# apache/yunikorn-k8shim

Measured on AMD Instinct MI355X. Metric: pod×node predicate evals/sec + decisions/sec, 50k nodes × 1M pods, higher is better.
Workload: dtype int64; 1 GPU; configs[2]: 50k nodes x 1M pods, NodeResourcesFit + TaintToleration + NodeAffinity; nodes_per_gpu=50000, total_nodes=50000, pods=1000000, templates=2000, pod_classes=2061, signature_planes=327, unique_requests=False, spread=False, gang_size=0, parallelism=single GPU

## Files before the change

### yunikorn-k8shim_amd/csrc/engine/engine.hip

```cpp
#include "../../../include/ykpred.h"

#include <hip/hip_runtime.h>
#include <dlfcn.h>
#include <rccl/rccl.h>

#include <algorithm>
#include <chrono>
#include <cstdio>
#include <cstdlib>
#include <cstring>
#include <mutex>
#include <string>
#include <map>
#include <unordered_map>
#include <vector>

#include "kernels.hip.h"
#include "preempt_headroom_finish.h"

using ykk::i64;
using ykk::u64;

namespace {

// ... 126 lines not shown
  T* as() const {
    return static_cast<T*>(p);
  }
};

struct ClassKey {
  int32_t a, b, c, d, pin;
  bool operator==(const ClassKey& o) const { return a == o.a && b == o.b && c == o.c && d == o.d && pin == o.pin; }
};
struct ClassKeyHash {
  size_t operator()(const ClassKey& k) const {
    uint64_t h = (uint64_t)(uint32_t)k.a * 0x9e3779b97f4a7c15ull;
    h ^= ((uint64_t)(uint32_t)k.b + 0x7f4a7c15ull) * 0xbf58476d1ce4e5b9ull;
    h ^= ((uint64_t)(uint32_t)k.c + 0x1ce4e5b9ull) * 0x94d049bb133111ebull;
    h ^= ((uint64_t)(uint32_t)k.pin + 0x133111ebull) * 0xd6e8feb86659fd93ull;
    h ^= ((uint64_t)(uint32_t)k.d + 0x6659fd93ull) * 0xff51afd7ed558ccdull;
    return (size_t)(h ^ (h >> 29));
  }
};

struct Family {
  int D = 0;
  int base = 0;
};

}

struct ykpred_engine {
  mutable std::recursive_mutex mu;
  ykpred_config_t cfg{};
  int R = 3, KT = 1, W = 1;
  hipStream_t own_stream = nullptr;
  std::string err;

  int N = 0;
  int row_words = 0, row_stride = 0;
  DevBuf d_alloc, d_req, d_allowed, d_count, d_nflags, d_taints, d_labels, d_domain, d_selcount, d_ports;
  int KD = 0, KS = 0, KP = 0;
  std::vector<int32_t> h_domain_sizes;
  DevBuf d_score, d_key, d_rank, d_perm, d_rankbuf, d_member_key, d_name_rank, d_member_tie;
  bool has_name_rank = false;
  bool nodes_set = false;

  int S = 0;
  std::vector<i64> h_req;
  std::vector<u64> h_tol, h_wanted;
  std::vector<uint32_t> h_sflags;
  std::vector<int32_t> h_aff_off, h_pre_off, h_spread_off;
  std::vector<ykpred_spread_t> h_spread;
  std::vector<u64> h_aff_terms, h_pre_terms;
  DevBuf d_sreq, d_stol, d_sflags, d_aff_off, d_aff_terms, d_pre_off, d_pre_terms;
  std::vector<int32_t> spec_sig_res, spec_sig_tol, spec_sig_aff;
  Family fam_res, fam_tol, fam_aff, fam_spread;
  DevBuf planes_canon, planes_ranked;
  DevBuf base_canon, base_ranked;
  u64 taint_used[ykk::kMaxKT] = {0, 0, 0, 0};
  int plane_rows_alloc = 0;
  std::vector<int32_t> spec_sig_spread;
  std::vector<std::vector<ykpred_spread_t>> spread_sig;
  std::vector<int32_t> spread_sig_aff, spread_sig_tol;
  DevBuf d_spec_spread, d_sp_coff, d_sp_c, d_sp_aff, d_sp_tol, d_sp_cnt, d_sp_present, d_sp_min;
  DevBuf d_sp_cnt_prev, d_sp_present_prev, d_sp_min_prev, d_sig_changed, d_class_dirty;
  int spread_constraints = 0;
  int64_t spread_cells = 0;
  bool spread_dirty = true;
  int res_vectors = 0;
  std::vector<i64> h_dim_val;
  std::vector<int32_t> h_dim_of;
  std::vector<int32_t> h_stage_rows;
  DevBuf d_dim_val, d_dim_order, d_dim_chunk_dim, d_dim_chunk_begin, d_dim_chunk_len, d_res_rows;
  int dim_chunks = 0;
  int walk_rows = 256;
  int wave_combine_below = 16;
  int n_big = 0, walk_chunks = 0, index_rows = 0;
  int NCB = 0;
  DevBuf d_big_dim, d_walk_big, d_walk_begin, d_walk_len, d_sfree_c, d_pmask_c, d_sfree_r, d_pmask_r, d_rbits_c;
  std::vector<int32_t> h_res_rows;
  std::vector<int32_t> h_row_pos;
  std::vector<int32_t> h_row_big;
  std::vector<int32_t> h_sorted_off;
  DevBuf d_sorted, d_sorted_off, d_ent_c;
  int sweep_min_run = 1;
  int sweep_groups = 0;
  bool sweep_ready = false;
  std::vector<int32_t> h_class_sweep;
  int sweep_rows[ykk::kMaxIdxRows] = {0, 0}, sweep_row_off[ykk::kMaxIdxRows + 1] = {0, 0, 0}, sweep_runs = 0;
  int index_rows_needed = 0;
  DevBuf d_agree;
  DevBuf d_explain;
  DevBuf d_headroom;
  DevBuf d_groups;
  DevBuf d_domain_head;
  DevBuf d_reach;
  DevBuf d_rc_req, d_rc_pods, d_rc_ports;
  int rc_tiers = 0;
  bool rc_ports = false;
  DevBuf d_victims;
  DevBuf d_vt_base, d_vt_tier_end, d_vt_cum, d_vt_ports;
  std::vector<int32_t> h_vt_base, h_vt_cap;
  int vt_tiers = 0;
  size_t vt_rows = 0;
  bool vt_ports = false;
  DevBuf d_bytes_gather;
  DevBuf d_topo_agree;
  u64 dict_digest = 0;
  int fuse_rows = 1;
  int fuse_wpl = 0;
  int fuse_count = 0, fuse_row_count = 0;
  bool fuse_ready = false;
  DevBuf d_fuse_rec;
  int fuse_combos = 0;
  int fuse_combine = 1;
  DevBuf d_fuse_combo_rec, d_fuse_combo;
  std::vector<uint8_t> h_class_fused;
  int run_decide = 1;
  int run_ranges = 0, n_decide_list = 0, run_decide_classes = -1;
  bool win_partial = false;
  DevBuf d_run_ranges, d_no_decide, d_glin_r;
  int class_runs = 1;
  int class_runs_min_rows = 16;
  int run_classes = 0, run_units = 0, run_rows = 0;
  DevBuf d_run_classes, d_run_units;
  DevBuf d_sweep_rows, d_sweep_runs, d_sweep_units;
  int sweep_units[ykk::kMaxIdxRows] = {0, 0}, sweep_unit_off[ykk::kMaxIdxRows + 1] = {0, 0, 0};
  DevBuf d_chunk_list_b0;
  int NCB0 = 0;
  DevBuf d_walk2_order, d_walk2_big, d_walk2_begin, d_walk2_len;
  int walk2_chunks = -1;
  DevBuf d_first_r;
  static constexpr bool decide_skip = true;
  DevBuf d_chunk_list_b;
  DevBuf d_slice_general;
  DevBuf d_slice_desc;
  DevBuf d_pfx_r;
  DevBuf d_idx_c;
  DevBuf d_win_r;
  int idx_stride = 0;
  DevBuf d_sig_tol, d_sig_tolflags, d_sig_ports, d_swanted;
  DevBuf d_sig_aff_flags, d_sig_aff_off, d_sig_aff_terms, d_sig_pre_off, d_sig_pre_terms;
  bool specs_set = false;

  int P = 0, C = 0, NC = 0;
  std::vector<int32_t> h_pod_spec, h_pod_pin;
  DevBuf d_pod_spec, d_pod_pin, d_pod_class;
  DevBuf d_class_sig, d_class_pin, d_class_first, d_class_word, d_chunk_class, d_chunk_begin, d_chunk_len, d_chunk_first, d_members;
  std::unordered_map<ClassKey, int32_t, ClassKeyHash> class_ids;
  std::vector<int32_t> h_pod_class, h_pod_slot;
  std::vector<int32_t> h_pod_row;
  int rows_total = 0, rows_a = 0, row_capacity = 0;
  DevBuf d_pod_row;
  bool bands_enabled = true;
  int band_steps = 0;
  int band_steps_now = 128;
  int round_batched = -1;
  int round_node_assume = 1;
  int round_prof = 0;
  int fail_after = 0;
  int sig_wpl = 0;
  int combine_slices = 1;
  int decide_groups_from = 16384;
  int early_counts = 1;
  int group_lds = -1;
  int group_scratch_mb = 256;
  int affinity_fill_waves = 0;
  int group_chunk_tasks = 0;
  int max_lds_bytes = 64 * 1024;
  int num_cus = 256;
  int n_bands = 0, n_band_steps = 0, n_classes_a = 0, n_fix_rows = 0;
  std::vector<int32_t> h_class_slot_a;
  DevBuf d_band_tab, d_class_rows_a, d_class_list_a, d_class_slot_a, d_fix_row, d_fix_slot, d_chunk_zone;
  DevBuf d_class_list_b;
  int n_classes_b = 0;
  std::vector<int32_t> h_ch_zone;
  std::vector<uint8_t> h_row_stale;
  std::vector<int32_t> h_class_sig, h_class_pin, h_class_first, h_class_live;
  std::vector<std::vector<int32_t>> h_class_chunks;
  std::vector<int32_t> h_members, h_ch_class, h_ch_begin, h_ch_len, h_ch_first;
  int patch_chunks = 0;
  bool rank_valid = false;
  uint64_t specs_version = 1, ranked_specs_version = 0, ranked_nodes_epoch = 0;
  unsigned ranked_pre = 0, ranked_filt = 0;
  bool ranked_has_first = false;
  DevBuf d_round;
  DevBuf d_fx_off, d_fx_cls, d_fx_cnt, d_fx_occ, d_sp_sig_of;
  uint64_t fx_version = 0;
  bool fx_contrib = false, fx_ports = false;
  std::vector<int32_t> h_fx_off;
  std::vector<int32_t> h_fx_cls;
  std::vector<int32_t> h_fx_cnt;
  std::vector<uint8_t> h_fx_occupies;
  DevBuf d_patches, d_rows, d_row_count, d_row_best;
  unsigned last_pre = 0, last_filt = 0;
  bool last_eval_valid = false;
  DevBuf d_class_count, d_class_best;
  bool pods_set = false, classes_dirty = true;
  int chunk_members = ykk::kChunkMembers;
  bool chunk_sorted = true;
  int combine_lds_bytes = 40000;

  DevBuf d_bitmap, d_counts, d_decisions, d_keys, d_scratch;
  void* last_bitmap = nullptr;
  int64_t last_bitmap_rows = 0;
  void *last_counts = nullptr, *last_decisions = nullptr, *last_keys = nullptr;

  hipStream_t aux_stream = nullptr;
  hipEvent_t ev_fork = nullptr, ev_planes = nullptr, ev_join = nullptr, ev_counts = nullptr, ev_zero = nullptr;
  hipStream_t peek_stream = nullptr;
  hipEvent_t ev_eval_done = nullptr;
  void* peek_pinned = nullptr;
  size_t peek_pinned_bytes = 0;

  struct GraphKey {
    uint64_t version;
    unsigned pre, filt, options;
    void *bitmap, *counts, *decisions, *keys;
    bool operator==(const GraphKey& o) const {
      return version == o.version && pre == o.pre && filt == o.filt && options == o.options && bitmap == o.bitmap && counts == o.counts &&
             decisions == o.decisions && keys == o.keys;
    }
  };
  std::vector<std::pair<GraphKey, hipGraphExec_t>> graphs;
  std::vector<GraphKey> seen;
  uint64_t tables_version = 1;
  bool graph_disabled = true;

  ncclComm_t comm = nullptr;
  int comm_rank = 0, comm_world = 1, node_offset = 0;
  int64_t round_exchanges = 0;
  void* h_round_pinned = nullptr;
  size_t h_round_pinned_bytes = 0;
  int64_t rounds_batched = 0, round_batched_asks = 0, round_batches = 0, rounds_sequential = 0, round_sequential_asks = 0;
  int forced_stride = 0;
  DevBuf d_gathered, d_gathered_map, d_xkey, d_xcand;
  bool last_has_keys = false;
  DevBuf d_class_rows_all, d_gathered_classes, d_class_rows_slot, d_class_sig_ident, d_expand_count, d_layout_hash, d_gathered_pod_class, d_row_pod;
  int ident_classes = 0;
  uint64_t layout_version = 1, layout_hashed_version = 0, layout_hash_value = 0, row_pod_version = 0;
  uint64_t ask_epoch = 1, hdr_epoch = 0;
  std::vector<uint64_t> hdr_cache;
  uint64_t nodes_epoch = 1, hist_epoch = 0;
  uint64_t bitmap_epoch = 0;

  int64_t n_full_evals = 0, n_node_patches = 0, n_row_patches = 0, n_queries = 0, n_gathers = 0, n_uploads = 0;

  hipEvent_t ev[2 * YKPRED_MAX_TIMED_KERNELS + 2]{};
  bool ev_ready = false;
  int timed = 0;
  const char* timed_name[YKPRED_MAX_TIMED_KERNELS]{};
  bool timing_valid = false;
};

namespace {

int fail(ykpred_engine* e, int code, const std::string& msg) {
  if (e) e->err = msg;
  if (e && (code == YKPRED_E_DEVICE || code == YKPRED_E_NOMEM)) {
    e->last_eval_valid = false;
    e->rank_valid = false;
    e->classes_dirty = true;
    e->spread_dirty = true;
    e->hist_epoch = 0;
    e->ranked_nodes_epoch = 0;
    e->tables_version++;
  }
  return code;
}
inline bool inject_failure(ykpred_engine* e) { return e && e->fail_after > 0 && --e->fail_after == 0; }
#define HIPCHK(call)                                                                                        \
  do {                                                                                                      \
    hipError_t _s = inject_failure(e) ? hipErrorUnknown : (call);                                          \
    if (_s != hipSuccess)                                                                                   \
      return fail(e, _s == hipErrorOutOfMemory ? YKPRED_E_NOMEM : YKPRED_E_DEVICE,                          \
                  std::string(#call) + ": " + hipGetErrorString(_s));                                       \
  } while (0)

template <class T>
int upload(ykpred_engine* e, DevBuf& b, const T* src, size_t n, hipStream_t st) {
  HIPCHK(b.ensure(n * sizeof(T)));
  if (n) HIPCHK(hipMemcpyAsync(b.p, src, n * sizeof(T), hipMemcpyHostToDevice, st));
  return YKPRED_OK;
}
#define TRY(x)                     \
  do {                             \
    int _r = (x);                  \
    if (_r != YKPRED_OK) return _r; \
  } while (0)

ykk::NodeTable node_table(const ykpred_engine* e) {
  ykk::NodeTable t;
  t.n = e->N;
  t.R = e->R;
  t.KT = e->KT;
  t.W = e->W;
  t.alloc = e->d_alloc.as<i64>();
  t.req = e->d_req.as<i64>();
  t.allowed = e->d_allowed.as<int>();
  t.count = e->d_count.as<int>();
  t.flags = e->d_nflags.as<unsigned>();
  t.taints = e->d_taints.as<u64>();
  t.labels = e->d_labels.as<u64>();
  t.KD = e->KD;
  t.KS = e->KS;
  t.domain = e->d_domain.as<int>();
  t.selcount = e->d_selcount.as<int>();
  t.KP = e->KP;
  t.ports = e->d_ports.as<u64>();
  return t;
}
ykk::SpreadSigs spread_sigs(const ykpred_engine* e) {
  ykk::SpreadSigs sp;
  sp.D = e->fam_spread.D;
  sp.c_off = e->d_sp_coff.as<int>();
  sp.c = e->d_sp_c.as<ykk::SpreadC>();
  sp.aff_sig = e->d_sp_aff.as<int>();
  sp.tol_sig = e->d_sp_tol.as<int>();
  sp.cnt = e->d_sp_cnt.as<int>();
  sp.present = e->d_sp_present.as<int>();
  sp.minv = e->d_sp_min.as<int>();
  return sp;
}
ykk::SpecTable spec_table(const ykpred_engine* e) {
  ykk::SpecTable s;
  s.R = e->R;
  s.KT = e->KT;
  s.W = e->W;
  s.req = e->d_sreq.as<i64>();
  s.tol = e->d_stol.as<u64>();
  s.flags = e->d_sflags.as<unsigned>();
  s.aff.flags = e->d_sflags.as<unsigned>();
  s.aff.term_off = e->d_aff_off.as<int>();
  s.aff.terms = e->d_aff_terms.as<u64>();
  s.aff.pre_off = e->d_pre_off.as<int>();
  s.aff.pre_terms = e->d_pre_terms.as<u64>();
  s.KP = e->KP;
  s.wanted_ports = e->d_swanted.as<u64>();
  s.spread_sig = e->d_spec_spread.as<int>();
  s.spread = spread_sigs(e);
  return s;
}

int build_classes(ykpred_engine* e, hipStream_t st) {
  e->tables_version++;
  const int P = e->P;
  auto& ids = e->class_ids;
  ids.clear();
  ids.reserve(1024);
  auto& pod_class = e->h_pod_class;
  pod_class.assign((size_t)P, 0);
  auto &class_sig = e->h_class_sig, &class_pin = e->h_class_pin, &class_size = e->h_class_live;
  class_sig.clear();
  class_pin.clear();
  class_size.clear();
  for (int p = 0; p < P; ++p) {
    int s = e->h_pod_spec[(size_t)p];
    ClassKey k{e->spec_sig_res[(size_t)s], e->spec_sig_tol[(size_t)s], e->spec_sig_aff[(size_t)s], e->spec_sig_spread[(size_t)s],
               e->h_pod_pin[(size_t)p]};
    auto it = ids.find(k);
    int32_t c;
    if (it == ids.end()) {
      c = (int32_t)class_pin.size();
      ids.emplace(k, c);
      class_sig.insert(class_sig.end(), {k.a, k.b, k.c, k.d});
      class_pin.push_back(k.pin);
      class_size.push_back(0);
    } else {
      c = it->second;
    }
    pod_class[(size_t)p] = c;
    class_size[(size_t)c]++;
  }
  const int C = (int)class_pin.size();
  std::vector<int32_t> class_off((size_t)C + 1, 0);
  for (int c = 0; c < C; ++c) class_off[(size_t)c + 1] = class_off[(size_t)c] + class_size[(size_t)c];
  auto& members = e->h_members;
  members.assign((size_t)P, 0);
  e->h_pod_slot.assign((size_t)P, 0);
  std::vector<int32_t> cursor(class_off.begin(), class_off.end() - 1);
  for (int p = 0; p < P; ++p) {
    int slot = cursor[(size_t)pod_class[(size_t)p]]++;
    members[(size_t)slot] = p;
    e->h_pod_slot[(size_t)p] = slot;
  }
  const long row_b = (long)e->row_stride * 8, win = (long)ykk::kBandGroups * 4096;
  const int KC = ykk::kBandClasses;
  auto piece_min_of = [&](int steps) { return (int)((double)steps * (4096.0 + (double)row_b) / (double)row_b / (double)(KC - 1) * 1.3) + 3; };
  int S = e->band_steps;
  if (S <= 0) {
    int s_min = 8;
    while (s_min < 128 && (long)s_min * 4096 < 5L * KC * row_b) s_min *= 2;
    auto coverage = [&](int steps) {
      const int need = 2 * piece_min_of(steps);
      long rows = 0;
      for (int c = 0; c < C; ++c)
        if (class_size[(size_t)c] >= need) rows += class_size[(size_t)c];
      return rows;
    };
    const long best = coverage(s_min);
    S = 128;
    while (S > s_min && (double)coverage(S) < 0.5 * (double)best) S /= 2;
  }
  while (S > 4 && (long)S * win / row_b >= (1L << 21)) S -= 4;
  e->band_steps_now = S;
  const int piece_min = piece_min_of(S);
  e->h_class_slot_a.assign((size_t)C, -1);
  e->h_pod_row.assign((size_t)P, -1);
  std::vector<ykk::BandEntry> band_tab;
  std::vector<int32_t> class_list_a, fix_row, fix_slot;
  int n_steps = 0, n_bands = 0, rows_a = 0;
  const bool geometry_ok = e->bands_enabled && e->N > 0 && (size_t)2 * KC * (size_t)row_b <= (size_t)std::min(ykk::kBandMaxLds, e->max_lds_bytes);
  if (geometry_ok) {
    long rows_needed = 0;
    for (int c = 0; c < C; ++c)
      if (class_size[(size_t)c] >= 2 * piece_min) {
        e->h_class_slot_a[(size_t)c] = (int32_t)class_list_a.size();
        class_list_a.push_back(c);
// ... 433 lines not shown
          else rec.row[rec.n++] = r;
        }
        if (!ok) continue;
        recs.push_back(rec);
        e->h_class_fused[(size_t)c] = 1;
        e->fuse_count++;
        e->fuse_row_count += rec.len;
      }
      e->fuse_combos = 0;
      if (e->fuse_count > 0) {
        std::unordered_map<uint64_t, int32_t> combo_of;
        std::vector<ykk::FuseRec> combo_recs;
        std::vector<int32_t> combo_ix(recs.size(), -1);
        for (size_t i = 0; i < recs.size(); ++i) {
          const int32_t c = recs[i].cls;
          const uint64_t k2 = ((uint64_t)(uint32_t)key(c, 1) << 32) | (uint32_t)key(c, 0);
          auto it = combo_of.find(k2);
          if (it == combo_of.end()) {
            it = combo_of.emplace(k2, (int32_t)combo_recs.size()).first;
            ykk::FuseRec cr{};
            cr.cls = 0, cr.dest = it->second, cr.len = 1;
            for (int k = 1; k < recs[i].n; ++k) cr.row[cr.n++] = recs[i].row[k];
            combo_recs.push_back(cr);
          }
          combo_ix[i] = it->second;
        }
        bool combine = e->fuse_combine != 0 && combo_recs.size() * 4 <= recs.size() && combo_recs.size() <= 16384;
        for (const ykk::FuseRec& cr : combo_recs) combine = combine && cr.n >= 1;
        if (combine) {
          for (size_t i = 0; i < recs.size(); ++i) {
            recs[i].n = 2;
            recs[i].row[1] = (3 << ykk::kFuseFamShift) | combo_ix[i];
          }
          e->fuse_combos = (int)combo_recs.size();
          TRY(upload(e, e->d_fuse_combo_rec, combo_recs.data(), combo_recs.size(), st));
          HIPCHK(e->d_fuse_combo.ensure((size_t)e->fuse_combos * (size_t)e->row_stride * sizeof(u64)));
        }
        TRY(upload(e, e->d_fuse_rec, recs.data(), recs.size(), st));
        e->fuse_ready = true;
      }
      if (getenv("YKPRED_TRACE_RUNS")) {
        long t_cls = 0, t_rows = 0, t_single = 0, t_single_shared = 0, t_single_big = 0, t_single_spread = 0, t_pinned = 0;
        for (int32_t c : order_b) {
          if (!tail[(size_t)c] || e->h_class_sweep[(size_t)c] || e->h_class_fused[(size_t)c]) continue;
          ++t_cls, t_rows += class_size[(size_t)c];
          if (class_size[(size_t)c] == 1) {
            ++t_single;
            const int sa = key(c, 2);
            if (sa >= 0 && sa < e->fam_aff.D && users[(size_t)sa] != 1) ++t_single_shared;
            if (key(c, 3) >= 0) ++t_single_spread;
            if (class_pin[(size_t)c] != -1) ++t_pinned;
            const int sr = key(c, 0);
            if (sr >= 0)
              for (int k = 0; k < R1; ++k)
                if (e->h_res_rows[(size_t)sr * (size_t)R1 + (size_t)k] > 0 && (e->h_res_rows[(size_t)sr * (size_t)R1 + (size_t)k] >> ykk::kRowBigShift)) { ++t_single_big; break; }
          }
        }
        fprintf(stderr, "fused: %d classes, %d rows, %d combinations; chunk writers keep %ld classes / %ld rows of zone B (%ld single-row: %ld share their affinity signature, %ld with an index row, %ld spread, %ld pinned)\n",
                e->fuse_count, e->fuse_row_count, e->fuse_combos, t_cls, t_rows, t_single, t_single_shared, t_single_big, t_single_spread, t_pinned);
      }
    }
  }
  e->rows_total = next_row;
  e->rows_a = rows_a;
  e->n_bands = n_bands;
  e->n_band_steps = n_steps;
  e->n_classes_a = (int)class_list_a.size();
  e->n_fix_rows = (int)fix_row.size();
  if (e->row_capacity && e->rows_total > e->row_capacity)
    return fail(e, YKPRED_E_INVALID, "the bitmap needs more rows than ykpred_set_row_capacity allows");
  const int cm = e->chunk_members;
  struct Chunk {
    int32_t cls, begin, len, first, first_row;
  };
  std::vector<Chunk> chunks;
  for (int c = 0; c < C; ++c)
    for (int b = class_off[(size_t)c]; b < class_off[(size_t)c + 1]; b += cm)
      chunks.push_back({c, b, std::min(cm, class_off[(size_t)c + 1] - b), b == class_off[(size_t)c] ? 1 : 0, e->h_pod_row[(size_t)members[(size_t)b]]});
  if (e->chunk_sorted)
    std::stable_sort(chunks.begin(), chunks.end(), [](const Chunk& x, const Chunk& y) { return x.first_row < y.first_row; });
  auto &ch_class = e->h_ch_class, &ch_begin = e->h_ch_begin, &ch_len = e->h_ch_len, &ch_first = e->h_ch_first;
  ch_class.clear();
  ch_begin.clear();
  ch_len.clear();
  ch_first.clear();
  e->h_ch_zone.clear();
  e->h_class_chunks.assign((size_t)C, {});
  for (const Chunk& k : chunks) {
    e->h_class_chunks[(size_t)k.cls].push_back((int32_t)ch_class.size());
    ch_class.push_back(k.cls);
    ch_begin.push_back(k.begin);
    ch_len.push_back(k.len);
    ch_first.push_back(k.first);
    e->h_ch_zone.push_back(e->h_class_slot_a[(size_t)k.cls] >= 0 ? 1 : (e->h_class_sweep[(size_t)k.cls] ? 2 : (e->h_class_fused[(size_t)k.cls] ? 3 : 0)));
  }
  std::vector<int32_t> chunk_list_b;
  for (size_t k = 0; k < e->h_ch_zone.size(); ++k)
    if (e->h_ch_zone[k] != 1) chunk_list_b.push_back((int32_t)k);
  e->NCB = (int)chunk_list_b.size();
  {
    std::vector<int32_t> chunk_list_b0;
    for (size_t k = 0; k < e->h_ch_zone.size(); ++k)
      if (e->h_ch_zone[k] == 0) chunk_list_b0.push_back((int32_t)k);
    e->NCB0 = (int)chunk_list_b0.size();
    TRY(upload(e, e->d_chunk_list_b0, chunk_list_b0.data(), chunk_list_b0.size(), st));
  }
  e->h_class_first.assign((size_t)C, -1);
  for (int c = 0; c < C; ++c) e->h_class_first[(size_t)c] = members[(size_t)class_off[(size_t)c]];
  std::vector<int32_t> member_rows((size_t)P);
  for (int i = 0; i < P; ++i) member_rows[(size_t)i] = e->h_pod_row[(size_t)members[(size_t)i]];
  e->h_row_stale.assign((size_t)P, 0);
  e->C = C;
  e->NC = (int)ch_class.size();
  e->patch_chunks = 0;
  TRY(upload(e, e->d_pod_class, pod_class.data(), pod_class.size(), st));
  TRY(upload(e, e->d_class_sig, class_sig.data(), class_sig.size(), st));
  TRY(upload(e, e->d_class_pin, class_pin.data(), class_pin.size(), st));
  TRY(upload(e, e->d_class_first, e->h_class_first.data(), e->h_class_first.size(), st));
  TRY(upload(e, e->d_members, member_rows.data(), member_rows.size(), st));
  TRY(upload(e, e->d_pod_row, e->h_pod_row.data(), e->h_pod_row.size(), st));
  TRY(upload(e, e->d_chunk_zone, e->h_ch_zone.data(), e->h_ch_zone.size(), st));
  TRY(upload(e, e->d_chunk_list_b, chunk_list_b.data(), chunk_list_b.size(), st));
  TRY(upload(e, e->d_band_tab, band_tab.data(), band_tab.size(), st));
  TRY(upload(e, e->d_class_list_a, class_list_a.data(), class_list_a.size(), st));
  TRY(upload(e, e->d_class_slot_a, e->h_class_slot_a.data(), e->h_class_slot_a.size(), st));
  TRY(upload(e, e->d_fix_row, fix_row.data(), fix_row.size(), st));
  TRY(upload(e, e->d_fix_slot, fix_slot.data(), fix_slot.size(), st));
  HIPCHK(e->d_class_rows_a.ensure((size_t)std::max<size_t>(class_list_a.size(), 1) * (size_t)e->row_stride * sizeof(u64)));
  TRY(upload(e, e->d_chunk_class, ch_class.data(), ch_class.size(), st));
  TRY(upload(e, e->d_chunk_begin, ch_begin.data(), ch_begin.size(), st));
  TRY(upload(e, e->d_chunk_len, ch_len.data(), ch_len.size(), st));
  TRY(upload(e, e->d_chunk_first, ch_first.data(), ch_first.size(), st));
  HIPCHK(e->d_class_count.ensure((size_t)std::max(C, 1) * sizeof(int)));
  HIPCHK(e->d_class_best.ensure((size_t)std::max(C, 1) * sizeof(int)));
  HIPCHK(hipStreamSynchronize(st));
  e->classes_dirty = false;
  e->layout_version++;
  e->last_eval_valid = false;
  return YKPRED_OK;
}

int ensure_planes(ykpred_engine* e, hipStream_t st) {
  int rows = 0;
  for (Family* f : {&e->fam_res, &e->fam_spread, &e->fam_tol, &e->fam_aff}) {
    f->base = rows;
    rows += std::max(f->D, 1);
  }
  size_t need = ((size_t)rows * (size_t)e->row_stride + 64) * sizeof(u64);
  for (DevBuf* b : {&e->planes_canon, &e->planes_ranked}) {
    if (b->cap < need || e->plane_rows_alloc != rows) {
      e->tables_version++;
      HIPCHK(b->ensure(need));
      HIPCHK(hipMemsetAsync(b->p, 0, need, st));
    }
  }
  e->plane_rows_alloc = rows;
  size_t base_need = (size_t)(64 * (e->W + e->KT + e->KP) + 2) * (size_t)e->row_stride * sizeof(u64);
  for (DevBuf* b : {&e->base_canon, &e->base_ranked}) {
    if (b->cap < base_need) {
      e->tables_version++;
      HIPCHK(b->ensure(base_need));
      HIPCHK(hipMemsetAsync(b->p, 0, base_need, st));
    }
  }
  return YKPRED_OK;
}

int build_spread_tables(ykpred_engine* e, hipStream_t st) {
  e->tables_version++;
  std::vector<int32_t> coff{0}, aff, tol;
  std::vector<ykk::SpreadC> rows;
  int64_t cells = 0;
  for (size_t d = 0; d < e->spread_sig.size(); ++d) {
    for (const ykpred_spread_t& c : e->spread_sig[d]) {
      if (c.topology_key < 0 || c.topology_key >= e->KD || c.selector_class >= e->KS)
        return fail(e, YKPRED_E_INVALID, "spread constraint references a topology key / selector class outside the node table");
      ykk::SpreadC r;
      r.kd = c.topology_key;
      r.ks = c.selector_class;
      r.max_skew = c.max_skew;
      r.min_domains = c.min_domains;
      r.self_match = c.self_match;
      r.flags = c.flags;
      r.kind = c.kind;
      r.dom_size = (size_t)c.topology_key < e->h_domain_sizes.size() ? e->h_domain_sizes[(size_t)c.topology_key] : 0;
      r.cnt_off = (int)cells;
      cells += r.dom_size;
      if (cells > 0x7fffffff) return fail(e, YKPRED_E_UNSUPPORTED, "spread histograms exceed 2^31 cells");
      rows.push_back(r);
    }
    coff.push_back((int32_t)rows.size());
    aff.push_back(e->spread_sig_aff[d]);
    tol.push_back(e->spread_sig_tol[d]);
  }
  e->spread_constraints = (int)rows.size();
  e->spread_cells = cells;
  TRY(upload(e, e->d_sp_coff, coff.data(), coff.size(), st));
  TRY(upload(e, e->d_sp_c, rows.data(), rows.size(), st));
  TRY(upload(e, e->d_sp_aff, aff.data(), aff.size(), st));
  TRY(upload(e, e->d_sp_tol, tol.data(), tol.size(), st));
  HIPCHK(e->d_sp_cnt.ensure((size_t)std::max<int64_t>(cells, 1) * sizeof(int)));
  HIPCHK(e->d_sp_present.ensure((size_t)std::max<int64_t>(cells, 1) * sizeof(int)));
  HIPCHK(e->d_sp_min.ensure((size_t)std::max(e->spread_constraints, 1) * sizeof(int)));
  HIPCHK(hipStreamSynchronize(st));
  e->spread_dirty = false;
  return YKPRED_OK;
}

struct Timer {
  ykpred_engine* e;
  bool on;
  void start(hipStream_t st) {
    e->timed = 0;
    e->timing_valid = false;
    if (on) (void)hipEventRecord(e->ev[2 * YKPRED_MAX_TIMED_KERNELS], st);
  }
  void begin(hipStream_t st) {
    if (on && e->timed < YKPRED_MAX_TIMED_KERNELS) (void)hipEventRecord(e->ev[2 * e->timed], st);
  }
  void end(hipStream_t st, const char* name) {
    if (trace_kernels_on()) {
      const hipError_t s = hipStreamSynchronize(st);
      fprintf(stderr, "ykpred: %s %s\n", name, s == hipSuccess ? "done" : hipGetErrorString(s));
      fflush(stderr);
    }
    if (!on || e->timed >= YKPRED_MAX_TIMED_KERNELS) return;
    (void)hipEventRecord(e->ev[2 * e->timed + 1], st);
    e->timed_name[e->timed] = name;
    e->timed++;
  }
  void done(hipStream_t st) {
    if (on) (void)hipEventRecord(e->ev[2 * YKPRED_MAX_TIMED_KERNELS + 1], st);
    e->timing_valid = on;
  }
};

int grow_owned_outputs(ykpred_engine* e) {
  const size_t P = (size_t)std::max(e->P, 1);
  if (e->last_bitmap && e->last_bitmap == e->d_bitmap.p) {
    HIPCHK(e->d_bitmap.reserve_keep((size_t)std::max(std::max(e->rows_total, e->row_capacity), 1) * (size_t)e->row_stride * sizeof(u64), e->d_bitmap.cap));
    e->last_bitmap = e->d_bitmap.p;
  }
  if (e->last_counts && e->last_counts == e->d_counts.p) {
    HIPCHK(e->d_counts.reserve_keep(P * sizeof(int), e->d_counts.cap));
    e->last_counts = e->d_counts.p;
  }
  if (e->last_decisions && e->last_decisions == e->d_decisions.p) {
    HIPCHK(e->d_decisions.reserve_keep(P * sizeof(int), e->d_decisions.cap));
    e->last_decisions = e->d_decisions.p;
  }
  if (e->last_keys && e->last_keys == e->d_keys.p) {
    HIPCHK(e->d_keys.reserve_keep(P * sizeof(i64), e->d_keys.cap));
    e->last_keys = e->d_keys.p;
  }
  return YKPRED_OK;
}

int run_spread_prefilter(ykpred_engine* e, hipStream_t st, Timer* tm, bool do_count, bool do_min) {
  if (e->spread_dirty) TRY(build_spread_tables(e, st));
  if (e->fam_spread.D == 0 || e->N == 0) return YKPRED_OK;
  ykk::NodeTable nt = node_table(e);
  ykk::SpreadSigs sp = spread_sigs(e);
  if (do_count) {
    HIPCHK(hipMemsetAsync(e->d_sp_cnt.p, 0, (size_t)e->spread_cells * sizeof(int), st));
    HIPCHK(hipMemsetAsync(e->d_sp_present.p, 0, (size_t)e->spread_cells * sizeof(int), st));
    ykk::AffSigs as{e->d_sig_aff_flags.as<unsigned>(), e->d_sig_aff_off.as<int>(), e->d_sig_aff_terms.as<u64>(), e->d_sig_pre_off.as<int>(),
                    e->d_sig_pre_terms.as<u64>()};
    if (tm) tm->begin(st);
    hipLaunchKernelGGL(ykk::k_spread_count, dim3((unsigned)e->fam_spread.D, (unsigned)((e->N + ykk::kBlock - 1) / ykk::kBlock)),
                       dim3(ykk::kBlock), 0, st, nt, sp, as, e->d_sig_tol.as<u64>());
    if (tm) tm->end(st, "k_spread_count");
  }
  if (do_min) {
    if (tm) tm->begin(st);
    hipLaunchKernelGGL(ykk::k_spread_min, dim3((unsigned)e->spread_constraints), dim3(ykk::kWave), 0, st, sp, e->spread_constraints);
    if (tm) tm->end(st, "k_spread_min");
  }
  HIPCHK(hipGetLastError());
  return YKPRED_OK;
}

struct Roctx {
  int (*push)(const char*) = nullptr;
  int (*pop)() = nullptr;
};
Roctx* roctx() {
  static Roctx r;
  static std::once_flag once;
  std::call_once(once, [] {
    void* lib = nullptr;
    const char* names[] = {"librocprofiler-sdk-roctx.so.1", "libroctx64.so.4", "libroctx64.so"};
    for (const char* n : names)
      if (!lib) lib = dlopen(n, RTLD_NOW | RTLD_NOLOAD);
    const char* want = getenv("YKPRED_ROCTX");
    if (!lib && want && want[0] == '1')
      for (const char* n : names)
        if (!lib) lib = dlopen(n, RTLD_NOW | RTLD_GLOBAL);
    if (!lib) return;
    r.push = (int (*)(const char*))dlsym(lib, "roctxRangePushA");
    r.pop = (int (*)())dlsym(lib, "roctxRangePop");
    if (!r.push || !r.pop) r.push = nullptr;
  });
  return &r;
}
struct Range {
  bool on;
  explicit Range(const char* name) : on(roctx()->push != nullptr) {
    if (on) roctx()->push(name);
  }
  ~Range() {
    if (on) roctx()->pop();
  }
};

struct Rccl {
  void* lib = nullptr;
  ncclResult_t (*GetUniqueId)(ncclUniqueId*) = nullptr;
  ncclResult_t (*CommInitRank)(ncclComm_t*, int, ncclUniqueId, int) = nullptr;
  ncclResult_t (*CommDestroy)(ncclComm_t) = nullptr;
  ncclResult_t (*AllGather)(const void*, void*, size_t, ncclDataType_t, ncclComm_t, hipStream_t) = nullptr;
  ncclResult_t (*AllReduce)(const void*, void*, size_t, ncclDataType_t, ncclRedOp_t, ncclComm_t, hipStream_t) = nullptr;
  const char* (*GetErrorString)(ncclResult_t) = nullptr;
  std::string error;
};
std::string& rccl_library_override() {
  static std::string path;
  return path;
}
Rccl* rccl() {
  static Rccl r;
  static std::once_flag once;
  std::call_once(once, [] {
    if (!rccl_library_override().empty()) {
      r.lib = dlopen(rccl_library_override().c_str(), RTLD_NOW | RTLD_LOCAL);
      if (!r.lib) {
        r.error = std::string("cannot load ") + rccl_library_override() + ": " + dlerror();
        return;
      }
    }
    for (const char* name : {"librccl.so.1", "librccl.so", "/opt/rocm/lib/librccl.so.1"}) {
      if (r.lib) break;
      r.lib = dlopen(name, RTLD_NOW | RTLD_GLOBAL | RTLD_NOLOAD);
    }
    for (const char* name : {"librccl.so.1", "librccl.so", "/opt/rocm/lib/librccl.so.1"}) {
      if (r.lib) break;
      r.lib = dlopen(name, RTLD_NOW | RTLD_GLOBAL);
    }
    if (!r.lib) {
      r.error = std::string("cannot load librccl: ") + dlerror();
      return;
    }
    auto sym = [&](const char* n) {
      void* p = dlsym(r.lib, n);
      if (!p && r.error.empty()) r.error = std::string("librccl lacks ") + n;
      return p;
    };
    r.GetUniqueId = (decltype(r.GetUniqueId))sym("ncclGetUniqueId");
    r.CommInitRank = (decltype(r.CommInitRank))sym("ncclCommInitRank");
    r.CommDestroy = (decltype(r.CommDestroy))sym("ncclCommDestroy");
    r.AllGather = (decltype(r.AllGather))sym("ncclAllGather");
    r.AllReduce = (decltype(r.AllReduce))sym("ncclAllReduce");
    r.GetErrorString = (decltype(r.GetErrorString))sym("ncclGetErrorString");
  });
  return &r;
}
#define NCCLCHK(call)                                                                                     \
  do {                                                                                                    \
    ncclResult_t _s = (call);                                                                             \
    if (_s != ncclSuccess) return fail(e, YKPRED_E_DEVICE, std::string(#call) + ": " + rccl()->GetErrorString(_s)); \
  } while (0)

u64 topology_digest(const ykpred_engine* e) {
  u64 h = 0xcbf29ce484222325ull;
  auto mix = [&](u64 v) { h = (h ^ v) * 0x100000001b3ull; };
  mix((u64)e->spread_cells);
  mix((u64)e->spread_constraints);
  mix((u64)e->KD);
  mix((u64)e->KS);
  for (int32_t d : e->h_domain_sizes) mix((u64)(uint32_t)d);
  mix(e->dict_digest);
  return h;
}
struct TopoShape {
  int64_t cells;
  u64 digest;
};
int agree_topology(ykpred_engine* e, hipStream_t st, const char* where) {
  const int W = e->comm_world;
  const TopoShape mine{e->spread_cells, topology_digest(e)};
  HIPCHK(e->d_topo_agree.ensure((size_t)(W + 1) * sizeof(TopoShape)));
  TopoShape* d = e->d_topo_agree.as<TopoShape>();
  HIPCHK(hipMemcpyAsync(d + W, &mine, sizeof mine, hipMemcpyHostToDevice, st));
  NCCLCHK(rccl()->AllGather(d + W, d, sizeof(TopoShape), ncclInt8, e->comm, st));
  std::vector<TopoShape> all((size_t)W);
  HIPCHK(hipMemcpyAsync(all.data(), d, (size_t)W * sizeof(TopoShape), hipMemcpyDeviceToHost, st));
  HIPCHK(hipStreamSynchronize(st));
  for (int g = 0; g < W; ++g)
    if (all[(size_t)g].cells != all[0].cells || all[(size_t)g].digest != all[0].digest)
      return fail(e, YKPRED_E_INVALID, std::string(where) + " (sharded): rank " + std::to_string(g) + "'s topology histograms have " +
                                         std::to_string(all[(size_t)g].cells) + " cells, rank 0's " + std::to_string(all[0].cells) +
                                         (all[(size_t)g].cells == all[0].cells ? " laid out differently" : "") +
                                         ": the shards do not share the topology-domain dictionaries (a node update brought a domain to one "
                                         "shard only?) — no rank sums them");
  return YKPRED_OK;
}

int allreduce_spread(ykpred_engine* e, hipStream_t st) {
  if (!e->comm || e->comm_world <= 1) return YKPRED_OK;
  TRY(agree_topology(e, st, "topology histogram sum"));
  if (e->spread_cells == 0) return YKPRED_OK;
  NCCLCHK(rccl()->AllReduce(e->d_sp_cnt.p, e->d_sp_cnt.p, (size_t)e->spread_cells, ncclInt32, ncclSum, e->comm, st));
  NCCLCHK(rccl()->AllReduce(e->d_sp_present.p, e->d_sp_present.p, (size_t)e->spread_cells, ncclInt32, ncclMax, e->comm, st));
  return YKPRED_OK;
}

int ensure_histograms(ykpred_engine* e, hipStream_t st) {
  if (e->spread_dirty) TRY(build_spread_tables(e, st));
  if (e->fam_spread.D == 0 || e->hist_epoch == e->nodes_epoch) return YKPRED_OK;
  if (e->comm && e->comm_world > 1)
    return fail(e, YKPRED_E_STATE, "topology histograms are stale on a sharded engine: run ykpred_eval on every shard first (it sums them across shards)");
  TRY(run_spread_prefilter(e, st, nullptr, true, true));
  e->hist_epoch = e->nodes_epoch;
  return YKPRED_OK;
}

int complete_windows(ykpred_engine* e, hipStream_t st) {
  if (!e->win_partial || e->n_big == 0 || e->walk_chunks == 0) return YKPRED_OK;
  ykk::DimWalk dw{e->d_dim_val.as<i64>(), e->d_dim_order.as<int>(), e->d_big_dim.as<int>(), e->d_walk_big.as<int>(), e->d_walk_begin.as<int>(),
                  e->d_walk_len.as<int>(), e->d_sfree_r.as<i64>(), e->d_pmask_r.as<u64>(), e->n_big, e->walk_chunks, e->row_words, nullptr,
                  nullptr, e->d_sorted.as<i64>(), e->d_sorted_off.as<int>(), nullptr};
  const unsigned gy = (unsigned)((e->row_words + ykk::kBlock * ykk::kWalkWords - 1) / (ykk::kBlock * ykk::kWalkWords));
  hipLaunchKernelGGL(ykk::k_dim_walk_window<ykk::kWalkBatch>, dim3((unsigned)e->walk_chunks, gy), dim3(ykk::kBlock), 0, st, dw, e->d_pfx_r.as<i64>(), e->d_win_r.as<unsigned char>());
  HIPCHK(hipGetLastError());
  e->win_partial = false;
  return YKPRED_OK;
}

ykk::Planes ranked_planes_of(const ykpred_engine* e, unsigned pre, unsigned filt, bool spread_on, bool with_first) {
  const bool res_on = filt & YKPRED_PLUGIN_NODE_RESOURCES_FIT, aff_on = (filt | pre) & YKPRED_PLUGIN_NODE_AFFINITY;
  const int fit_error = (pre & YKPRED_PLUGIN_NODE_RESOURCES_FIT) ? 0 : 1;
  auto ranked_of = [&](const Family& f) { return e->planes_ranked.as<u64>() + (size_t)f.base * e->row_stride; };
  int* first_r = with_first ? e->d_first_r.as<int>() : nullptr;
  ykk::Planes pr{res_on ? ranked_of(e->fam_res) : nullptr, ranked_of(e->fam_tol), aff_on ? ranked_of(e->fam_aff) : nullptr,
                 spread_on ? ranked_of(e->fam_spread) : nullptr, e->row_stride, e->d_res_rows.as<int>(), 1 + e->R, nullptr,
                 e->idx_stride, e->d_pmask_r.as<u64>(), e->row_words, first_r, e->fam_res.base, e->fam_tol.base, e->fam_aff.base,
                 e->fam_spread.base, 0, nullptr, nullptr, nullptr, nullptr, nullptr};
  pr.n_big = res_on ? e->n_big : 0;
  if (res_on && e->n_big > 0) {
    pr.res_win = e->d_win_r.as<unsigned char>();
    pr.sfree = e->d_sfree_r.as<i64>();
    pr.res_val = e->d_dim_val.as<i64>();
    if (!fit_error) pr.pfx = e->d_pfx_r.as<i64>();
  }
  return pr;
}

}

#define YK_SERIALISE(eng) \
  std::unique_lock<std::recursive_mutex> engine_lock; \
  if (eng) engine_lock = std::unique_lock<std::recursive_mutex>((eng)->mu)

extern "C" {

int32_t ykpred_abi_version(void) { return YKPRED_ABI_VERSION; }

const char* ykpred_last_error(const ykpred_engine_t* e) { return e ? e->err.c_str() : g_create_error.c_str(); }

int32_t ykpred_create(const ykpred_config_t* cfg, ykpred_engine_t** out) {
  if (!cfg || !out) {
    g_create_error = "null argument";
    return YKPRED_E_INVALID;
  }
  if (cfg->abi_version != YKPRED_ABI_VERSION) {
    g_create_error = "ABI version mismatch";
    return YKPRED_E_INVALID;
  }
  if (cfg->num_resources < 3 || cfg->num_resources > ykk::kMaxR || cfg->taint_words < 1 || cfg->taint_words > ykk::kMaxKT ||
      cfg->label_words < 1 || cfg->label_words > ykk::kMaxWTotal) {
    g_create_error = "config out of range: need 3<=R<=8, 1<=KT<=4, 1<=W<=32";
    return YKPRED_E_UNSUPPORTED;
  }
  if (cfg->topology_keys < 0 || cfg->topology_keys > ykk::kMaxKD || cfg->selector_classes < 0 || cfg->selector_classes > 4096 ||
      cfg->port_words < 0 || cfg->port_words > ykk::kMaxKP) {
    g_create_error = "config out of range: need 0<=KD<=8 topology keys, 0<=KS<=4096 selector classes, 0<=KP<=4 port words";
    return YKPRED_E_UNSUPPORTED;
  }
  int ndev = 0;
  hipError_t s = hipGetDeviceCount(&ndev);
  if (s != hipSuccess || ndev <= 0) {
    g_create_error = std::string("no HIP device: ") + hipGetErrorString(s) + " (libykpred has no CPU fallback)";
    return YKPRED_E_DEVICE;
  }
  if (cfg->device < 0 || cfg->device >= ndev) {
    g_create_error = "device ordinal out of range";
    return YKPRED_E_INVALID;
  }
  s = hipSetDevice(cfg->device);
  if (s != hipSuccess) {
    g_create_error = std::string("hipSetDevice: ") + hipGetErrorString(s);
    return YKPRED_E_DEVICE;
  }
  auto* e = new ykpred_engine();
  e->cfg = *cfg;
  e->R = cfg->num_resources;
  e->KT = cfg->taint_words;
  e->W = cfg->label_words;
  e->KD = cfg->topology_keys;
  e->KS = cfg->selector_classes;
  e->KP = cfg->port_words;
  if (cfg->reserved[0] >= 1 && cfg->reserved[0] <= ykk::kChunkMembers) e->chunk_members = cfg->reserved[0];
  e->chunk_sorted = cfg->reserved[1] != 1;
  if (cfg->reserved[2] > 0 && cfg->reserved[2] <= 160 * 1024) e->combine_lds_bytes = cfg->reserved[2];
  if (cfg->reserved[2] < 0) e->combine_lds_bytes = 0;
  if (cfg->reserved[4] > 0) e->walk_rows = cfg->reserved[4];
  if (cfg->reserved[5] > 0) e->wave_combine_below = cfg->reserved[5];
  if (cfg->reserved[5] < 0) e->wave_combine_below = 0;
  if (cfg->reserved[6] < 0) e->bands_enabled = false;
  if (cfg->reserved[6] > 0) e->band_steps = std::min(256, std::max(4, (cfg->reserved[6] + 3) / 4 * 4));
  e->graph_disabled = cfg->reserved[3] != 1;
  {
    int lds = 0;
    if (hipDeviceGetAttribute(&lds, hipDeviceAttributeMaxSharedMemoryPerBlock, cfg->device) == hipSuccess && lds > 0) e->max_lds_bytes = lds;
    int cus = 0;
    if (hipDeviceGetAttribute(&cus, hipDeviceAttributeMultiprocessorCount, cfg->device) == hipSuccess && cus > 0) e->num_cus = cus;
  }
  if (const char* tune = getenv("YKPRED_TUNE")) {
    std::string text(tune);
    size_t at = 0;
    while (at < text.size()) {
      size_t stop = text.find(',', at);
      if (stop == std::string::npos) stop = text.size();
      const std::string item = text.substr(at, stop - at);
      at = stop + 1;
      if (item.empty()) continue;
      const size_t eq = item.find('=');
      const std::string key = item.substr(0, eq);
      const int val = eq == std::string::npos ? 1 : atoi(item.c_str() + eq + 1);
      if (key == "walk_rows") e->walk_rows = std::max(val, 1);
      else if (key == "sig_wpl") e->sig_wpl = val;
      else if (key == "combine_slices") e->combine_slices = val;
      else if (key == "decide_groups_from") e->decide_groups_from = val;
      else if (key == "graph") e->graph_disabled = val != 1;
      else if (key == "early_counts") e->early_counts = val;
      else if (key == "band_steps") {
        e->bands_enabled = val >= 0;
        e->band_steps = val > 0 ? std::min(256, std::max(4, (val + 3) / 4 * 4)) : 0;
      } else if (key == "chunk_members") e->chunk_members = std::min(std::max(val, 1), (int)ykk::kChunkMembers);
      else if (key == "wave_combine_below") e->wave_combine_below = std::max(val, 0);
      else if (key == "fail_after") e->fail_after = std::max(val, 0);
      else if (key == "round_prof") e->round_prof = val;
      else if (key == "round_batched") e->round_batched = val;
      else if (key == "round_node_assume") e->round_node_assume = val;
      else if (key == "sweep_min_run") e->sweep_min_run = std::max(val, 0);
      else if (key == "sweep_groups") e->sweep_groups = std::max(val, 0);
      else if (key == "class_runs") e->class_runs = val;
      else if (key == "run_decide") e->run_decide = val;
      else if (key == "fuse_rows") e->fuse_rows = val;
      else if (key == "fuse_wpl") e->fuse_wpl = val;
      else if (key == "fuse_combine") e->fuse_combine = val;
      else if (key == "class_runs_min_rows") e->class_runs_min_rows = std::max(val, 1);
      else if (key == "group_lds") e->group_lds = val;
      else if (key == "group_scratch_mb") e->group_scratch_mb = std::max(val, 0);
      else if (key == "group_chunk_tasks") e->group_chunk_tasks = std::max(val, 0);
      else if (key == "affinity_fill_waves") e->affinity_fill_waves = val;
      else {
        g_create_error = "YKPRED_TUNE: unknown key '" + key + "'";
        delete e;
        return YKPRED_E_INVALID;
      }
    }
  }
  s = hipStreamCreateWithFlags(&e->own_stream, hipStreamNonBlocking);
  if (s != hipSuccess) {
    g_create_error = std::string("hipStreamCreate: ") + hipGetErrorString(s);
    delete e;
    return YKPRED_E_DEVICE;
  }
  {
    int lo = 0, hi = 0;
    (void)hipDeviceGetStreamPriorityRange(&lo, &hi);
    if (hipStreamCreateWithPriority(&e->aux_stream, hipStreamNonBlocking, hi) != hipSuccess)
      (void)hipStreamCreateWithFlags(&e->aux_stream, hipStreamNonBlocking);
  }
  if (hipStreamCreateWithFlags(&e->peek_stream, hipStreamNonBlocking) != hipSuccess) e->peek_stream = nullptr;
  (void)hipEventCreateWithFlags(&e->ev_eval_done, hipEventDisableTiming);
  (void)hipEventCreateWithFlags(&e->ev_fork, hipEventDisableTiming);
  (void)hipEventCreateWithFlags(&e->ev_join, hipEventDisableTiming);
  (void)hipEventCreateWithFlags(&e->ev_planes, hipEventDisableTiming);
  (void)hipEventCreateWithFlags(&e->ev_counts, hipEventDisableTiming);
  (void)hipEventCreateWithFlags(&e->ev_zero, hipEventDisableTiming);
  for (auto& ev : e->ev) (void)hipEventCreate(&ev);
  e->ev_ready = true;
  *out = e;
  return YKPRED_OK;
}

void ykpred_destroy(ykpred_engine_t* e) {
  if (!e) return;
  (void)hipSetDevice(e->cfg.device);
  (void)hipDeviceSynchronize();
  if (e->comm) (void)rccl()->CommDestroy(e->comm);
  e->comm = nullptr;
  for (DevBuf* b : {&e->d_gathered, &e->d_gathered_map, &e->d_xkey, &e->d_xcand}) b->release();
  for (auto& g : e->graphs) (void)hipGraphExecDestroy(g.second);
  e->graphs.clear();
  for (DevBuf* b : {&e->d_alloc, &e->d_req, &e->d_allowed, &e->d_count, &e->d_nflags, &e->d_taints, &e->d_labels, &e->d_domain, &e->d_selcount, &e->d_ports, &e->d_sig_ports, &e->d_swanted,
                    &e->d_sp_cnt_prev, &e->d_sp_present_prev, &e->d_sp_min_prev, &e->d_sig_changed, &e->d_class_dirty,
                    &e->d_spec_spread, &e->d_sp_coff, &e->d_sp_c, &e->d_sp_aff, &e->d_sp_tol, &e->d_sp_cnt, &e->d_sp_present, &e->d_sp_min,
                    &e->planes_canon, &e->planes_ranked, &e->base_canon, &e->base_ranked, &e->d_rankbuf, &e->d_score, &e->d_key,
                    &e->d_rank, &e->d_perm, &e->d_sreq, &e->d_stol, &e->d_sflags, &e->d_aff_off, &e->d_aff_terms, &e->d_pre_off,
                    &e->d_pre_terms, &e->d_dim_val, &e->d_dim_order, &e->d_dim_chunk_dim, &e->d_dim_chunk_begin, &e->d_dim_chunk_len,
                    &e->d_res_rows, &e->d_big_dim, &e->d_walk_big, &e->d_walk_begin, &e->d_walk_len, &e->d_sfree_c, &e->d_pmask_c,
                    &e->d_sfree_r, &e->d_pmask_r, &e->d_rbits_c, &e->d_sorted, &e->d_sorted_off, &e->d_ent_c, &e->d_agree, &e->d_topo_agree, &e->d_bytes_gather, &e->d_fuse_rec, &e->d_fuse_combo_rec, &e->d_fuse_combo, &e->d_run_ranges, &e->d_no_decide, &e->d_glin_r, &e->d_run_classes, &e->d_run_units, &e->d_sweep_rows, &e->d_sweep_runs, &e->d_sweep_units, &e->d_chunk_list_b0, &e->d_walk2_order, &e->d_walk2_big, &e->d_walk2_begin, &e->d_walk2_len, &e->d_idx_c, &e->d_win_r, &e->d_pfx_r, &e->d_slice_desc, &e->d_slice_general, &e->d_chunk_list_b, &e->d_first_r, &e->d_sig_tol, &e->d_sig_tolflags, &e->d_sig_aff_flags, &e->d_sig_aff_off,
                    &e->d_sig_aff_terms, &e->d_sig_pre_off, &e->d_sig_pre_terms, &e->d_pod_spec, &e->d_pod_pin, &e->d_pod_class,
                    &e->d_class_sig, &e->d_class_pin, &e->d_class_first, &e->d_class_word, &e->d_chunk_class, &e->d_chunk_begin, &e->d_chunk_len, &e->d_chunk_first,
                    &e->d_pod_row, &e->d_band_tab, &e->d_class_rows_a, &e->d_class_list_a, &e->d_class_slot_a, &e->d_fix_row, &e->d_fix_slot, &e->d_chunk_zone,
                    &e->d_members, &e->d_patches, &e->d_rows, &e->d_row_count, &e->d_row_best, &e->d_class_count, &e->d_class_best, &e->d_bitmap, &e->d_counts, &e->d_decisions, &e->d_keys, &e->d_scratch,
                    &e->d_member_key, &e->d_name_rank, &e->d_member_tie, &e->d_class_rows_all, &e->d_gathered_classes, &e->d_class_rows_slot,
                    &e->d_class_sig_ident, &e->d_expand_count, &e->d_layout_hash, &e->d_gathered_pod_class, &e->d_row_pod,
                    &e->d_round, &e->d_fx_off, &e->d_fx_cls, &e->d_fx_cnt, &e->d_fx_occ, &e->d_sp_sig_of, &e->d_class_list_b, &e->d_gathered, &e->d_gathered_map,
                    &e->d_xkey, &e->d_xcand, &e->d_reach, &e->d_rc_req, &e->d_rc_pods, &e->d_rc_ports, &e->d_victims,
                    &e->d_vt_base, &e->d_vt_tier_end, &e->d_vt_cum, &e->d_vt_ports})
    b->release();
  if (e->ev_ready)
    for (auto& ev : e->ev) (void)hipEventDestroy(ev);
  if (e->ev_fork) (void)hipEventDestroy(e->ev_fork);
  if (e->ev_join) (void)hipEventDestroy(e->ev_join);
  if (e->ev_planes) (void)hipEventDestroy(e->ev_planes);
  if (e->ev_counts) (void)hipEventDestroy(e->ev_counts);
  if (e->ev_zero) (void)hipEventDestroy(e->ev_zero);
  if (e->h_round_pinned) (void)hipHostFree(e->h_round_pinned);
  if (e->ev_eval_done) (void)hipEventDestroy(e->ev_eval_done);
  if (e->peek_pinned) (void)hipHostFree(e->peek_pinned);
  if (e->peek_stream) (void)hipStreamDestroy(e->peek_stream);
  if (e->aux_stream) (void)hipStreamDestroy(e->aux_stream);
  if (e->own_stream) (void)hipStreamDestroy(e->own_stream);
  delete e;
}

int32_t ykpred_set_nodes(ykpred_engine_t* e, const ykpred_nodes_t* n) {
  YK_SERIALISE(e);
  Range roctx_range("ykpred:upload_nodes");
  if (e) e->n_uploads++;
  if (e) e->tables_version++;
  if (e) e->nodes_epoch++;
  if (e) e->ask_epoch++;
  if (e) e->last_eval_valid = false;
  if (!e || !n || n->count < 0) return fail(e, YKPRED_E_INVALID, "set_nodes: bad argument");
  if (n->count > 0 && (!n->allocatable || !n->requested || !n->allowed_pods || !n->pod_count || !n->flags || !n->taint_bits ||
                       !n->label_bits))
    return fail(e, YKPRED_E_INVALID, "set_nodes: null column");
  if ((e->KD > 0 && (!n->domain_sizes || (n->count > 0 && !n->domain_id))) || (e->KS > 0 && n->count > 0 && !n->selector_count))
    return fail(e, YKPRED_E_INVALID, "set_nodes: topology / selector columns missing (config has KD/KS > 0)");
  if (e->KP > 0 && n->count > 0 && !n->port_bits) return fail(e, YKPRED_E_INVALID, "set_nodes: port_bits missing (config has KP > 0)");
  HIPCHK(hipSetDevice(e->cfg.device));
  hipStream_t st = e->own_stream;
  e->rank_valid = false;
  const size_t N = (size_t)n->count;
  TRY(upload(e, e->d_alloc, n->allocatable, N * (size_t)e->R, st));
  TRY(upload(e, e->d_req, n->requested, N * (size_t)e->R, st));
  TRY(upload(e, e->d_allowed, n->allowed_pods, N, st));
  TRY(upload(e, e->d_count, n->pod_count, N, st));
  TRY(upload(e, e->d_nflags, n->flags, N, st));
  TRY(upload(e, e->d_taints, n->taint_bits, N * (size_t)e->KT, st));
  TRY(upload(e, e->d_labels, n->label_bits, N * (size_t)e->W, st));
  TRY(upload(e, e->d_domain, n->domain_id, N * (size_t)e->KD, st));
  TRY(upload(e, e->d_selcount, n->selector_count, N * (size_t)e->KS, st));
  TRY(upload(e, e->d_ports, n->port_bits, N * (size_t)e->KP, st));
  e->has_name_rank = n->name_rank != nullptr && N > 0;
  if (e->has_name_rank) TRY(upload(e, e->d_name_rank, n->name_rank, N, st));
  HIPCHK(e->d_member_tie.ensure(std::max<size_t>(N, 1) * sizeof(int)));
  for (int k = 0; k < ykk::kMaxKT; ++k) e->taint_used[k] = 0;
  for (int k = 0; k < e->KT; ++k)
    for (size_t i = 0; i < N; ++i) e->taint_used[k] |= n->taint_bits[(size_t)k * N + i];
  e->h_domain_sizes.assign(n->domain_sizes, n->domain_sizes + e->KD);
  e->spread_dirty = true;
  HIPCHK(e->d_score.ensure(N * sizeof(double)));
  HIPCHK(e->d_key.ensure(N * sizeof(u64)));
  HIPCHK(e->d_rank.ensure(N * sizeof(int)));
  HIPCHK(e->d_perm.ensure(N * sizeof(int)));
  HIPCHK(e->d_rankbuf.ensure((3 * (size_t)ykk::kRankBuckets + 1 + N) * sizeof(int)));
  HIPCHK(e->d_member_key.ensure(N * sizeof(u64)));
  HIPCHK(hipStreamSynchronize(st));
  if (e->N != n->count) {
    e->planes_canon.release();
    e->planes_ranked.release();
    e->base_canon.release();
    e->base_ranked.release();
    e->rc_tiers = 0;
    e->vt_tiers = 0;
  }
  e->N = n->count;
  e->row_words = (e->N + 63) / 64;
  e->row_stride = std::max(16, (e->row_words + 15) / 16 * 16);
  if (e->forced_stride) {
    if (e->forced_stride < e->row_stride) return fail(e, YKPRED_E_INVALID, "set_nodes: ykpred_set_row_stride is smaller than this shard needs");
    e->row_stride = e->forced_stride;
  }
  e->nodes_set = true;
  return YKPRED_OK;
}

int32_t ykpred_update_node(ykpred_engine_t* e, int32_t idx, const ykpred_nodes_t* n) {
  YK_SERIALISE(e);
// ... 314 lines not shown
        e->h_sorted_off.push_back((int32_t)sorted.size());
      }
      sorted.push_back(0);
      TRY(upload(e, e->d_sorted, sorted.data(), sorted.size(), st));
      TRY(upload(e, e->d_sorted_off, e->h_sorted_off.data(), e->h_sorted_off.size(), st));
    }
    e->h_stage_rows.clear();
    {
      std::vector<uint8_t> walked((size_t)R, 0);
      for (int32_t d : big_dim) walked[(size_t)d] = 1;
      for (int d = 1; d < rows && (int)e->h_stage_rows.size() < ykk::kWalkMaxStage; ++d)
        if (!walked[(size_t)e->h_dim_of[(size_t)d]]) e->h_stage_rows.push_back(d);
    }
    e->dim_chunks = (int)cdim.size();
    e->n_big = (int)big_dim.size();
    e->walk_chunks = (int)wbig.size();
    TRY(upload(e, e->d_dim_val, e->h_dim_val.data(), e->h_dim_val.size(), st));
    TRY(upload(e, e->d_dim_order, order.data(), order.size(), st));
    TRY(upload(e, e->d_dim_chunk_dim, cdim.data(), cdim.size(), st));
    TRY(upload(e, e->d_dim_chunk_begin, cbegin.data(), cbegin.size(), st));
    TRY(upload(e, e->d_dim_chunk_len, clen.data(), clen.size(), st));
    TRY(upload(e, e->d_big_dim, big_dim.data(), big_dim.size(), st));
    TRY(upload(e, e->d_walk_big, wbig.data(), wbig.size(), st));
    TRY(upload(e, e->d_walk_begin, wbegin.data(), wbegin.size(), st));
    TRY(upload(e, e->d_walk_len, wlen.data(), wlen.size(), st));
    TRY(upload(e, e->d_res_rows, res_rows.data(), res_rows.size(), st));
  }
  TRY(upload(e, e->d_sig_tol, sig_tol.data(), sig_tol.size(), st));
  TRY(upload(e, e->d_sig_tolflags, sig_tolflags.data(), sig_tolflags.size(), st));
  TRY(upload(e, e->d_sig_ports, sig_ports.data(), sig_ports.size(), st));
  TRY(upload(e, e->d_sig_aff_flags, sig_aff_flags.data(), sig_aff_flags.size(), st));
  TRY(upload(e, e->d_sig_aff_off, sig_aff_off.data(), sig_aff_off.size(), st));
  TRY(upload(e, e->d_sig_pre_off, sig_pre_off.data(), sig_pre_off.size(), st));
  TRY(upload(e, e->d_sig_aff_terms, sig_aff_terms.data(), sig_aff_terms.size(), st));
  TRY(upload(e, e->d_sig_pre_terms, sig_pre_terms.data(), sig_pre_terms.size(), st));
  HIPCHK(hipStreamSynchronize(st));
  e->specs_set = true;
  if (!append_only) e->classes_dirty = true;
  if (!spread_unchanged) e->last_eval_valid = false;
  return YKPRED_OK;
}

int32_t ykpred_set_pods(ykpred_engine_t* e, const ykpred_pods_t* p) {
  YK_SERIALISE(e);
  Range roctx_range("ykpred:upload_asks");
  if (e) e->n_uploads++;
  if (e) e->tables_version++;
  if (e) e->ask_epoch++;
  if (!e || !p || p->count < 0) return fail(e, YKPRED_E_INVALID, "set_pods: bad argument");
  if (p->count > 0 && (!p->spec_index || !p->node_name_index)) return fail(e, YKPRED_E_INVALID, "set_pods: null column");
  HIPCHK(hipSetDevice(e->cfg.device));
  e->P = p->count;
  e->h_pod_spec.assign(p->spec_index, p->spec_index + p->count);
  e->h_pod_pin.assign(p->node_name_index, p->node_name_index + p->count);
  TRY(upload(e, e->d_pod_spec, e->h_pod_spec.data(), e->h_pod_spec.size(), e->own_stream));
  TRY(upload(e, e->d_pod_pin, e->h_pod_pin.data(), e->h_pod_pin.size(), e->own_stream));
  HIPCHK(hipStreamSynchronize(e->own_stream));
  e->pods_set = true;
  e->classes_dirty = true;
  return YKPRED_OK;
}

static int validate_state(ykpred_engine* e) {
  if (!e->nodes_set || !e->specs_set || !e->pods_set) return fail(e, YKPRED_E_STATE, "nodes, specs and pods must be uploaded first");
  for (int p = 0; p < e->P; ++p) {
    int s = e->h_pod_spec[(size_t)p], pin = e->h_pod_pin[(size_t)p];
    if (s < 0 || s >= e->S) return fail(e, YKPRED_E_INVALID, "pod references a spec that was not uploaded");
    if (pin < YKPRED_UNKNOWN_NODE_NAME || pin >= e->N) return fail(e, YKPRED_E_INVALID, "pod node_name_index out of range");
  }
  return YKPRED_OK;
}

int32_t ykpred_eval(ykpred_engine_t* e, const ykpred_eval_args_t* a) {
  YK_SERIALISE(e);
  Range roctx_range("ykpred:eval");
  if (!e || !a) return fail(e, YKPRED_E_INVALID, "eval: bad argument");
  HIPCHK(hipSetDevice(e->cfg.device));
  hipStream_t st = a->stream ? (hipStream_t)a->stream : e->own_stream;
  if (e->classes_dirty) {
    if (a->options & (YKPRED_EVAL_SKIP_BITMAP | YKPRED_EVAL_DIRTY_CLASSES))
      return fail(e, YKPRED_E_STATE, "eval: the pod classes are due for a rebuild — run a full ykpred_eval (bitmap included)");
    TRY(validate_state(e));
    TRY(build_classes(e, e->own_stream));
  }
  const unsigned pre = a->prefilter_plugins, filt = a->filter_plugins;
  const bool spread_filt = filt & YKPRED_PLUGIN_POD_TOPOLOGY_SPREAD, spread_pre = pre & YKPRED_PLUGIN_POD_TOPOLOGY_SPREAD;
  const bool ipa_filt = filt & YKPRED_PLUGIN_INTER_POD_AFFINITY, ipa_pre = pre & YKPRED_PLUGIN_INTER_POD_AFFINITY;
  const bool spread_err = (spread_filt && !spread_pre) || (ipa_filt && !ipa_pre) ||
                          ((filt & YKPRED_PLUGIN_NODE_PORTS) && !(pre & YKPRED_PLUGIN_NODE_PORTS));
  if (e->spread_dirty) TRY(build_spread_tables(e, e->own_stream));
  const bool pts_en = spread_filt && spread_pre, ipa_en = ipa_filt && ipa_pre;
  const bool spread_on = (pts_en || ipa_en) && e->fam_spread.D > 0;
  const int N = e->N, P = e->P;
  const size_t bitmap_bytes = (size_t)std::max(std::max(e->rows_total, e->row_capacity), 1) * (size_t)e->row_stride * sizeof(u64);
  u64* bitmap = (u64*)a->bitmap;
  int64_t bitmap_rows = 0;
  if (!bitmap || (void*)bitmap == e->d_bitmap.p) {
    HIPCHK(e->d_bitmap.ensure(bitmap_bytes));
    bitmap = e->d_bitmap.as<u64>();
    bitmap_rows = (int64_t)(e->d_bitmap.cap / ((size_t)std::max(e->row_stride, 1) * sizeof(u64)));
  } else {
    bitmap_rows = a->bitmap_rows ? (int64_t)a->bitmap_rows : (int64_t)e->row_capacity;
    if (bitmap_rows == 0)
      return fail(e, YKPRED_E_INVALID, "eval: a caller-owned bitmap needs eval_args.bitmap_rows or ykpred_set_row_capacity (it must hold layout.num_rows rows)");
    if ((int64_t)e->rows_total > bitmap_rows)
      return fail(e, YKPRED_E_INVALID, "eval: the caller-owned bitmap holds fewer rows than the layout needs (layout.num_rows)");
  }
  e->last_bitmap = bitmap;
  e->last_bitmap_rows = bitmap_rows;
  HIPCHK(e->d_counts.ensure((size_t)std::max(P, 1) * sizeof(int)));
  HIPCHK(e->d_decisions.ensure((size_t)std::max(P, 1) * sizeof(int)));
  HIPCHK(e->d_keys.ensure((size_t)std::max(P, 1) * sizeof(i64)));
  e->last_counts = a->counts ? a->counts : e->d_counts.p;
  e->last_decisions = a->decisions ? a->decisions : e->d_decisions.p;
  e->last_keys = a->decision_keys ? a->decision_keys : e->d_keys.p;
  TRY(ensure_planes(e, st));
  if (e->n_big > 0) {
    const size_t cells = (size_t)e->n_big * (size_t)std::max(e->row_words, 1);
    for (DevBuf* b : {&e->d_sfree_c, &e->d_sfree_r}) HIPCHK(b->ensure(cells * 64 * sizeof(i64)));
    for (DevBuf* b : {&e->d_pmask_c, &e->d_pmask_r}) HIPCHK(b->ensure(cells * 65 * sizeof(u64)));
    HIPCHK(e->d_rbits_c.ensure(cells * ykk::kRankBits * sizeof(u64)));
    HIPCHK(e->d_ent_c.ensure(cells * 65 * sizeof(unsigned)));
    HIPCHK(e->d_glin_r.ensure(cells * 65 * sizeof(unsigned)));
    const int idx_stride_before = e->idx_stride;
    e->idx_stride = (std::max(e->row_words, e->row_stride) + 63) / 64 * 64;
    for (DevBuf* b : {&e->d_idx_c}) {
      const size_t need = (size_t)e->fam_res.D * (size_t)e->idx_stride;
      if (b->cap < need || !b->p || idx_stride_before != e->idx_stride) {
        HIPCHK(b->ensure(need));
        HIPCHK(hipMemsetAsync(b->p, 64, need, st));
      }
    }
    {
      const size_t need = (size_t)e->fam_res.D * 64;
      if (e->d_win_r.cap < need || !e->d_win_r.p) {
        HIPCHK(e->d_win_r.ensure(need));
        HIPCHK(hipMemsetAsync(e->d_win_r.p, 64, need, st));
      }
    }
  }
  Timer tm{e, (a->options & YKPRED_EVAL_PROFILE) != 0};
  tm.start(st);
  if (N == 0 || P == 0) {
    tm.done(st);
    return YKPRED_OK;
  }
  ykk::NodeTable nt = node_table(e);
  const bool want_keys = a->options & YKPRED_OUT_DECISION_KEYS;
  const bool want_dec = (a->options & YKPRED_OUT_DECISIONS) || want_keys;
  const bool want_cnt = a->options & YKPRED_OUT_COUNTS;
  const int nblk_nodes = (N + ykk::kBlock - 1) / ykk::kBlock;

  bool use_run_decide_pass = false;
  auto enqueue = [&]() -> int {
  if (spread_on || (a->options & YKPRED_EVAL_SPREAD_COUNT_ONLY)) {
    const bool ready = a->options & YKPRED_EVAL_SPREAD_COUNTS_READY, only = a->options & YKPRED_EVAL_SPREAD_COUNT_ONLY;
    TRY(run_spread_prefilter(e, st, &tm, !ready, false));
    if (only) return 1;
    if (!ready) TRY(allreduce_spread(e, st));
    TRY(run_spread_prefilter(e, st, &tm, false, true));
    e->hist_epoch = e->nodes_epoch;
  }
  if (a->options & YKPRED_EVAL_DIRECT) {
    ykk::SpecTable stbl = spec_table(e);
    dim3 grid((unsigned)((P + ykk::kWave - 1) / ykk::kWave), (unsigned)((e->row_stride + ykk::kWavesPerBlock - 1) / ykk::kWavesPerBlock));
    tm.begin(st);
    hipLaunchKernelGGL(ykk::k_direct, grid, dim3(ykk::kBlock), 0, st, nt, stbl, P, e->d_pod_spec.as<int>(), e->d_pod_pin.as<int>(),
                       e->d_pod_row.as<int>(), pre, filt, bitmap, e->row_words, e->row_stride);
    tm.end(st, "k_direct");
    HIPCHK(hipGetLastError());
    return 1;
  }

  const unsigned wgroups = (unsigned)((e->row_words + ykk::kWavesPerBlock - 1) / ykk::kWavesPerBlock);
  const bool res_on = filt & YKPRED_PLUGIN_NODE_RESOURCES_FIT;
  const bool aff_on = (filt | pre) & YKPRED_PLUGIN_NODE_AFFINITY;
  const int fit_error = (pre & YKPRED_PLUGIN_NODE_RESOURCES_FIT) ? 0 : 1;
  auto sig_chunks = [](int D) {
    const int spb = ykk::sigs_per_block(D);
    return (unsigned)((D + spb - 1) / spb);
  };
  ykk::AffSigs as{e->d_sig_aff_flags.as<unsigned>(), e->d_sig_aff_off.as<int>(), e->d_sig_aff_terms.as<u64>(), e->d_sig_pre_off.as<int>(),
                  e->d_sig_pre_terms.as<u64>()};
  auto canon_of = [&](const Family& f) { return e->planes_canon.as<u64>() + (size_t)f.base * e->row_stride; };
  auto ranked_of = [&](const Family& f) { return e->planes_ranked.as<u64>() + (size_t)f.base * e->row_stride; };
  ykk::PlaneOut o_res{canon_of(e->fam_res), ranked_of(e->fam_res), e->row_stride, e->fam_res.D, nullptr};
  ykk::PlaneOut o_tol{canon_of(e->fam_tol), ranked_of(e->fam_tol), e->row_stride, e->fam_tol.D, nullptr};
  ykk::PlaneOut o_aff{canon_of(e->fam_aff), ranked_of(e->fam_aff), e->row_stride, e->fam_aff.D, nullptr};
  ykk::PlaneOut o_spread{canon_of(e->fam_spread), ranked_of(e->fam_spread), e->row_stride, e->fam_spread.D, nullptr};
  const bool full_pass = !(a->options & (YKPRED_EVAL_SKIP_BITMAP | YKPRED_EVAL_DIRTY_CLASSES));
  const bool counts_early_here = e->early_counts != 0 && full_pass && e->n_classes_a > 0 && e->patch_chunks == 0 &&
                                 !((long)e->NC * e->wave_combine_below > (long)P) && e->n_classes_b <= 16384;
  const bool zero_counts_beside = full_pass && !counts_early_here && e->ev_zero != nullptr && e->C >= 65536 &&
                                  (a->options & (YKPRED_OUT_DECISIONS | YKPRED_OUT_DECISION_KEYS)) != 0;
  const bool use_sweep = e->sweep_ready && e->sweep_runs > 0 && res_on && !fit_error && full_pass && !counts_early_here;
  const bool sweep_rows_on = use_sweep && e->n_big > 0 && e->sweep_row_off[ykk::kMaxIdxRows] > 0;
  const bool fuse_on = e->fuse_ready && res_on && !fit_error && full_pass && !counts_early_here && aff_on && !spread_err;
  const bool use_run_decide = e->run_decide != 0 && e->sweep_ready && e->run_ranges > 0 && res_on && !fit_error && e->n_big > 0 &&
                              (a->options & (YKPRED_OUT_DECISIONS | YKPRED_OUT_DECISION_KEYS)) && e->walk2_chunks >= 0 &&
                              e->C == e->run_decide_classes;
  use_run_decide_pass = use_run_decide;
  ykk::ClassTable ct{e->d_class_sig.as<int>(), e->d_class_pin.as<int>(),  e->d_chunk_class.as<int>(), e->d_chunk_begin.as<int>(),
                     e->d_chunk_len.as<int>(), e->d_chunk_first.as<int>(), e->d_members.as<int>(), e->d_chunk_zone.as<int>(), (use_sweep ? 1 : 0) | (fuse_on ? 2 : 0),
                     use_run_decide ? e->d_no_decide.as<int>() : nullptr};
  ykk::Planes pc{res_on ? o_res.canon : nullptr, o_tol.canon, aff_on ? o_aff.canon : nullptr, spread_on ? o_spread.canon : nullptr,
                 e->row_stride, e->d_res_rows.as<int>(), 1 + e->R, e->d_idx_c.as<unsigned char>(), e->idx_stride, e->d_pmask_c.as<u64>(), e->row_words,
                 nullptr, 0, 0, 0, 0, 0, nullptr, nullptr, nullptr, nullptr, nullptr};
  int* first_r = nullptr;
  if ((a->options & (YKPRED_OUT_DECISIONS | YKPRED_OUT_DECISION_KEYS)) && e->decide_skip) {
    HIPCHK(e->d_first_r.ensure((size_t)std::max(e->plane_rows_alloc, 1) * sizeof(int)));
    first_r = e->d_first_r.as<int>();
  }
  if (want_dec && res_on && e->n_big > 0 && !fit_error) HIPCHK(e->d_pfx_r.ensure((size_t)e->n_big * (size_t)std::max(e->row_words, 1) * sizeof(i64)));
  ykk::Planes pr = ranked_planes_of(e, pre, filt, spread_on, first_r != nullptr);
  pc.n_big = pr.n_big;
  pc.rbits = e->d_rbits_c.as<u64>();
  const int pin_on = ((filt & YKPRED_PLUGIN_NODE_NAME) ? 1 : 0) | (spread_err ? 2 : 0);
  hipStream_t sb = e->aux_stream;

  if (want_dec) {
    HIPCHK(hipEventRecord(e->ev_fork, st));
    HIPCHK(hipStreamWaitEvent(sb, e->ev_fork, 0));
    if (zero_counts_beside) {
      HIPCHK(hipMemsetAsync(e->d_class_count.p, 0, (size_t)e->C * sizeof(int), sb));
      HIPCHK(hipEventRecord(e->ev_zero, sb));
    }
    if (first_r) HIPCHK(hipMemsetAsync(first_r, 0x7f, (size_t)std::max(e->plane_rows_alloc, 1) * sizeof(int), sb));
    tm.begin(sb);
    hipLaunchKernelGGL(ykk::k_score, dim3((unsigned)nblk_nodes), dim3(ykk::kBlock), 0, sb, nt, e->d_score.as<double>(), e->d_key.as<u64>());
    tm.end(sb, "k_score");
    int* hist = e->d_rankbuf.as<int>();
    int* bucket_off = hist + ykk::kRankBuckets;
    int* cursor = bucket_off + ykk::kRankBuckets + 1;
    int* members = cursor + ykk::kRankBuckets;
    HIPCHK(hipMemsetAsync(hist, 0, ykk::kRankBuckets * sizeof(int), sb));
    tm.begin(sb);
    hipLaunchKernelGGL(ykk::k_rank_hist, dim3((unsigned)nblk_nodes), dim3(ykk::kBlock), 0, sb, N, e->d_score.as<double>(), hist);
    hipLaunchKernelGGL(ykk::k_rank_scan, dim3(1), dim3(ykk::kRankBuckets), 0, sb, hist, bucket_off, cursor);
    hipLaunchKernelGGL(ykk::k_rank_fill, dim3((unsigned)nblk_nodes), dim3(ykk::kBlock), 0, sb, N, e->d_score.as<double>(), e->d_key.as<u64>(),
                       e->has_name_rank ? e->d_name_rank.as<int>() : (const int*)nullptr, cursor, members, e->d_member_tie.as<int>(),
                       e->d_member_key.as<u64>());
    hipLaunchKernelGGL(ykk::k_rank_final, dim3((unsigned)ykk::kRankBuckets), dim3(ykk::kBlock), 0, sb, bucket_off, members,
                       e->d_member_tie.as<int>(), e->d_member_key.as<u64>(), e->d_rank.as<int>(), e->d_perm.as<int>());
    tm.end(sb, "k_rank");
  }
  auto base_of = [&](DevBuf& buf) {
    ykk::BasePlanes bp;
    bp.req = buf.as<u64>();
    bp.taint = bp.req + (size_t)64 * e->W * e->row_stride;
    bp.port = bp.taint + (size_t)64 * e->KT * e->row_stride;
    bp.unsched = bp.port + (size_t)64 * e->KP * e->row_stride;
    bp.exists = bp.unsched + e->row_stride;
    bp.stride = e->row_stride;
    return bp;
  };
  auto launch_dictionary_planes = [&](hipStream_t s, const int* perm, bool ranked, const char* base_name, const char* sig_name, bool base_done = false) -> int {
    ykk::BasePlanes bp = base_of(ranked ? e->base_ranked : e->base_canon);
    if (!base_done) {
      tm.begin(s);
      hipLaunchKernelGGL(ykk::k_base_planes, dim3((unsigned)(e->W + e->KT + e->KP + 1), wgroups), dim3(ykk::kBlock), 0, s, nt, perm, bp,
                         e->row_words);
      tm.end(s, base_name);
    }
    ykk::SigPlaneArgs sa{};
    sa.base = bp;
    sa.tol = o_tol;
    sa.aff = o_aff;
    if (ranked) {
      sa.tol.canon = o_tol.ranked;
      sa.aff.canon = o_aff.ranked;
      sa.tol.first = first_r ? first_r + e->fam_tol.base : nullptr;
      sa.aff.first = first_r ? first_r + e->fam_aff.base : nullptr;
    }
    if (!aff_on) sa.aff.D = 0;
    sa.sig_tol = e->d_sig_tol.as<u64>();
    sa.sig_tolflags = e->d_sig_tolflags.as<unsigned>();
    sa.sig_ports = e->d_sig_ports.as<u64>();
    sa.KP = e->KP;
    for (int k = 0; k < ykk::kMaxKT; ++k) sa.taint_used[k] = e->taint_used[k];
    sa.affs = as;
    sa.KT = e->KT;
    sa.W = e->W;
    sa.pre_mask = pre;
    sa.filt_mask = filt;
    sa.n_words = e->row_words;
    tm.begin(s);
    const int wpl = e->sig_wpl > 0 ? e->sig_wpl : (e->row_words >= 4 * ykk::kWave ? 4 : (e->row_words >= 2 * ykk::kWave ? 2 : 1));
    const unsigned chunks = std::max((unsigned)((std::max(sa.tol.D, sa.aff.D) + ykk::kBitSigsPerBlock - 1) / ykk::kBitSigsPerBlock), 1u);
    const unsigned ygroups = (unsigned)((e->row_words + ykk::kBlock * wpl - 1) / (ykk::kBlock * wpl));
    if (wpl >= 4)
      hipLaunchKernelGGL(ykk::k_sig_planes<4>, dim3(chunks, ygroups, 2u), dim3(ykk::kBlock), 0, s, sa);
    else if (wpl >= 2)
      hipLaunchKernelGGL(ykk::k_sig_planes<2>, dim3(chunks, ygroups, 2u), dim3(ykk::kBlock), 0, s, sa);
    else
      hipLaunchKernelGGL(ykk::k_sig_planes<1>, dim3(chunks, ygroups, 2u), dim3(ykk::kBlock), 0, s, sa);
    tm.end(s, sig_name);
    return YKPRED_OK;
  };
  if (want_dec) TRY(launch_dictionary_planes(sb, e->d_perm.as<int>(), true, "k_base_planes(ranked)", "k_sig_planes(ranked)"));
  auto ranked_walk = [](const int* perm) { return perm != nullptr; };
  auto launch_ballot_planes = [&](hipStream_t s, const int* perm, const char* name, bool with_base = false) {
    ykk::PlaneArgs pa{};
    pa.perm = perm;
    pa.res = o_res;
    pa.spread = o_spread;
    if (perm && first_r) {
      pa.res.first = first_r + e->fam_res.base;
      pa.spread.first = first_r + e->fam_spread.base;
    }
    if (!spread_on) pa.spread.D = 0;
    pa.dims = ykk::DimPlanes{e->d_dim_val.as<i64>(), e->d_dim_order.as<int>(), e->d_dim_chunk_dim.as<int>(), e->d_dim_chunk_begin.as<int>(),
                             e->d_dim_chunk_len.as<int>(), res_on ? e->dim_chunks : 0};
    pa.spreads = spread_sigs(e);
    pa.fit_error = fit_error;
    pa.n_words = e->row_words;
    pa.spread_en = pts_en ? 1 : 0;
    pa.ipa_en = ipa_en ? 1 : 0;
    unsigned xchunks = std::max((unsigned)pa.dims.n_chunks, sig_chunks(pa.spread.D));
    tm.begin(s);
    if (with_base) {
      xchunks = std::max(xchunks, (unsigned)(e->W + e->KT + e->KP + 1));
      hipLaunchKernelGGL(ykk::k_node_planes, dim3(std::max(xchunks, 1u), wgroups, 3u), dim3(ykk::kBlock), 0, s, nt, pa,
                         base_of(perm ? e->base_ranked : e->base_canon));
    } else {
      hipLaunchKernelGGL(ykk::k_planes, dim3(std::max(xchunks, 1u), wgroups, spread_on ? 2u : 1u), dim3(ykk::kBlock), 0, s, nt, pa);
    }
    tm.end(s, name);
    if (res_on && e->n_big > 0 && !fit_error) {
      const bool ranked = perm != nullptr;
      ykk::DimWalk dw{e->d_dim_val.as<i64>(), e->d_dim_order.as<int>(), e->d_big_dim.as<int>(), e->d_walk_big.as<int>(), e->d_walk_begin.as<int>(),
                      e->d_walk_len.as<int>(), (ranked ? e->d_sfree_r : e->d_sfree_c).as<i64>(), (ranked ? e->d_pmask_r : e->d_pmask_c).as<u64>(),
                      e->n_big, e->walk_chunks, e->row_words, ranked ? nullptr : e->d_rbits_c.as<u64>(),
                      (!ranked && sweep_rows_on) ? e->d_ent_c.as<unsigned>() : nullptr, e->d_sorted.as<i64>(), e->d_sorted_off.as<int>(),
                      (ranked && use_run_decide) ? e->d_glin_r.as<unsigned>() : nullptr};
      tm.begin(s);
      hipLaunchKernelGGL(ykk::k_dim_sort, dim3((unsigned)e->n_big, wgroups), dim3(ykk::kBlock), 0, s, nt, perm, dw);
      tm.end(s, ranked ? "k_dim_sort(ranked)" : "k_dim_sort");
      tm.begin(s);
      const unsigned walk_gy = (unsigned)((e->row_words + ykk::kBlock * ykk::kWalkWords - 1) / (ykk::kBlock * ykk::kWalkWords));
      const dim3 walk_grid((unsigned)e->walk_chunks, walk_gy);
      if (!ranked && use_sweep && e->walk2_chunks >= 0) {
        if (e->walk2_chunks > 0) {
          ykk::DimWalk dw2 = dw;
          dw2.order = e->d_walk2_order.as<int>();
          dw2.chunk_big = e->d_walk2_big.as<int>();
          dw2.chunk_begin = e->d_walk2_begin.as<int>();
          dw2.chunk_len = e->d_walk2_len.as<int>();
          dw2.n_chunks = e->walk2_chunks;
          hipLaunchKernelGGL(ykk::k_dim_walk, dim3((unsigned)e->walk2_chunks, walk_gy), dim3(ykk::kBlock), 0, s, dw2, e->d_idx_c.as<unsigned char>(), e->idx_stride);
        }
      } else if (!ranked) {
        hipLaunchKernelGGL(ykk::k_dim_walk, walk_grid, dim3(ykk::kBlock), 0, s, dw, e->d_idx_c.as<unsigned char>(), e->idx_stride);
      } else {
        hipLaunchKernelGGL(ykk::k_dim_prefix_max, dim3((unsigned)e->n_big), dim3(ykk::kPfxBlock), 0, s, dw, e->d_pfx_r.as<i64>());
        if (use_run_decide) {
          if (e->walk2_chunks > 0) {
            ykk::DimWalk dw2 = dw;
            dw2.order = e->d_walk2_order.as<int>();
            dw2.chunk_big = e->d_walk2_big.as<int>();
            dw2.chunk_begin = e->d_walk2_begin.as<int>();
            dw2.chunk_len = e->d_walk2_len.as<int>();
            dw2.n_chunks = e->walk2_chunks;
            hipLaunchKernelGGL(ykk::k_dim_walk_window<8>, dim3((unsigned)e->walk2_chunks, walk_gy), dim3(ykk::kBlock), 0, s, dw2, e->d_pfx_r.as<i64>(), e->d_win_r.as<unsigned char>());
          }
        } else {
          hipLaunchKernelGGL(ykk::k_dim_walk_window<ykk::kWalkBatch>, walk_grid, dim3(ykk::kBlock), 0, s, dw, e->d_pfx_r.as<i64>(), e->d_win_r.as<unsigned char>());
        }
      }
      tm.end(s, ranked ? "k_dim_walk(ranked)" : "k_dim_walk");
    } else if (res_on && e->n_big > 0) {
      if (!ranked_walk(perm)) (void)hipMemsetAsync(e->d_idx_c.p, 64, (size_t)e->fam_res.D * (size_t)e->idx_stride, s);
      (void)hipMemsetAsync((ranked_walk(perm) ? e->d_pmask_r : e->d_pmask_c).p, 0, (size_t)e->n_big * (size_t)e->row_words * 65 * sizeof(u64), s);
      if (!ranked_walk(perm)) (void)hipMemsetAsync(e->d_rbits_c.p, 0, (size_t)e->n_big * (size_t)e->row_words * ykk::kRankBits * sizeof(u64), s);
    }
  };
  const bool fused_planes = res_on || spread_on;
  if (fused_planes) launch_ballot_planes(st, nullptr, "k_planes+k_base_planes", true);
  TRY(launch_dictionary_planes(st, nullptr, false, "k_base_planes", "k_sig_planes", fused_planes));
  if (want_dec) {
    HIPCHK(hipEventRecord(e->ev_planes, st));
    HIPCHK(hipStreamWaitEvent(sb, e->ev_planes, 0));
    const int ballot_rows = e->fam_tol.base;
    if (ballot_rows <= ykk::kManySigs && e->n_big == 0) {
      tm.begin(sb);
      hipLaunchKernelGGL(ykk::k_permute_planes, dim3(sig_chunks(ballot_rows), wgroups), dim3(ykk::kBlock), 0, sb, N, e->d_perm.as<int>(),
                         e->planes_canon.as<u64>(), e->planes_ranked.as<u64>(), e->row_stride, ballot_rows, e->row_words, first_r);
      tm.end(sb, "k_permute_planes");
    } else if (res_on || spread_on) {
      launch_ballot_planes(sb, e->d_perm.as<int>(), "k_planes(ranked)");
    }
    if (use_run_decide) {
      tm.begin(sb);
      hipLaunchKernelGGL(ykk::k_run_decide, dim3((unsigned)((e->run_ranges + ykk::kWavesPerBlock - 1) / ykk::kWavesPerBlock)), dim3(ykk::kBlock), 0, sb, pr,
                         e->d_sweep_runs.as<ykk::SweepRun>(), e->d_run_ranges.as<ykk::RunRange>(), e->run_ranges, e->d_sweep_rows.as<ykk::SweepRow>(),
                         e->d_glin_r.as<unsigned>(), e->d_sorted.as<i64>(), e->d_sorted_off.as<int>(), e->d_perm.as<int>(), e->row_words, N, pin_on,
                         e->d_class_best.as<int>());
      tm.end(sb, "k_run_decide");
    }
    tm.begin(sb);
    const int n_decide = use_run_decide ? e->n_decide_list : e->C;
    if (n_decide == 0) {
    } else if (n_decide >= e->decide_groups_from) {
      const int per_block = ykk::kWavesPerBlock * ykk::kDecideGroups;
      hipLaunchKernelGGL(ykk::k_decide_groups, dim3((unsigned)((n_decide + per_block - 1) / per_block)), dim3(ykk::kBlock), 0, sb, ct, pr, n_decide,
                         e->row_words, e->d_perm.as<int>(), e->d_rank.as<int>(), pin_on, e->d_class_best.as<int>());
    } else {
      hipLaunchKernelGGL(ykk::k_decide, dim3((unsigned)((n_decide + ykk::kWavesPerBlock - 1) / ykk::kWavesPerBlock)), dim3(ykk::kBlock), 0, sb, ct,
                         pr, n_decide, e->row_words, e->d_perm.as<int>(), e->d_rank.as<int>(), pin_on, e->d_class_best.as<int>(), n_decide <= 4096 ? 1 : 0);
    }
    tm.end(sb, "k_decide");
  }
  const bool skip_combine = a->options & YKPRED_EVAL_SKIP_BITMAP;
  const bool dirty_only = a->options & YKPRED_EVAL_DIRTY_CLASSES;
  const int* class_dirty = nullptr;
  if (!skip_combine && dirty_only) {
    HIPCHK(e->d_class_dirty.ensure((size_t)std::max(e->C, 1) * sizeof(int)));
    hipLaunchKernelGGL(ykk::k_mark_dirty_classes, dim3((unsigned)((e->C + ykk::kBlock - 1) / ykk::kBlock)), dim3(ykk::kBlock), 0, st, e->C,
                       e->d_class_sig.as<int>(), e->d_sig_changed.as<int>(), e->d_class_dirty.as<int>(), e->d_class_count.as<int>());
    class_dirty = e->d_class_dirty.as<int>();
  }
  const bool small_chunks = (long)e->NC * e->wave_combine_below > (long)P;
  const bool counts_early = e->early_counts != 0 && !skip_combine && !dirty_only && e->n_classes_a > 0 && e->patch_chunks == 0 && !small_chunks && e->n_classes_b <= 16384;
  bool scattered = false;
  if (!skip_combine && !dirty_only && !counts_early) {
    if (zero_counts_beside) HIPCHK(hipStreamWaitEvent(st, e->ev_zero, 0));
    else HIPCHK(hipMemsetAsync(e->d_class_count.p, 0, (size_t)e->C * sizeof(int), st));
  }
  if (!skip_combine) {
    int tpg = ykk::kBlock;
    while (tpg > ykk::kWave && (tpg / 2) * 2 >= e->row_stride) tpg /= 2;
    const int seg = tpg * ykk::kCombineUnroll * 2;
    const bool listed = !dirty_only && e->patch_chunks == 0;
    const bool short_list = use_sweep && (fuse_on || e->fuse_count == 0);
    const int* chunk_list = listed ? (short_list ? e->d_chunk_list_b0 : e->d_chunk_list_b).as<int>() : nullptr;
    const int n_run = listed ? (short_list ? e->NCB0 : e->NCB) : e->NC;
    dim3 grid((unsigned)std::max(n_run, 1), (unsigned)((e->row_stride + seg - 1) / seg));
    hipStream_t sz = st;
    if (!dirty_only && e->n_classes_a > 0) {
      tm.begin(st);
      const int n_counted_b = counts_early ? e->n_classes_b : 0;
      hipLaunchKernelGGL(ykk::k_class_rows, dim3((unsigned)((e->n_classes_a + n_counted_b + ykk::kWavesPerBlock - 1) / ykk::kWavesPerBlock)), dim3(ykk::kBlock), 0, st,
                         ct, pc, e->d_class_list_a.as<int>(), e->n_classes_a, e->row_words, e->row_stride, pin_on, e->d_class_rows_a.as<u64>(),
                         e->d_class_count.as<int>(), (const int*)nullptr, e->d_class_list_b.as<int>(), n_counted_b);
      tm.end(st, "k_class_rows");
      if (counts_early && want_dec) {
        HIPCHK(hipEventRecord(e->ev_counts, st));
        HIPCHK(hipStreamWaitEvent(sb, e->ev_counts, 0));
        tm.begin(sb);
        hipLaunchKernelGGL(ykk::k_scatter, dim3((unsigned)((P + ykk::kBlock - 1) / ykk::kBlock)), dim3(ykk::kBlock), 0, sb, P,
                           e->d_pod_class.as<int>(), e->d_class_count.as<int>(), e->d_class_best.as<int>(), e->d_key.as<u64>(),
                           want_cnt ? (int*)e->last_counts : nullptr, (int*)e->last_decisions, want_keys ? (i64*)e->last_keys : nullptr);
        tm.end(sb, "k_scatter");
        scattered = true;
      }
      const size_t lds_bytes = (size_t)2 * ykk::kBandClasses * (size_t)e->row_stride * sizeof(u64);
      if (lds_bytes > 64 * 1024)
        HIPCHK(hipFuncSetAttribute((const void*)ykk::k_expand_bands, hipFuncAttributeMaxDynamicSharedMemorySize, (int)lds_bytes));
      tm.begin(st);
      hipLaunchKernelGGL(ykk::k_expand_bands, dim3((unsigned)ykk::kBandGroups), dim3(ykk::kBandBlock), lds_bytes, st, bitmap,
                         e->d_class_rows_a.as<u64>(), e->d_band_tab.as<ykk::BandEntry>(), e->n_bands, e->row_stride);
      if (e->n_fix_rows > 0 && !counts_early)
        hipLaunchKernelGGL(ykk::k_fix_rows, dim3((unsigned)e->n_fix_rows), dim3(ykk::kBlock), 0, st, bitmap, e->d_class_rows_a.as<u64>(),
                           e->d_fix_row.as<int>(), e->d_fix_slot.as<int>(), e->n_fix_rows, e->row_stride);
      tm.end(st, "k_expand_bands");
    }
    if (use_sweep && e->run_classes > 0) {
      ykk::WalkStage rstage{};
      rstage.n = (int)e->h_stage_rows.size();
      for (int k = 0; k < rstage.n; ++k) rstage.row[k] = e->h_stage_rows[(size_t)k];
      const int its = (e->row_stride + ykk::kWave - 1) / ykk::kWave;
      int segs = (its + ykk::kWalkMaxIt - 1) / ykk::kWalkMaxIt, nit = (its + segs - 1) / segs;
      while (nit > 1 && ykk::runs_lds_bytes(rstage.n, nit) > (size_t)e->max_lds_bytes) {
        ++segs;
        nit = (its + segs - 1) / segs;
      }
      const int n_long = segs - (nit * segs - its);
      const size_t lds = ykk::runs_lds_bytes(rstage.n, nit);
      const int per_cu = lds * 2 <= (size_t)e->max_lds_bytes ? 2 : 1;
      const int groups = std::max(1, std::min(per_cu * e->num_cus, (e->run_units + ykk::kRunsWaves - 1) / ykk::kRunsWaves));
      tm.begin(sz);
      auto launch_runs = [&](auto kernel) -> int {
        if (lds > 64 * 1024) HIPCHK(hipFuncSetAttribute((const void*)kernel, hipFuncAttributeMaxDynamicSharedMemorySize, (int)lds));
        hipLaunchKernelGGL(kernel, dim3((unsigned)groups, (unsigned)segs), dim3(ykk::kRunsThreads), lds, sz, pc, e->d_run_classes.as<ykk::RunClass>(),
                           e->d_sweep_runs.as<ykk::SweepRun>(), e->run_classes, e->d_run_units.as<int>(), e->run_units, bitmap, e->row_words,
                           e->row_stride, pin_on, e->d_class_count.as<int>(), n_long, rstage);
        return YKPRED_OK;
      };
      switch (nit) {
        case 1: TRY(launch_runs(ykk::k_class_runs<1>)); break;
        case 2: TRY(launch_runs(ykk::k_class_runs<2>)); break;
        case 3: TRY(launch_runs(ykk::k_class_runs<3>)); break;
        case 4: TRY(launch_runs(ykk::k_class_runs<4>)); break;
        case 5: TRY(launch_runs(ykk::k_class_runs<5>)); break;
        case 6: TRY(launch_runs(ykk::k_class_runs<6>)); break;
        default: TRY(launch_runs(ykk::k_class_runs<7>)); break;
      }
      tm.end(sz, "k_class_runs");
    }
    if (sweep_rows_on) {
      const int its = (e->row_stride + ykk::kWave - 1) / ykk::kWave;
      int segs = (its + ykk::kWalkMaxIt - 1) / ykk::kWalkMaxIt, nit = (its + segs - 1) / segs;
      while (nit > 1 && ykk::sweep_lds_bytes(nit) > (size_t)e->max_lds_bytes) {
        ++segs;
        nit = (its + segs - 1) / segs;
      }
      const int n_long = segs - (nit * segs - its);
      tm.begin(sz);
      for (int b = 0; b < e->n_big; ++b) {
        const int n_rows = e->sweep_rows[b];
        if (n_rows == 0) continue;
        const int n_units = e->sweep_units[b];
        const int groups = std::max(1, std::min(e->sweep_groups > 0 ? e->sweep_groups : e->num_cus, (n_units + ykk::kSweepWaves - 1) / ykk::kSweepWaves));
        auto launch_sweep = [&](auto kernel) -> int {
          const size_t lds = ykk::sweep_lds_bytes(nit);
          if (lds > 64 * 1024) HIPCHK(hipFuncSetAttribute((const void*)kernel, hipFuncAttributeMaxDynamicSharedMemorySize, (int)lds));
          hipLaunchKernelGGL(kernel, dim3((unsigned)groups, (unsigned)segs), dim3(ykk::kSweepThreads), lds, sz, pc,
                             e->d_ent_c.as<unsigned>() + (size_t)b * 65 * (size_t)e->row_words, e->d_rbits_c.as<u64>() + (size_t)b * ykk::kRankBits * (size_t)e->row_words,
                             e->d_sweep_rows.as<ykk::SweepRow>() + e->sweep_row_off[b], e->d_sweep_runs.as<ykk::SweepRun>(), n_rows,
                             e->d_sweep_units.as<int>() + e->sweep_unit_off[b], n_units, bitmap, e->row_words, e->row_stride, pin_on,
                             e->d_class_count.as<int>(), n_long);
          return YKPRED_OK;
        };
        switch (nit) {
          case 1: TRY(launch_sweep(ykk::k_sweep_rows<1>)); break;
          case 2: TRY(launch_sweep(ykk::k_sweep_rows<2>)); break;
          case 3: TRY(launch_sweep(ykk::k_sweep_rows<3>)); break;
          case 4: TRY(launch_sweep(ykk::k_sweep_rows<4>)); break;
          case 5: TRY(launch_sweep(ykk::k_sweep_rows<5>)); break;
          case 6: TRY(launch_sweep(ykk::k_sweep_rows<6>)); break;
          default: TRY(launch_sweep(ykk::k_sweep_rows<7>)); break;
        }
      }
      tm.end(sz, "k_sweep_rows");
    }
    if (fuse_on) {
      const int wpl = e->fuse_wpl >= 5 ? 5 : (e->fuse_wpl >= 2 ? 2 : (e->fuse_wpl == 1 ? 1 : (e->row_words > 384 ? 5 : (e->row_words > 192 ? 2 : 1))));
      const int gw = ykk::kFuseComputeWaves * ykk::kWave * wpl;
      const unsigned ygroups = (unsigned)((e->row_words + gw - 1) / gw);
      ykk::FuseSrc fsrc{e->planes_canon.as<u64>(), e->fuse_combos > 0 ? e->d_fuse_combo.as<u64>() : nullptr, {e->fam_res.base, e->fam_tol.base, e->fam_aff.base}};
      tm.begin(sz);
      auto launch_fused = [&](auto kernel, const ykk::FuseRec* recs, int n, u64* out, int* counts) {
        hipLaunchKernelGGL(kernel, dim3((unsigned)((n + ykk::kFuseRecsPerBlock - 1) / ykk::kFuseRecsPerBlock), ygroups), dim3(ykk::kBlock), 0, sz, recs, n, fsrc,
                           e->row_words, e->row_stride, out, counts);
      };
      auto launch_wide = [&](const ykk::FuseRec* recs, int n, u64* out, int* counts) {
        if (wpl == 5) launch_fused(ykk::k_fused_rows<5, 8>, recs, n, out, counts);
        else if (wpl == 2) launch_fused(ykk::k_fused_rows<2, 8>, recs, n, out, counts);
        else launch_fused(ykk::k_fused_rows<1, 8>, recs, n, out, counts);
      };
      if (e->fuse_combos > 0) {
        launch_wide(e->d_fuse_combo_rec.as<ykk::FuseRec>(), e->fuse_combos, e->d_fuse_combo.as<u64>(), nullptr);
        if (wpl == 5) launch_fused(ykk::k_fused_rows<5, 2>, e->d_fuse_rec.as<ykk::FuseRec>(), e->fuse_count, bitmap, e->d_class_count.as<int>());
        else if (wpl == 2) launch_fused(ykk::k_fused_rows<2, 2>, e->d_fuse_rec.as<ykk::FuseRec>(), e->fuse_count, bitmap, e->d_class_count.as<int>());
        else launch_fused(ykk::k_fused_rows<1, 2>, e->d_fuse_rec.as<ykk::FuseRec>(), e->fuse_count, bitmap, e->d_class_count.as<int>());
      } else {
        launch_wide(e->d_fuse_rec.as<ykk::FuseRec>(), e->fuse_count, bitmap, e->d_class_count.as<int>());
      }
      tm.end(sz, "k_fused_rows");
    }
    tm.begin(sz);
    int walk_nit = 0, walk_segs = 0, walk_long = 0;
    ykk::WalkStage wstage{};
    wstage.n = (int)e->h_stage_rows.size();
    for (int k = 0; k < wstage.n; ++k) wstage.row[k] = e->h_stage_rows[(size_t)k];
    bool slices = small_chunks && e->combine_slices != 0 && pc.n_big > 0 && pc.res != nullptr && !(use_sweep && e->sweep_min_run <= 1 && listed);
    if (slices) {
      const int its = (e->row_stride + ykk::kWave - 1) / ykk::kWave;
      const size_t lds_cap = std::min((size_t)e->max_lds_bytes, (size_t)80 * 1024);
      walk_segs = (its + ykk::kWalkMaxIt - 1) / ykk::kWalkMaxIt;
      walk_nit = (its + walk_segs - 1) / walk_segs;
      while (walk_nit > 1 && ykk::walk_lds_bytes(pc.n_big, wstage.n, walk_nit) > lds_cap) {
        ++walk_segs;
        walk_nit = (its + walk_segs - 1) / walk_segs;
      }
      walk_long = walk_segs - (walk_nit * walk_segs - its);
      slices = ykk::walk_lds_bytes(pc.n_big, wstage.n, walk_nit) <= (size_t)e->max_lds_bytes && its * ykk::kWave <= e->idx_stride;
    }
    if (slices) {
      HIPCHK(e->d_slice_desc.ensure((size_t)std::max(e->NC, 1) * sizeof(ykk::SliceDesc)));
      HIPCHK(e->d_slice_general.ensure(sizeof(int)));
      HIPCHK(hipMemsetAsync(e->d_slice_general.p, 0, sizeof(int), sz));
      hipLaunchKernelGGL(ykk::k_slice_desc, dim3((unsigned)((e->NC + ykk::kBlock - 1) / ykk::kBlock)), dim3(ykk::kBlock), 0, sz, ct, pc, e->NC, class_dirty,
                         pin_on, e->d_slice_desc.as<ykk::SliceDesc>(), e->d_slice_general.as<int>(), wstage);
      tm.end(sz, "k_slice_desc");
      tm.begin(sz);
      const int per_group = ykk::kRowsWaves * ykk::kWalkChunksPerWave;
      const unsigned gx = (unsigned)((e->NC + per_group - 1) / per_group);
      auto launch_walk = [&](auto kernel, int nit, int segs, int w_base) -> int {
        const size_t lds = ykk::walk_lds_bytes(pc.n_big, wstage.n, nit);
        if (lds > 64 * 1024) HIPCHK(hipFuncSetAttribute((const void*)kernel, hipFuncAttributeMaxDynamicSharedMemorySize, (int)lds));
        hipLaunchKernelGGL(kernel, dim3(gx, (unsigned)segs), dim3(ykk::kRowsThreads), lds, sz, pc, e->d_slice_desc.as<ykk::SliceDesc>(), bitmap,
                           e->row_words, e->row_stride, pin_on, e->d_class_count.as<int>(), e->NC, w_base, wstage);
        return YKPRED_OK;
      };
      auto launch_segments = [&](int nit, int segs, int w_base, bool tail) -> int {
        if (segs <= 0) return YKPRED_OK;
        switch (nit * 2 + (tail ? 1 : 0)) {
#define YK_WALK_CASE(N)                                                         \
  case (N) * 2: return launch_walk(ykk::k_walk_rows<(N), false>, nit, segs, w_base); \
  case (N) * 2 + 1: return launch_walk(ykk::k_walk_rows<(N), true>, nit, segs, w_base);
          YK_WALK_CASE(1) YK_WALK_CASE(2) YK_WALK_CASE(3) YK_WALK_CASE(4) YK_WALK_CASE(5) YK_WALK_CASE(6) YK_WALK_CASE(7)
#undef YK_WALK_CASE
        }
        return fail(e, YKPRED_E_INVALID, "k_walk_rows: no kernel for " + std::to_string(nit) + " word groups per lane");
      };
      {
        const int n_short = walk_segs - walk_long, nit_last = n_short > 0 ? walk_nit - 1 : walk_nit;
        const int long_plain = n_short > 0 ? walk_long : walk_long - 1, short_plain = n_short > 0 ? n_short - 1 : 0;
        TRY(launch_segments(walk_nit, long_plain, 0, false));
        TRY(launch_segments(walk_nit - 1, short_plain, walk_long * walk_nit * ykk::kWave, false));
        TRY(launch_segments(nit_last, 1, (long_plain * walk_nit + short_plain * (walk_nit - 1)) * ykk::kWave, true));
      }
      tm.end(sz, "k_walk_rows");
      tm.begin(sz);
      hipLaunchKernelGGL(ykk::k_combine_wave, dim3((unsigned)((e->NC + ykk::kWavesPerBlock - 1) / ykk::kWavesPerBlock)), dim3(ykk::kBlock), 0, sz, ct,
                         pc, bitmap, e->row_words, e->row_stride, pin_on, e->d_class_count.as<int>(), e->NC, class_dirty,
                         e->d_slice_desc.as<ykk::SliceDesc>(), e->d_slice_general.as<int>(), (const int*)nullptr);
    } else if (counts_early) {
      const ykk::FixRows fix{e->d_class_rows_a.as<u64>(), e->d_fix_row.as<int>(), e->d_fix_slot.as<int>(), e->n_fix_rows};
      const int blocks = n_run + e->n_fix_rows;
      if (blocks > 0)
        hipLaunchKernelGGL(ykk::k_combine, dim3((unsigned)blocks, grid.y), dim3(ykk::kBlock), (size_t)e->combine_lds_bytes, sz, ct, pc, bitmap, e->row_words,
                           e->row_stride, pin_on, (int*)nullptr, tpg, class_dirty, chunk_list, fix, n_run);
    } else if (n_run == 0) {
    } else if (small_chunks) {
      const dim3 wgrid((unsigned)((std::max(n_run, 1) + ykk::kWavesPerBlock - 1) / ykk::kWavesPerBlock));
      hipLaunchKernelGGL(ykk::k_combine_wave, wgrid, dim3(ykk::kBlock), 0, sz, ct, pc, bitmap, e->row_words, e->row_stride, pin_on,
                         e->d_class_count.as<int>(), n_run, class_dirty, (const ykk::SliceDesc*)nullptr, (const int*)nullptr, chunk_list);
    } else {
      hipLaunchKernelGGL(ykk::k_combine, grid, dim3(ykk::kBlock), (size_t)e->combine_lds_bytes, sz, ct, pc, bitmap, e->row_words, e->row_stride,
                         pin_on, e->d_class_count.as<int>(), tpg, class_dirty, chunk_list, ykk::FixRows{nullptr, nullptr, nullptr, 0}, n_run);
    }
    tm.end(sz, dirty_only ? "k_combine(dirty classes)" : "k_combine");
  }
  if (want_dec) {
    HIPCHK(hipEventRecord(e->ev_join, sb));
    HIPCHK(hipStreamWaitEvent(st, e->ev_join, 0));
  }
  if ((want_dec || want_cnt) && !scattered) {
    tm.begin(st);
    hipLaunchKernelGGL(ykk::k_scatter, dim3((unsigned)((P + ykk::kBlock - 1) / ykk::kBlock)), dim3(ykk::kBlock), 0, st, P,
                       e->d_pod_class.as<int>(), e->d_class_count.as<int>(), e->d_class_best.as<int>(), e->d_key.as<u64>(),
                       want_cnt ? (int*)e->last_counts : nullptr, want_dec ? (int*)e->last_decisions : nullptr,
                       want_keys ? (i64*)e->last_keys : nullptr);
    tm.end(st, "k_scatter");
  }
  HIPCHK(hipGetLastError());
  return YKPRED_OK;
  };
  const bool graphable = !tm.on && !e->graph_disabled && !(e->comm && e->comm_world > 1) && !(a->options & (YKPRED_EVAL_DIRECT | YKPRED_EVAL_SPREAD_COUNT_ONLY));
  hipGraphExec_t exec = nullptr;
  if (graphable) {
    ykpred_engine::GraphKey key{e->tables_version, pre, filt, a->options, (void*)bitmap, e->last_counts, e->last_decisions, e->last_keys};
    for (size_t i = 0; i < e->graphs.size();) {
      if (e->graphs[i].first.version != e->tables_version) {
        (void)hipGraphExecDestroy(e->graphs[i].second);
        e->graphs.erase(e->graphs.begin() + (long)i);
      } else {
        if (e->graphs[i].first == key) exec = e->graphs[i].second;
        ++i;
      }
    }
    bool repeated = false;
    for (size_t i = 0; i < e->seen.size();) {
      if (e->seen[i].version != e->tables_version) {
        e->seen.erase(e->seen.begin() + (long)i);
        continue;
      }
      repeated = repeated || e->seen[i] == key;
      ++i;
    }
    if (!repeated && e->seen.size() < 8) e->seen.push_back(key);
    if (!exec && repeated) {
      hipGraph_t g = nullptr;
      int crc = YKPRED_E_DEVICE;
      if (hipStreamBeginCapture(st, hipStreamCaptureModeThreadLocal) == hipSuccess) {
        crc = enqueue();
        if (hipStreamEndCapture(st, &g) != hipSuccess) crc = YKPRED_E_DEVICE;
      }
      if (crc == YKPRED_OK && g && hipGraphInstantiate(&exec, g, nullptr, nullptr, 0) == hipSuccess) {
        if (e->graphs.size() >= 8) {
          (void)hipGraphExecDestroy(e->graphs.front().second);
          e->graphs.erase(e->graphs.begin());
        }
        e->graphs.emplace_back(key, exec);
      } else {
        exec = nullptr;
        e->graph_disabled = true;
        (void)hipGetLastError();
      }
      if (g) (void)hipGraphDestroy(g);
    }
  }
  if (exec) {
    HIPCHK(hipGraphLaunch(exec, st));
  } else {
    int rc = enqueue();
    if (rc < 0) return rc;
    if (rc == 1) {
      tm.done(st);
      return YKPRED_OK;
    }
  }
  tm.done(st);
  if (e->ev_eval_done) (void)hipEventRecord(e->ev_eval_done, st);
  e->bitmap_epoch = e->nodes_epoch;
  e->last_pre = pre;
  e->last_filt = filt;
  e->last_eval_valid = true;
  if (!(a->options & (YKPRED_EVAL_SKIP_BITMAP | YKPRED_EVAL_DIRTY_CLASSES))) e->n_full_evals++;
  if (!(a->options & (YKPRED_EVAL_SKIP_BITMAP | YKPRED_EVAL_DIRTY_CLASSES))) std::fill(e->h_row_stale.begin(), e->h_row_stale.end(), 0);
  if (want_dec) {
    e->win_partial = use_run_decide_pass;
    e->rank_valid = true;
    e->ranked_specs_version = e->specs_version;
    e->ranked_nodes_epoch = e->nodes_epoch;
    e->ranked_pre = pre;
    e->ranked_filt = filt;
    e->ranked_has_first = e->decide_skip;
  }
  e->last_has_keys = want_keys;
  return YKPRED_OK;
}

int32_t ykpred_eval_nodes(ykpred_engine_t* e, const ykpred_eval_args_t* a, int32_t num_nodes, const int32_t* node_index) {
  YK_SERIALISE(e);
  Range roctx_range("ykpred:eval_nodes");
  if (e) e->n_node_patches++;
  if (!e || !a || num_nodes < 0 || (num_nodes > 0 && !node_index)) return fail(e, YKPRED_E_INVALID, "eval_nodes: bad argument");
  HIPCHK(hipSetDevice(e->cfg.device));
  hipStream_t st = a->stream ? (hipStream_t)a->stream : e->own_stream;
  const unsigned pre = a->prefilter_plugins, filt = a->filter_plugins;
  u64* bitmap = a->bitmap ? (u64*)a->bitmap : e->d_bitmap.as<u64>();
  if (e->classes_dirty || !e->last_eval_valid || pre != e->last_pre || filt != e->last_filt || (void*)bitmap != e->last_bitmap)
    return fail(e, YKPRED_E_STATE, "eval_nodes: no matching previous ykpred_eval (tables, plugin lists or bitmap changed)");
  const bool topo = (pre & filt & (YKPRED_PLUGIN_POD_TOPOLOGY_SPREAD | YKPRED_PLUGIN_INTER_POD_AFFINITY)) && e->fam_spread.D > 0;
  const bool sharded = e->comm && e->comm_world > 1;
  const bool hist_ready = a->options & YKPRED_EVAL_SPREAD_COUNTS_READY, hist_only = a->options & YKPRED_EVAL_SPREAD_COUNT_ONLY;
  const bool topo_pass = topo && e->P > 0 && (num_nodes > 0 || sharded || hist_ready || hist_only);
  if (topo && e->spread_dirty) return fail(e, YKPRED_E_STATE, "eval_nodes: topology tables changed — run ykpred_eval");
  for (int i = 0; i < num_nodes; ++i)
    if (node_index[i] < 0 || node_index[i] >= e->N) return fail(e, YKPRED_E_INVALID, "eval_nodes: node index out of range");
  Timer tm{e, (a->options & YKPRED_EVAL_PROFILE) != 0};
  tm.start(st);
  const bool want_cnt = a->options & YKPRED_OUT_COUNTS;
  const bool want_keys = a->options & YKPRED_OUT_DECISION_KEYS;
  const bool want_dec = (a->options & YKPRED_OUT_DECISIONS) || want_keys;
  if (topo_pass) {
    const size_t cells = (size_t)std::max<int64_t>(e->spread_cells, 1) * sizeof(int), mins = (size_t)std::max(e->spread_constraints, 1) * sizeof(int);
    HIPCHK(e->d_sp_cnt_prev.ensure(cells));
    HIPCHK(e->d_sp_present_prev.ensure(cells));
    HIPCHK(e->d_sp_min_prev.ensure(mins));
    HIPCHK(e->d_sig_changed.ensure((size_t)e->fam_spread.D * sizeof(int)));
    if (e->hist_epoch == 0) return fail(e, YKPRED_E_STATE, "eval_nodes: no topology histograms from a previous ykpred_eval");
    if (!hist_ready) {
      HIPCHK(hipMemcpyAsync(e->d_sp_cnt_prev.p, e->d_sp_cnt.p, cells, hipMemcpyDeviceToDevice, st));
      HIPCHK(hipMemcpyAsync(e->d_sp_present_prev.p, e->d_sp_present.p, cells, hipMemcpyDeviceToDevice, st));
      HIPCHK(hipMemcpyAsync(e->d_sp_min_prev.p, e->d_sp_min.p, mins, hipMemcpyDeviceToDevice, st));
      TRY(run_spread_prefilter(e, st, &tm, true, false));
    }
    if (hist_only) {
      tm.done(st);
      return YKPRED_OK;
    }
    if (!hist_ready) TRY(allreduce_spread(e, st));
    TRY(run_spread_prefilter(e, st, &tm, false, true));
    e->hist_epoch = e->nodes_epoch;
    tm.begin(st);
    hipLaunchKernelGGL(ykk::k_spread_diff, dim3((unsigned)e->fam_spread.D), dim3(ykk::kWave), 0, st, spread_sigs(e), e->d_sp_cnt_prev.as<int>(),
                       e->d_sp_present_prev.as<int>(), e->d_sp_min_prev.as<int>(), e->d_sig_changed.as<int>());
    tm.end(st, "k_spread_diff");
  }
  if (num_nodes > 0 && e->P > 0) {
    std::vector<int32_t> nodes(node_index, node_index + num_nodes);
    std::sort(nodes.begin(), nodes.end());
    nodes.erase(std::unique(nodes.begin(), nodes.end()), nodes.end());
    HIPCHK(e->d_class_word.ensure((size_t)std::max(e->C, 1) * ykk::kMaxColGroups * sizeof(u64)));
    ykk::NodeTable nt = node_table(e);
    ykk::SpecTable stbl = spec_table(e);
    size_t i = 0;
    while (i < nodes.size()) {
      ykk::ColumnGroups cg{};
      int filled = 0;
      while (i < nodes.size() && cg.n_groups < ykk::kMaxColGroups && filled < 64) {
        int w = nodes[i] >> 6;
        cg.word[cg.n_groups] = w;
        cg.first[cg.n_groups] = filled;
        while (i < nodes.size() && (nodes[i] >> 6) == w && filled < 64) cg.nodes[filled++] = nodes[i++];
        cg.n_groups++;
        if (i < nodes.size() && (nodes[i] >> 6) == w) break;
      }
      cg.first[cg.n_groups] = filled;
      tm.begin(st);
      hipLaunchKernelGGL(ykk::k_column_class, dim3((unsigned)((e->C + ykk::kBlock - 1) / ykk::kBlock)), dim3(ykk::kBlock), 0, st, nt, stbl, cg,
                         e->C, e->d_class_first.as<int>(), e->d_class_pin.as<int>(), e->d_pod_spec.as<int>(), e->d_pod_row.as<int>(), pre, filt, bitmap,
                         e->row_stride, e->d_class_word.as<u64>(), e->d_class_count.as<int>());
      tm.end(st, "k_column_class");
      tm.begin(st);
      hipLaunchKernelGGL(ykk::k_column_patch, dim3((unsigned)((e->P + ykk::kBlock - 1) / ykk::kBlock)), dim3(ykk::kBlock), 0, st, cg, e->P,
                         e->d_pod_class.as<int>(), e->d_pod_row.as<int>(), e->d_class_word.as<u64>(), e->d_class_count.as<int>(), bitmap, e->row_stride,
                         want_cnt ? (int*)(a->counts ? a->counts : e->last_counts) : nullptr);
      tm.end(st, "k_column_patch");
    }
  }
  HIPCHK(hipGetLastError());
  tm.done(st);
  if (e->ev_eval_done) (void)hipEventRecord(e->ev_eval_done, st);
  e->bitmap_epoch = e->nodes_epoch;
  if (topo_pass) {
    ykpred_eval_args_t b = *a;
    b.bitmap = bitmap;
    b.options = (a->options & ~(uint32_t)YKPRED_EVAL_SPREAD_COUNT_ONLY) | YKPRED_OUT_BITMAP | YKPRED_EVAL_DIRTY_CLASSES | YKPRED_EVAL_SPREAD_COUNTS_READY;
    int rc = ykpred_eval(e, &b);
    if (rc != YKPRED_OK) return rc;
  } else if (want_dec) {
    ykpred_eval_args_t b = *a;
    b.options = (a->options & ~(uint32_t)YKPRED_OUT_BITMAP) | YKPRED_EVAL_SKIP_BITMAP;
    int rc = ykpred_eval(e, &b);
    if (rc != YKPRED_OK) return rc;
  }
  return YKPRED_OK;
}

int32_t ykpred_update_pods(ykpred_engine_t* e, int32_t num_pods_after, int32_t count, const int32_t* rows, const int32_t* spec_index,
                           const int32_t* node_name_index) {
  YK_SERIALISE(e);
  Range roctx_range("ykpred:update_asks");
  if (e) e->n_uploads++;
  if (e) e->tables_version++;
  if (e) e->layout_version++;
  if (e) e->ask_epoch++;
  if (!e || num_pods_after < 0 || count < 0 || (count > 0 && (!rows || !spec_index || !node_name_index)))
    return fail(e, YKPRED_E_INVALID, "update_pods: bad argument");
  if (!e->pods_set || !e->specs_set) return fail(e, YKPRED_E_STATE, "update_pods: ykpred_set_specs and ykpred_set_pods come first");
  HIPCHK(hipSetDevice(e->cfg.device));
  const int oldP = e->P, newP = num_pods_after;
  {
    std::vector<uint8_t> listed((size_t)std::max(newP - oldP, 0), 0);
    std::vector<int32_t> sorted(rows, rows + count);
    std::sort(sorted.begin(), sorted.end());
    if (std::adjacent_find(sorted.begin(), sorted.end()) != sorted.end()) return fail(e, YKPRED_E_INVALID, "update_pods: a row is listed twice");
    for (int i = 0; i < count; ++i) {
      if (rows[i] < 0 || rows[i] >= newP) return fail(e, YKPRED_E_INVALID, "update_pods: row out of range");
      if (spec_index[i] < 0 || spec_index[i] >= e->S) return fail(e, YKPRED_E_INVALID, "update_pods: pod references a spec that was not uploaded");
      if (node_name_index[i] < YKPRED_UNKNOWN_NODE_NAME || (e->nodes_set && node_name_index[i] >= e->N))
        return fail(e, YKPRED_E_INVALID, "update_pods: node_name_index out of range");
      if (rows[i] >= oldP) listed[(size_t)(rows[i] - oldP)] = 1;
    }
    for (uint8_t l : listed)
      if (!l) return fail(e, YKPRED_E_INVALID, "update_pods: every appended row must be listed");
  }
  hipStream_t st = e->own_stream;
  if (!e->classes_dirty) {
    const int64_t after = (int64_t)e->rows_total + count;
    const bool caller_owned = e->last_bitmap && e->last_bitmap != e->d_bitmap.p;
    if ((e->row_capacity && after > (int64_t)e->row_capacity) || (caller_owned && e->last_eval_valid && after > e->last_bitmap_rows)) {
      e->classes_dirty = true;
      e->last_eval_valid = false;
    }
  }
  if (e->classes_dirty) {
    e->h_pod_spec.resize((size_t)newP);
    e->h_pod_pin.resize((size_t)newP);
    for (int i = 0; i < count; ++i) {
      e->h_pod_spec[(size_t)rows[i]] = spec_index[i];
// ... 146 lines not shown
    ykk::TablePtrs tp{};
    tp.t[T_POD_SPEC] = e->d_pod_spec.as<int>();
    tp.t[T_POD_PIN] = e->d_pod_pin.as<int>();
    tp.t[T_POD_CLASS] = e->d_pod_class.as<int>();
    tp.t[T_MEMBERS] = e->d_members.as<int>();
    tp.t[T_CH_CLASS] = e->d_chunk_class.as<int>();
    tp.t[T_CH_BEGIN] = e->d_chunk_begin.as<int>();
    tp.t[T_CH_LEN] = e->d_chunk_len.as<int>();
    tp.t[T_CH_FIRST] = e->d_chunk_first.as<int>();
    tp.t[T_CLASS_SIG] = e->d_class_sig.as<int>();
    tp.t[T_CLASS_PIN] = e->d_class_pin.as<int>();
    tp.t[T_CLASS_FIRST] = e->d_class_first.as<int>();
    tp.t[T_POD_ROW] = e->d_pod_row.as<int>();
    tp.t[T_CH_ZONE] = e->d_chunk_zone.as<int>();
    TRY(upload(e, e->d_patches, patches.data(), patches.size(), st));
    hipLaunchKernelGGL(ykk::k_apply_patches, dim3((unsigned)((patches.size() + ykk::kBlock - 1) / ykk::kBlock)), dim3(ykk::kBlock), 0, st, tp,
                       (int)patches.size(), e->d_patches.as<ykk::TablePatch>());
    HIPCHK(hipGetLastError());
    HIPCHK(hipStreamSynchronize(st));
  }
  if (e->patch_chunks > std::max(4096, (e->NC - e->patch_chunks) / 4) || e->rows_total > newP + std::max(8192, newP / 4)) e->classes_dirty = true;
  return YKPRED_OK;
}

int32_t ykpred_eval_pods(ykpred_engine_t* e, const ykpred_eval_args_t* a, int32_t num_rows, const int32_t* rows) {
  YK_SERIALISE(e);
  Range roctx_range("ykpred:eval_pods");
  if (e) e->n_row_patches++;
  if (!e || !a || num_rows < 0 || (num_rows > 0 && !rows)) return fail(e, YKPRED_E_INVALID, "eval_pods: bad argument");
  HIPCHK(hipSetDevice(e->cfg.device));
  hipStream_t st = a->stream ? (hipStream_t)a->stream : e->own_stream;
  const unsigned pre = a->prefilter_plugins, filt = a->filter_plugins;
  const bool own_bitmap = !a->bitmap && e->last_bitmap == e->d_bitmap.p;
  if (e->classes_dirty || !e->last_eval_valid || pre != e->last_pre || filt != e->last_filt || (a->bitmap && a->bitmap != e->last_bitmap) ||
      (!a->bitmap && !own_bitmap))
    return fail(e, YKPRED_E_STATE, "eval_pods: no matching previous ykpred_eval (tables, plugin lists or bitmap changed)");
  const bool want_cnt = a->options & YKPRED_OUT_COUNTS;
  const bool want_keys = a->options & YKPRED_OUT_DECISION_KEYS;
  const bool want_dec = (a->options & YKPRED_OUT_DECISIONS) || want_keys;
  if (want_dec && !e->rank_valid) return fail(e, YKPRED_E_STATE, "eval_pods: the bin-pack order is stale — run ykpred_eval with decisions");
  for (int i = 0; i < num_rows; ++i)
    if (rows[i] < 0 || rows[i] >= e->P) return fail(e, YKPRED_E_INVALID, "eval_pods: row out of range");
  TRY(grow_owned_outputs(e));
  Timer tm{e, (a->options & YKPRED_EVAL_PROFILE) != 0};
  tm.start(st);
  if (num_rows > 0 && e->N > 0) {
    u64* bitmap = (u64*)e->last_bitmap;
    TRY(upload(e, e->d_rows, rows, (size_t)num_rows, st));
    HIPCHK(e->d_row_count.ensure((size_t)num_rows * sizeof(int)));
    HIPCHK(e->d_row_best.ensure((size_t)num_rows * sizeof(int)));
    HIPCHK(hipMemsetAsync(e->d_row_count.p, 0, (size_t)num_rows * sizeof(int), st));
    HIPCHK(hipMemsetAsync(e->d_row_best.p, 0x7f, (size_t)num_rows * sizeof(int), st));
    ykk::NodeTable nt = node_table(e);
    ykk::SpecTable stbl = spec_table(e);
    const unsigned wgroups = (unsigned)((e->row_stride + ykk::kWavesPerBlock - 1) / ykk::kWavesPerBlock);
    tm.begin(st);
    hipLaunchKernelGGL(ykk::k_rows, dim3((unsigned)num_rows, wgroups), dim3(ykk::kBlock), 0, st, nt, stbl, num_rows, e->d_rows.as<int>(),
                       e->d_pod_spec.as<int>(), e->d_pod_pin.as<int>(), e->d_pod_row.as<int>(), pre, filt, bitmap, e->row_words, e->row_stride,
                       want_dec ? e->d_rank.as<int>() : nullptr, e->d_row_count.as<int>(), e->d_row_best.as<int>());
    tm.end(st, "k_rows");
    tm.begin(st);
    hipLaunchKernelGGL(ykk::k_rows_finish, dim3((unsigned)((num_rows + ykk::kBlock - 1) / ykk::kBlock)), dim3(ykk::kBlock), 0, st, num_rows,
                       e->d_rows.as<int>(), e->d_pod_class.as<int>(), e->d_row_count.as<int>(), e->d_row_best.as<int>(),
                       want_dec ? e->d_perm.as<int>() : nullptr, e->d_key.as<u64>(), e->d_class_count.as<int>(), e->d_class_best.as<int>(),
                       want_cnt ? (int*)(a->counts ? a->counts : e->last_counts) : nullptr,
                       (a->options & YKPRED_OUT_DECISIONS) ? (int*)(a->decisions ? a->decisions : e->last_decisions) : nullptr,
                       want_keys ? (i64*)(a->decision_keys ? a->decision_keys : e->last_keys) : nullptr);
    tm.end(st, "k_rows_finish");
    HIPCHK(hipGetLastError());
    HIPCHK(hipStreamSynchronize(st));
    for (int i = 0; i < num_rows; ++i)
      if ((size_t)rows[i] < e->h_row_stale.size()) e->h_row_stale[(size_t)rows[i]] = 0;
  }
  tm.done(st);
  if (e->ev_eval_done) (void)hipEventRecord(e->ev_eval_done, st);
  return YKPRED_OK;
}

int32_t ykpred_set_spec_effects(ykpred_engine_t* e, const ykpred_spec_effects_t* fx) {
  YK_SERIALISE(e);
  if (!e) return fail(e, YKPRED_E_INVALID, "set_spec_effects: bad argument");
  if (!fx) {
    e->fx_version = 0;
    return YKPRED_OK;
  }
  if (!e->specs_set || fx->count != e->S) return fail(e, YKPRED_E_STATE, "set_spec_effects: the effects must describe the uploaded spec table (same count)");
  HIPCHK(hipSetDevice(e->cfg.device));
  hipStream_t st = e->own_stream;
  const size_t S = (size_t)e->S;
  e->fx_version = 0;
  e->fx_contrib = false;
  e->fx_ports = false;
  e->h_fx_off.clear();
  e->h_fx_cls.clear();
  e->h_fx_cnt.clear();
  if (fx->contrib_off) {
    const int total = fx->contrib_off[S];
    if (fx->contrib_off[0] != 0 || total < 0 || (total > 0 && (!fx->contrib_class || !fx->contrib_count)))
      return fail(e, YKPRED_E_INVALID, "set_spec_effects: malformed contribution rows");
    for (size_t i = 0; i < S; ++i)
      if (fx->contrib_off[i + 1] < fx->contrib_off[i]) return fail(e, YKPRED_E_INVALID, "set_spec_effects: contrib_off must not decrease");
    for (int k = 0; k < total; ++k)
      if (fx->contrib_class[k] < 0 || fx->contrib_class[k] >= e->KS || fx->contrib_count[k] <= 0)
        return fail(e, YKPRED_E_INVALID, "set_spec_effects: contribution outside the selector classes of the node table, or not positive");
    TRY(upload(e, e->d_fx_off, fx->contrib_off, S + 1, st));
    e->h_fx_off.assign(fx->contrib_off, fx->contrib_off + S + 1);
    if (total > 0) e->h_fx_cls.assign(fx->contrib_class, fx->contrib_class + total);
    if (total > 0) e->h_fx_cnt.assign(fx->contrib_count, fx->contrib_count + total);
    TRY(upload(e, e->d_fx_cls, fx->contrib_class, (size_t)std::max(total, 1), st));
    TRY(upload(e, e->d_fx_cnt, fx->contrib_count, (size_t)std::max(total, 1), st));
    e->fx_contrib = total > 0;
  }
  e->h_fx_occupies.assign(S, 0);
  if (fx->occupied_ports && e->KP > 0) {
    TRY(upload(e, e->d_fx_occ, fx->occupied_ports, S * (size_t)e->KP, st));
    for (size_t i = 0; i < S * (size_t)e->KP; ++i)
      if (fx->occupied_ports[i] != 0) {
        e->fx_ports = true;
        e->h_fx_occupies[i / (size_t)e->KP] = 1;
      }
  }
  HIPCHK(hipStreamSynchronize(st));
  e->fx_version = e->specs_version;
  return YKPRED_OK;
}

static double host_node_score(const i64 (&total)[2], const i64 (&used)[2]) {
  double sum = 0.0, wsum = 0.0;
  for (int r = 0; r < 2; ++r) {
    if (total[r] <= 0) continue;
    const double avail = (double)(total[r] - used[r]);
    const double share = 1.0 - avail / (double)total[r];
    sum = sum + share;
    wsum = wsum + 1.0;
  }
  if (wsum == 0.0) return 1.0;
  return 1.0 - sum / wsum;
}
static u64 host_sortable_key(double v) {
  u64 b;
  memcpy(&b, &v, sizeof b);
  return (b >> 63) ? ~b : (b | 0x8000000000000000ull);
}
constexpr size_t kShardBatchMax = 256;
constexpr size_t kBatchBytesMax = kShardBatchMax * ykk::kPropK * sizeof(ykk::RoundProposal) +
                                  kShardBatchMax * ((kShardBatchMax * ykk::kPropK + 63) / 64) * sizeof(u64);
static_assert(kShardBatchMax * ykk::kPropK * 2 <= (size_t)ykk::kDistinctSlots, "k_round_distinct's table holds a batch's proposals");

int32_t ykpred_allocate_round(ykpred_engine_t* e, uint32_t pre, uint32_t filt, int32_t n_asks, const int32_t* asks, int32_t* out_nodes) {
  YK_SERIALISE(e);
  Range roctx_range("ykpred:allocate_round");
  if (!e || n_asks < 0 || (n_asks > 0 && (!asks || !out_nodes))) return fail(e, YKPRED_E_INVALID, "allocate_round: bad argument");
  const bool sharded = e->comm && e->comm_world > 1;
  const bool stale = e->classes_dirty || !e->last_eval_valid || !e->rank_valid || e->bitmap_epoch != e->nodes_epoch || pre != e->last_pre || filt != e->last_filt ||
                     e->ranked_pre != pre || e->ranked_filt != filt || e->ranked_nodes_epoch != e->nodes_epoch || e->ranked_specs_version != e->specs_version;
  const bool fx_current = e->fx_version == e->specs_version;
  const bool topo_on = (pre & filt & (YKPRED_PLUGIN_POD_TOPOLOGY_SPREAD | YKPRED_PLUGIN_INTER_POD_AFFINITY)) && e->fam_spread.D > 0;
  const bool ports_on = (pre & filt & YKPRED_PLUGIN_NODE_PORTS) && e->KP > 0;
  bool port_asks = false;
  for (int i = 0; i < n_asks && ports_on && !port_asks; ++i) {
    if (asks[i] < 0 || asks[i] >= e->P) break;
    const size_t sp = (size_t)e->h_pod_spec[(size_t)asks[i]];
    for (int k = 0; k < e->KP; ++k) port_asks = port_asks || e->h_wanted[sp * (size_t)e->KP + (size_t)k] != 0;
  }
  if (sharded) {
    struct Agree {
      int32_t rc, n;
      u64 hash;
      int64_t cells;
      u64 topo;
    };
    Agree mine{stale ? YKPRED_E_STATE : YKPRED_OK, n_asks, 0x9e3779b97f4a7c15ull, topo_on ? e->spread_cells : 0, topo_on ? topology_digest(e) : 0};
    if (mine.rc == YKPRED_OK && (topo_on || port_asks) && !fx_current) mine.rc = YKPRED_E_UNSUPPORTED;
    for (int i = 0; i < n_asks; ++i) {
      mine.hash = (mine.hash ^ (u64)(uint32_t)asks[i]) * 0x100000001b3ull;
      if (asks[i] < 0 || asks[i] >= e->P) mine.rc = YKPRED_E_INVALID;
      else if ((size_t)asks[i] < e->h_row_stale.size() && e->h_row_stale[(size_t)asks[i]]) mine.rc = YKPRED_E_STATE;
    }
    HIPCHK(hipSetDevice(e->cfg.device));
    const int W = e->comm_world;
    HIPCHK(e->d_agree.ensure((size_t)(W + 1) * sizeof(Agree)));
    Agree* d = e->d_agree.as<Agree>();
    HIPCHK(hipMemcpyAsync(d + W, &mine, sizeof(Agree), hipMemcpyHostToDevice, e->own_stream));
    NCCLCHK(rccl()->AllGather(d + W, d, sizeof(Agree), ncclInt8, e->comm, e->own_stream));
    std::vector<Agree> all((size_t)W);
    HIPCHK(hipMemcpyAsync(all.data(), d, (size_t)W * sizeof(Agree), hipMemcpyDeviceToHost, e->own_stream));
    HIPCHK(hipStreamSynchronize(e->own_stream));
    for (int g = 0; g < W; ++g) {
      if (all[(size_t)g].rc != YKPRED_OK)
        return fail(e, all[(size_t)g].rc, "allocate_round (sharded): rank " + std::to_string(g) + " cannot run the round (no current evaluation with decisions, "
                                          "an ask patched and not re-evaluated, an ask index out of range, or topology constraints / host ports "
                                          "without the specs' effects uploaded): no rank runs it");
    }
    for (int g = 0; g < W; ++g)
      if (all[(size_t)g].cells != all[0].cells || all[(size_t)g].topo != all[0].topo)
        return fail(e, YKPRED_E_INVALID, "allocate_round (sharded): rank " + std::to_string(g) + "'s topology histograms are laid out differently from rank 0's (" +
                                             std::to_string(all[(size_t)g].cells) + " against " + std::to_string(all[0].cells) +
                                             " cells, or other dictionaries behind the ids): the shards do not share the topology-domain dictionaries — no rank runs the round");
    for (int g = 0; g < W; ++g) {
      if (all[(size_t)g].n != all[0].n || all[(size_t)g].hash != all[0].hash)
        return fail(e, YKPRED_E_INVALID, "allocate_round (sharded): rank " + std::to_string(g) + " was handed a different ask list: every rank passes the same asks in the same order");
    }
  }
  if (stale)
    return fail(e, YKPRED_E_STATE, "allocate_round: no current evaluation WITH decisions of these plugin lists (run ykpred_eval with YKPRED_OUT_DECISIONS)");
  if (topo_on && !fx_current)
    return fail(e, YKPRED_E_UNSUPPORTED, "allocate_round: topology constraints are active (an assumed pod's labels move the histograms of later asks) and the "
                                         "specs' effects are not uploaded (ykpred_set_spec_effects): decide ask by ask");
  for (int i = 0; i < n_asks; ++i) {
    if (asks[i] < 0 || asks[i] >= e->P) return fail(e, YKPRED_E_INVALID, "allocate_round: ask index out of range");
    if ((size_t)asks[i] < e->h_row_stale.size() && e->h_row_stale[(size_t)asks[i]])
      return fail(e, YKPRED_E_STATE, "allocate_round: an ask of the round was patched and not re-evaluated yet");
  }
  if (port_asks && !fx_current)
    return fail(e, YKPRED_E_UNSUPPORTED, "allocate_round: an ask of the round requests a host port (an assumed pod's ports change later answers) and the specs' "
                                         "effects are not uploaded (ykpred_set_spec_effects): decide ask by ask");
  if (n_asks == 0) return YKPRED_OK;
  bool batched = sharded || e->round_batched > 0;
  if (!sharded && e->round_batched < 0 && !topo_on && n_asks >= 512) {
    int changes = 1;
    for (int i = 1; i < n_asks; ++i) changes += e->h_pod_spec[(size_t)asks[i]] != e->h_pod_spec[(size_t)asks[i - 1]] ? 1 : 0;
    batched = (int64_t)changes * 4 >= (int64_t)n_asks;
  }
  HIPCHK(hipSetDevice(e->cfg.device));
  hipStream_t st = e->own_stream;
  if (e->ev_eval_done) HIPCHK(hipStreamWaitEvent(st, e->ev_eval_done, 0));
  if (topo_on) TRY(ensure_histograms(e, st));
  const bool live_ports = port_asks || (ports_on && e->fx_ports && fx_current);
  const size_t N = (size_t)std::max(e->N, 1), R = (size_t)e->R, C = (size_t)std::max(e->C, 1), RW = (size_t)std::max(e->row_words, 1);
  const size_t G = topo_on ? (size_t)std::max(e->spread_constraints, 1) : 0, cells = topo_on ? (size_t)std::max<int64_t>(e->spread_cells, 1) : 0;
  size_t off = 0;
  auto take = [&](size_t bytes) {
    const size_t at = off;
    off += (bytes + 7) / 8 * 8;
    return at;
  };
  const size_t cap = N, cap64 = (N + 63) / 64, Wc = (size_t)std::min(e->W, ykk::kMaxW), KP1 = (size_t)std::max(e->KP, 1), KD1 = (size_t)std::max(e->KD, 1);
  const bool keep_failed = C * cap64 * sizeof(u64) <= ((size_t)256 << 20);
  const size_t o_req = take(R * N * sizeof(i64)), o_bits = take(RW * sizeof(u64)),
               o_ports = take(live_ports ? (size_t)e->KP * N * sizeof(u64) : 0), o_cnt = take(N * sizeof(int)), o_cur = take(C * sizeof(int)),
               o_slot = take(N * sizeof(int)), o_mnode = take(cap * sizeof(int)), o_mtie = take(cap * sizeof(int)), o_mkey = take(cap * sizeof(u64)),
               o_mfree = take(R * cap * sizeof(i64)), o_mroom = take(cap * sizeof(int)), o_mports = take(KP1 * cap * sizeof(u64)),
               o_mtaint = take((size_t)std::max(e->KT, 1) * cap * sizeof(u64)), o_mlabel = take(std::max<size_t>(Wc, 1) * cap * sizeof(u64)), o_mdom = take(KD1 * cap * sizeof(int)),
               o_mflags = take(cap * sizeof(unsigned)), o_dead = take(cap64 * sizeof(u64)), o_failed = take(keep_failed ? C * cap64 * sizeof(u64) : 0),
               o_asks = take((size_t)n_asks * sizeof(int)), o_out = take((size_t)n_asks * sizeof(int)),
               o_nm = take(sizeof(int)), o_hist = take(cells * sizeof(int)), o_minv = take(G * sizeof(int)), o_mn = take(G * sizeof(int)),
               o_at = take(G * sizeof(int)), o_nd = take(G * sizeof(int)), o_prof = take(16 * sizeof(i64)),
               o_rkey = take(N * sizeof(u64)), o_rtie = take(N * sizeof(int)), o_cdesc = take(C * ykk::kDescWords * sizeof(u64)),
               o_prop = take(batched ? kBatchBytesMax : 0),
               o_allprop = take(sharded ? (size_t)e->comm_world * kBatchBytesMax : 0),
               o_list = take(batched ? (kShardBatchMax * ykk::kPropK + 2) * sizeof(int) : 0),
               o_forced = take(batched ? (size_t)n_asks * sizeof(int) : 0), o_runlen = take(batched ? (size_t)n_asks * sizeof(int) : 0),
               o_deltas = take(batched ? kShardBatchMax * sizeof(ykk::RoundNodeDelta) : 0),
               o_delta = take((sharded && topo_on) ? (size_t)n_asks * ykk::kDeltaStride * sizeof(int) : 0),
               o_alldelta = take((sharded && topo_on) ? (size_t)e->comm_world * kShardBatchMax * ykk::kDeltaStride * sizeof(int) : 0);
  HIPCHK(e->d_round.ensure(off));
  char* base = (char*)e->d_round.p;
  HIPCHK(hipMemcpyAsync(base + o_req, e->d_req.p, R * (size_t)e->N * sizeof(i64), hipMemcpyDeviceToDevice, st));
  HIPCHK(hipMemcpyAsync(base + o_cnt, e->d_count.p, (size_t)e->N * sizeof(int), hipMemcpyDeviceToDevice, st));
  if (live_ports) HIPCHK(hipMemcpyAsync(base + o_ports, e->d_ports.p, (size_t)e->KP * (size_t)e->N * sizeof(u64), hipMemcpyDeviceToDevice, st));
  HIPCHK(hipMemsetAsync(base + o_bits, 0, RW * sizeof(u64), st));
  HIPCHK(hipMemsetAsync(base + o_cur, 0xff, C * sizeof(int), st));
  HIPCHK(hipMemsetAsync(base + o_slot, 0xff, N * sizeof(int), st));
  HIPCHK(hipMemsetAsync(base + o_dead, 0, cap64 * sizeof(u64), st));
  if (keep_failed) HIPCHK(hipMemsetAsync(base + o_failed, 0, C * cap64 * sizeof(u64), st));
  HIPCHK(hipMemsetAsync(base + o_nm, 0, sizeof(int), st));
  if (sharded && topo_on) HIPCHK(hipMemsetAsync(base + o_delta, 0, (size_t)n_asks * ykk::kDeltaStride * sizeof(int), st));
  HIPCHK(hipMemsetAsync(base + o_prof, 0, 16 * sizeof(i64), st));
  HIPCHK(hipMemcpyAsync(base + o_asks, asks, (size_t)n_asks * sizeof(int), hipMemcpyHostToDevice, st));
  ykk::NodeTable nt = node_table(e);
  nt.req = (const i64*)(base + o_req);
  nt.count = (const int*)(base + o_cnt);
  if (live_ports) nt.ports = (const u64*)(base + o_ports);
  ykk::ClassTable ct{e->d_class_sig.as<int>(), e->d_class_pin.as<int>(), e->d_chunk_class.as<int>(), e->d_chunk_begin.as<int>(),
                     e->d_chunk_len.as<int>(), e->d_chunk_first.as<int>(), e->d_members.as<int>(), e->d_chunk_zone.as<int>(), 0, nullptr};
  const bool spread_err = ((filt & YKPRED_PLUGIN_POD_TOPOLOGY_SPREAD) && !(pre & YKPRED_PLUGIN_POD_TOPOLOGY_SPREAD)) ||
                          ((filt & YKPRED_PLUGIN_INTER_POD_AFFINITY) && !(pre & YKPRED_PLUGIN_INTER_POD_AFFINITY)) ||
                          ((filt & YKPRED_PLUGIN_NODE_PORTS) && !(pre & YKPRED_PLUGIN_NODE_PORTS));
  ykk::RoundArgs ra{};
  ra.asks = (const int*)(base + o_asks);
  ra.pod_spec = e->d_pod_spec.as<int>();
  ra.pod_pin = e->d_pod_pin.as<int>();
  ra.pod_class = e->d_pod_class.as<int>();
  ra.perm = e->d_perm.as<int>();
  ra.rank = e->d_rank.as<int>();
  ra.key0 = e->d_key.as<u64>();
  ra.name_rank = e->has_name_rank ? e->d_name_rank.as<int>() : nullptr;
  ra.rkey = (const u64*)(base + o_rkey);
  ra.rtie = (const int*)(base + o_rtie);
  if (e->N > 0)
    hipLaunchKernelGGL(ykk::k_round_ranked_keys, dim3((unsigned)((e->N + ykk::kBlock - 1) / ykk::kBlock)), dim3(ykk::kBlock), 0, st, e->N, ra.perm, ra.key0,
                       ra.name_rank, (u64*)(base + o_rkey), (int*)(base + o_rtie));
  ra.pre = pre;
  ra.filt = filt;
  ra.row_words = e->row_words;
  ra.all_fail = spread_err ? 1 : 0;
  ra.req = (i64*)(base + o_req);
  ra.count = (int*)(base + o_cnt);
  ra.ports = live_ports ? (u64*)(base + o_ports) : nullptr;
  ra.moved_bits = (u64*)(base + o_bits);
  ra.cursor = (int*)(base + o_cur);
  ra.n_moved = (int*)(base + o_nm);
  ra.cap = (int)cap;
  ra.cap64 = (int)cap64;
  ra.slot_of = (int*)(base + o_slot);
  ra.m_node = (int*)(base + o_mnode);
  ra.m_tie = (int*)(base + o_mtie);
  ra.m_key = (u64*)(base + o_mkey);
  ra.m_free = (i64*)(base + o_mfree);
  ra.m_room = (int*)(base + o_mroom);
  ra.m_ports = (u64*)(base + o_mports);
  ra.m_taint = (u64*)(base + o_mtaint);
  ra.m_label = (u64*)(base + o_mlabel);
  ra.m_dom = (int*)(base + o_mdom);
  ra.m_flags = (unsigned*)(base + o_mflags);
  ra.dead = (u64*)(base + o_dead);
  ra.failed = keep_failed ? (u64*)(base + o_failed) : nullptr;
  ra.out = (int*)(base + o_out);
  ra.prof = e->round_prof ? (i64*)(base + o_prof) : nullptr;
  ra.mode = ykk::kRoundDecide;
  ra.node_offset = e->node_offset;
  if (fx_current) {
    ra.fx.off = e->fx_contrib ? e->d_fx_off.as<int>() : nullptr;
    ra.fx.cls = e->d_fx_cls.as<int>();
    ra.fx.cnt = e->d_fx_cnt.as<int>();
    ra.fx.occupied = (live_ports && e->fx_ports) ? e->d_fx_occ.as<u64>() : nullptr;
  }
  ykk::SpecTable stbl = spec_table(e);
  if (topo_on) {
    HIPCHK(hipMemcpyAsync(base + o_hist, e->d_sp_cnt.p, (size_t)e->spread_cells * sizeof(int), hipMemcpyDeviceToDevice, st));
    HIPCHK(hipMemcpyAsync(base + o_minv, e->d_sp_min.p, (size_t)e->spread_constraints * sizeof(int), hipMemcpyDeviceToDevice, st));
    stbl.spread.cnt = (int*)(base + o_hist);
    stbl.spread.minv = (int*)(base + o_minv);
    std::vector<int32_t> sig_of;
    for (size_t d = 0; d < e->spread_sig.size(); ++d) sig_of.insert(sig_of.end(), e->spread_sig[d].size(), (int32_t)d);
    sig_of.resize(G, 0);
    TRY(upload(e, e->d_sp_sig_of, sig_of.data(), sig_of.size(), st));
    HIPCHK(hipStreamSynchronize(st));
    ra.topo_on = 1;
    ra.G = e->spread_constraints;
    ra.sig_aff = ykk::AffSigs{e->d_sig_aff_flags.as<unsigned>(), e->d_sig_aff_off.as<int>(), e->d_sig_aff_terms.as<u64>(), e->d_sig_pre_off.as<int>(),
                              e->d_sig_pre_terms.as<u64>()};
    ra.sig_tol = e->d_sig_tol.as<u64>();
    ra.sig_of = e->d_sp_sig_of.as<int>();
    ra.mn = (int*)(base + o_mn);
    ra.at_min = (int*)(base + o_at);
    ra.nd = (int*)(base + o_nd);
    if (e->spread_constraints > 0)
      hipLaunchKernelGGL(ykk::k_round_topo_init, dim3((unsigned)e->spread_constraints), dim3(ykk::kWave), 0, st, stbl.spread, e->spread_constraints,
                         (int*)(base + o_mn), (int*)(base + o_at), (int*)(base + o_nd));
  }
  TRY(complete_windows(e, st));
  const ykk::Planes pr = ranked_planes_of(e, pre, filt, false, e->ranked_has_first);
  ra.cdesc = (const u64*)(base + o_cdesc);
  if (e->C > 0)
    hipLaunchKernelGGL(ykk::k_round_class_desc, dim3((unsigned)((e->C + ykk::kBlock - 1) / ykk::kBlock)), dim3(ykk::kBlock), 0, st, ct, pr, e->C,
                       (u64*)(base + o_cdesc));
  if (batched) {
    Rccl* r = sharded ? rccl() : nullptr;
    const int W = sharded ? e->comm_world : 1, me = sharded ? e->comm_rank : 0;
    constexpr int K = ykk::kPropK;
    auto cw_of = [](int b) { return (b * K + 63) / 64; };
    auto bytes_of = [&](int b) { return (size_t)b * K * sizeof(ykk::RoundProposal) + (size_t)b * (size_t)cw_of(b) * sizeof(u64); };
    char* d_send = base + o_prop;
    char* d_all = base + o_allprop;
    int* d_list = (int*)(base + o_list);
    int* d_nlist = d_list + kShardBatchMax * K;
    int* d_forced = (int*)(base + o_forced);
    int* d_runlen = (int*)(base + o_runlen);
    ykk::RoundNodeDelta* d_deltas = (ykk::RoundNodeDelta*)(base + o_deltas);
    std::vector<ykk::RoundNodeDelta> deltas;
    std::vector<int32_t> run_len;
    if (e->h_round_pinned_bytes < (size_t)W * kBatchBytesMax) {
      if (e->h_round_pinned) (void)hipHostFree(e->h_round_pinned);
      e->h_round_pinned = nullptr;
      e->h_round_pinned_bytes = 0;
      if (hipHostMalloc(&e->h_round_pinned, (size_t)W * kBatchBytesMax, hipHostMallocDefault) == hipSuccess) e->h_round_pinned_bytes = (size_t)W * kBatchBytesMax;
      else (void)hipGetLastError();
    }
// ... 2379 lines not shown
```

### yunikorn-k8shim_amd/csrc/engine/kernels.hip.h

```cpp
#pragma once
#include <hip/hip_runtime.h>
#include <stdint.h>

#include <type_traits>

namespace ykk {

typedef unsigned long long u64;
typedef long long i64;

constexpr int kMaxR = 8;
constexpr int kMaxKT = 4;
constexpr int kMaxW = 8;
constexpr int kMaxWTotal = 32;
constexpr int kMaxKD = 8;
constexpr int kMaxKP = 4;

constexpr int kWave = 64;
constexpr int kBlock = 256;
constexpr int kWavesPerBlock = kBlock / kWave;
constexpr int kSigsPerBlock = 16;
constexpr int kSigsPerBlockMany = 64;
constexpr int kManySigs = 4096;
__host__ __device__ inline int sigs_per_block(int D) { return D > kManySigs ? kSigsPerBlockMany : kSigsPerBlock; }
// ... 1970 lines not shown
  }
  __syncthreads();
  const int p = b * 4096 + tid * 16;
  const unsigned urow_b = (unsigned)row_b;
  const unsigned dcol = (unsigned)(kWin % row_b);
  unsigned ucol = (unsigned)(p % row_b);
  for (int band = 0; band < n_bands; ++band) {
    const BandEntry cur = tab[(size_t)band * kBandGroups + b];
    const int s0 = cur.first_step, s1 = s0 + cur.steps;
    const char* lds = (const char*)(band_lds + (size_t)(band & 1) * kBandClasses * row_stride);
    unsigned kb[kBandClasses - 1];
#pragma unroll
    for (int i = 0; i < kBandClasses - 1; ++i)
      kb[i] = cur.xb[i] == 0x7fffffff ? 0xffffffffu : (((unsigned)cur.xb[i] << 8) | (unsigned)(cur.sb[i] - s0));
    char* win_base = (char*)out + (long)s0 * kWin;
    auto run_band = [&](auto ncls_tag) {
      constexpr int kN = decltype(ncls_tag)::value;
      constexpr int kU = 4;
      for (int s = s0; s < s1; s += kU) {
        u64x2 v[kU];
        bool live[kU];
#pragma unroll
        for (int u = 0; u < kU; ++u) {
          unsigned off = ucol;
          live[u] = p >= (int)ucol;
          if (kN > 1) {
            const unsigned key = ((unsigned)(p - (int)ucol) << 8) | (unsigned)(s + u - s0);
#pragma unroll
            for (int i = 0; i < kN - 1; ++i) off += key >= kb[i] ? urow_b : 0u;
          }
          v[u] = *(const u64x2*)(lds + off);
          const unsigned t = ucol + dcol;
          ucol = min(t, t - urow_b);
        }
#pragma unroll
        for (int u = 0; u < kU; ++u) {
          if (live[u]) *(u64x2*)(win_base + p) = v[u];
          win_base += kWin;
        }
      }
    };
    if (cur.n <= 1)
      run_band(std::integral_constant<int, 1>{});
    else if (cur.n == 2)
      run_band(std::integral_constant<int, 2>{});
    else if (cur.n == 3)
      run_band(std::integral_constant<int, 3>{});
    else
      run_band(std::integral_constant<int, kBandClasses>{});
    __syncthreads();
  }
}
__global__ __launch_bounds__(kBlock) void k_fix_rows(u64* __restrict__ out, const u64* __restrict__ class_rows, const int* __restrict__ rows,
                                                     const int* __restrict__ slots, int n, int row_stride) {
  typedef u64 u64x2 __attribute__((ext_vector_type(2)));
  if ((int)blockIdx.x >= n) return;
  const u64* src = class_rows + (size_t)slots[blockIdx.x] * row_stride;
  u64* dst = out + (size_t)rows[blockIdx.x] * row_stride;
  for (int w = threadIdx.x * 2; w < row_stride; w += 2 * kBlock) *(u64x2*)(dst + w) = *(const u64x2*)(src + w);
}

__global__ __launch_bounds__(kBlock) void k_decide(ClassTable ct, Planes ranked, int n_classes, int row_words, const int* __restrict__ perm,
                                                   const int* __restrict__ rank, int pin_enabled, int* __restrict__ class_best, int eager) {
  int cls = blockIdx.x * kWavesPerBlock + threadIdx.x / kWave;
  if (cls >= n_classes) return;
  if (ct.decide_list) cls = ct.decide_list[cls];
  const int lane = threadIdx.x % kWave;
  const int sr = ct.sig[cls * 4 + 0], st = ct.sig[cls * 4 + 1], sa = ct.sig[cls * 4 + 2], ss = ct.sig[cls * 4 + 3];
  const bool all_fail = pin_enabled & 2;
  const int pin = (pin_enabled & 1) ? ct.pin[cls] : -1;
  int best = -1;
  const ClassRows cr = class_rows(ranked, sr, st, sa, ss);
  if (pin == -2 || all_fail) {
    best = -1;
  } else if (pin >= 0) {
    int pos = rank[pin];
    u64 x = class_word(cr, pos >> 6);
    best = ((x >> (pos & 63)) & 1ull) ? pin : -1;
  } else {
    for (int base = cr.start & ~(kWave - 1); base < row_words; base += kWave) {
      int w = base + lane;
      u64 x = w < row_words ? ~0ull : 0ull;
      if (eager) {
        const int ws = w < row_words ? w : 0;
        u64 y = ~0ull;
#pragma unroll
        for (int i = 0; i < kMaxClassRows; ++i)
          if (i < cr.n) y &= cr.row[i][ws];
        if (cr.ni) y &= class_idx_word(cr, ws);
        x &= y;
      } else {
        if (cr.ni && x) x &= class_idx_word(cr, w);
#pragma unroll
        for (int i = kMaxClassRows - 1; i >= 0; --i)
          if (i < cr.n && x) x &= cr.row[i][w];
      }
      u64 any = __ballot(x != 0);
      if (any) {
        int first_lane = __ffsll((long long)any) - 1;
        u64 xw = __shfl(x, first_lane, kWave);
        int pos = (base + first_lane) * kWave + (__ffsll((long long)xw) - 1);
        best = perm[pos];
        break;
      }
    }
  }
  if (lane == 0) class_best[cls] = best;
}

constexpr int kDecideGroups = 4, kDecideLanes = kWave / kDecideGroups;
__global__ __launch_bounds__(kBlock) void k_decide_groups(ClassTable ct, Planes ranked, int n_classes, int row_words, const int* __restrict__ perm,
                                                          const int* __restrict__ rank, int pin_enabled, int* __restrict__ class_best) {
  const int wave = blockIdx.x * kWavesPerBlock + threadIdx.x / kWave;
  const int lane = threadIdx.x % kWave, g = lane / kDecideLanes, l = lane % kDecideLanes;
  const int cls_raw = wave * kDecideGroups + g;
  const bool live = cls_raw < n_classes;
  const int cls = ct.decide_list ? ct.decide_list[live ? cls_raw : n_classes - 1] : (live ? cls_raw : n_classes - 1);
  const bool all_fail = pin_enabled & 2;
  const int sr = ct.sig[cls * 4 + 0], st = ct.sig[cls * 4 + 1], sa = ct.sig[cls * 4 + 2], ss = ct.sig[cls * 4 + 3];
  const int pin = (pin_enabled & 1) ? ct.pin[cls] : -1;
  const ClassRows cr = class_rows(ranked, sr, st, sa, ss);
  auto word_at = [&](int w) {
    u64 x = w < row_words ? ~0ull : 0ull;
    if (cr.ni && x) x &= class_idx_word(cr, w);
#pragma unroll
    for (int i = kMaxClassRows - 1; i >= 0; --i)
      if (i < cr.n && x) x &= cr.row[i][w];
    return x;
  };
  int best = -1;
  bool done = !live || pin == -2 || all_fail;
  if (!done && pin >= 0) {
    const int pos = rank[pin];
    const u64 x = word_at(pos >> 6);
    best = ((x >> (pos & 63)) & 1ull) ? pin : -1;
    done = true;
  }
  const int w0 = cr.start >= row_words ? row_words : (cr.start & ~(kDecideLanes - 1));
  for (int t = 0;; ++t) {
    const int base = w0 + t * kDecideLanes;
    if (base >= row_words) done = true;
    if (__ballot(!done) == 0) break;
    const u64 x = done ? 0ull : word_at(base + l);
    const u64 any = __ballot(x != 0);
    const unsigned mine = (unsigned)((any >> (g * kDecideLanes)) & ((1u << kDecideLanes) - 1u));
    const int first = mine ? __ffs((int)mine) - 1 : 0;
    const u64 xw = __shfl(x, g * kDecideLanes + first, kWave);
    if (!done && mine) {
      best = perm[(base + first) * kWave + (__ffsll((long long)xw) - 1)];
      done = true;
    }
  }
  if (live && l == 0) class_best[cls] = best;
}

constexpr int kRunDecideRows = 512;
struct RunRange {
  int run, big, begin, count;
};
__global__ __launch_bounds__(kBlock) void k_run_decide(Planes ranked, const SweepRun* __restrict__ runs, const RunRange* __restrict__ ranges, int n_ranges,
                                                       const SweepRow* __restrict__ rows, const unsigned* __restrict__ glin, const i64* __restrict__ sorted,
                                                       const int* __restrict__ sorted_off, const int* __restrict__ perm, int n_words, int n_nodes,
                                                       int pin_enabled, int* __restrict__ class_best) {
  const int k = __builtin_amdgcn_readfirstlane((int)(blockIdx.x * kWavesPerBlock + threadIdx.x / kWave));
  if (k >= n_ranges) return;
  const int lane = threadIdx.x % kWave;
  const RunRange rr = ranges[k];
  const SweepRun run = runs[rr.run];
  const int4* vrow = (const int4*)(rows + rr.begin);
  const bool all_fail = pin_enabled & 2;
  const u64* p0 = ranked.res;
  const u64* pp = ranked.res ? ranked.res + (size_t)run.prow * ranked.stride : nullptr;
  const u64* pt = (ranked.tol && run.st >= 0) ? ranked.tol + (size_t)run.st * ranked.stride : p0;
  const u64* pa = (ranked.aff && run.sa >= 0) ? ranked.aff + (size_t)run.sa * ranked.stride : p0;
  const u64* ps = (ranked.spread && run.ss >= 0) ? ranked.spread + (size_t)run.ss * ranked.stride : p0;
  const unsigned* gl = glin + (size_t)rr.big * n_words * 64;
  const unsigned* gmax = glin + (size_t)ranked.n_big * n_words * 64 + (size_t)rr.big * n_words;
  int i = 0, ib = 0;
  int4 d = vrow[min(lane, rr.count - 1)];
  int start = 0;
  if (ranked.pfx) {
    const i64 v = sorted[sorted_off[rr.big] + __builtin_amdgcn_readfirstlane(d.z)];
    const i64* px = ranked.pfx + (size_t)rr.big * n_words;
    int lo = 0, hi = n_words;
    while (lo < hi) {
      const int mid = (lo + hi) >> 1;
      if (px[mid] < v) lo = mid + 1; else hi = mid;
    }
    start = lo;
  }
  unsigned cur = (unsigned)__builtin_amdgcn_readfirstlane(d.z);
  if (!all_fail && p0)
    for (int wb = start & ~(kWave - 1); wb < n_words && i < rr.count; wb += kWave) {
      const int w = wb + lane;
      const u64 S = w < n_words ? (p0[w] & pp[w] & pt[w] & pa[w] & ps[w]) : 0ull;
      const unsigned wmx = w < n_words ? gmax[w] : 0u;
      u64 done_mask = 0;
      for (;;) {
        const u64 todo = __ballot(S != 0 && wmx > cur) & ~done_mask;
        if (!todo || i >= rr.count) break;
        const int wk = __ffsll((long long)todo) - 1;
        done_mask |= (2ull << wk) - 1;
        const u64 Sk = (u64)readlane_i64((i64)S, wk);
        const unsigned g = gl[(size_t)(wb + wk) * 64 + lane];
        u64 m = __ballot(((Sk >> lane) & 1ull) && g > cur);
        while (m && i < rr.count) {
          const int f = __ffsll((long long)m) - 1;
          cur = (unsigned)__builtin_amdgcn_readlane((int)g, f);
          const int pos = (wb + wk) * kWave + f;
          const int node = pos < n_nodes ? perm[pos] : -1;
          for (;;) {
            const int idx = ib + lane;
            const bool take = idx >= i && idx < rr.count && (unsigned)d.z < cur;
            if (take) class_best[d.x] = node;
            i += __popcll(__ballot(take));
            if (i < ib + kWave || i >= rr.count) break;
            ib += kWave;
            d = vrow[min(ib + lane, rr.count - 1)];
          }
          m = __ballot(((Sk >> lane) & 1ull) && g > cur);
        }
      }
    }
  while (i < rr.count) {
    const int idx = ib + lane;
    if (idx >= i && idx < rr.count) class_best[d.x] = -1;
    i = min(ib + kWave, rr.count);
    if (i < rr.count) {
      ib += kWave;
      d = vrow[min(ib + lane, rr.count - 1)];
    }
  }
}
__global__ __launch_bounds__(kBlock) void k_scatter(int n_pods, const int* __restrict__ pod_class, const int* __restrict__ class_count,
                                                    const int* __restrict__ class_best, const u64* __restrict__ node_key,
                                                    int* __restrict__ counts, int* __restrict__ decisions, i64* __restrict__ keys) {
  int p = blockIdx.x * kBlock + threadIdx.x;
  if (p >= n_pods) return;
  int c = pod_class[p];
  if (counts) counts[p] = class_count[c];
  int b = (decisions || keys) ? class_best[c] : -1;
  if (decisions) decisions[p] = b;
  if (keys) keys[p] = b >= 0 ? (i64)(node_key[b] ^ 0x8000000000000000ull) : 0x7fffffffffffffffll;
}

struct SpecTable {
  int R, KT, W;
  const i64* req;
  const u64* tol;
  const unsigned* flags;
  AffSigs aff;
  int KP;
  const u64* wanted_ports;
  const int* spread_sig;
  SpreadSigs spread;
};

struct NodeRegs {
  i64 fr[kMaxR];
  u64 tn[kMaxKT];
  u64 lb[kMaxW];
  const u64* lb_more;
  size_t lb_stride;
  u64 pt[kMaxKP];
  int dom[kMaxKD];
  bool slots_ok, unsched;
};
__device__ __forceinline__ void load_node(const NodeTable& t, int n, NodeRegs* r) {
#pragma unroll
  for (int i = 0; i < kMaxR; ++i) r->fr[i] = (i < t.R && n >= 0) ? t.alloc[(size_t)i * t.n + n] - t.req[(size_t)i * t.n + n] : 0;
#pragma unroll
  for (int i = 0; i < kMaxKT; ++i) r->tn[i] = (i < t.KT && n >= 0) ? t.taints[(size_t)i * t.n + n] : 0;
#pragma unroll
  for (int i = 0; i < kMaxW; ++i) r->lb[i] = (i < t.W && n >= 0) ? t.labels[(size_t)i * t.n + n] : 0;
  r->lb_more = (t.W > kMaxW && n >= 0) ? t.labels + (size_t)kMaxW * t.n + n : nullptr;
  r->lb_stride = (size_t)t.n;
#pragma unroll
  for (int i = 0; i < kMaxKP; ++i) r->pt[i] = (i < t.KP && n >= 0) ? t.ports[(size_t)i * t.n + n] : 0;
#pragma unroll
  for (int i = 0; i < kMaxKD; ++i) r->dom[i] = (i < t.KD && n >= 0) ? t.domain[(size_t)i * t.n + n] : -1;
  r->slots_ok = n >= 0 && (i64)t.count[n] + 1 <= (i64)t.allowed[n];
  r->unsched = n >= 0 && (t.flags[n] & kNodeUnschedulable);
}

template <bool LIVE = false>
__device__ __forceinline__ bool eval_pair(const SpecTable& s, int spec, int pin, int node, const NodeRegs& nr, unsigned pre_mask,
                                          unsigned filt_mask, int* code, unsigned* reason) {
  unsigned f = s.flags[spec];
  *code = 0;
  *reason = 0;
  if (f & kSpecUnsupported) {
    *code = 255;
    return false;
  }
  if ((pre_mask & kPlugAffinity) && !(f & kSpecAffSkip)) {
    if (f & kSpecPreReject) {
      *code = 0;
      *reason = 1u << 2;
      return false;
    }
    if ((f & kSpecPreNames) && !dnf_match(s.aff.pre_terms, s.aff.pre_off[spec], s.aff.pre_off[spec + 1], nr.lb, s.W, nr.lb_more, nr.lb_stride)) {
      *code = 4;
      *reason = 1u << 1;
      return false;
    }
  }
// ... 2544 lines not shown
```

Before: 42480 billion evals/s.

## Decide pod classes from canonical rows in perm order, skip ranked plane build

Adds a k_decide_rows kernel. Each block stages a class's canonical feasibility row in LDS, then walks the node permutation in rank order and stops at the first feasible node. When this path is eligible, the evaluation no longer builds the permuted (ranked) dictionary and ballot planes or fills first_r. allocate_round now rebuilds ranked planes lazily through a new build_ranked_planes helper, and the plane-launch lambdas are moved into a PlaneJobs struct. The trade is permuted random LDS lookups per class, plus a serial scan when the first feasible node ranks late, in exchange for skipping full ranked-plane construction.

Result: faster. 43400 billion evals/s, median of 6 (+2.1%).

```diff
diff --git a/yunikorn-k8shim_amd/csrc/engine/engine.hip b/yunikorn-k8shim_amd/csrc/engine/engine.hip
--- a/yunikorn-k8shim_amd/csrc/engine/engine.hip
+++ b/yunikorn-k8shim_amd/csrc/engine/engine.hip
@@ -302,6 +302,7 @@
   bool bands_enabled = true;
   int band_steps = 0;
   int band_steps_now = 128;
+  int decide_rows = 1;
   int round_batched = -1;
   int round_node_assume = 1;
   int round_prof = 0;
@@ -331,6 +332,7 @@
   uint64_t specs_version = 1, ranked_specs_version = 0, ranked_nodes_epoch = 0;
   unsigned ranked_pre = 0, ranked_filt = 0;
   bool ranked_has_first = false;
+  uint64_t canon_specs_version = 0, canon_nodes_epoch = 0;
   DevBuf d_round;
   DevBuf d_fx_off, d_fx_cls, d_fx_cnt, d_fx_occ, d_sp_sig_of;
   uint64_t fx_version = 0;
@@ -411,6 +413,7 @@
     e->spread_dirty = true;
     e->hist_epoch = 0;
     e->ranked_nodes_epoch = 0;
+    e->canon_nodes_epoch = 0;
     e->tables_version++;
   }
   return code;
@@ -1150,6 +1153,7 @@
       e->tables_version++;
       HIPCHK(b->ensure(need));
       HIPCHK(hipMemsetAsync(b->p, 0, need, st));
+      e->ranked_nodes_epoch = e->canon_nodes_epoch = 0;
     }
   }
   e->plane_rows_alloc = rows;
@@ -1159,6 +1163,7 @@
       e->tables_version++;
       HIPCHK(b->ensure(base_need));
       HIPCHK(hipMemsetAsync(b->p, 0, base_need, st));
+      e->ranked_nodes_epoch = e->canon_nodes_epoch = 0;
     }
   }
   return YKPRED_OK;
@@ -1453,6 +1458,206 @@
   return pr;
 }
 
+struct PlaneJobs {
+  ykpred_engine* e;
+  Timer* tm;
+  unsigned pre, filt;
+  ykk::NodeTable nt;
+  bool res_on, aff_on, pts_en, ipa_en, spread_on;
+  int fit_error;
+  unsigned wgroups;
+  ykk::AffSigs as;
+  ykk::PlaneOut o_res, o_tol, o_aff, o_spread;
+  int* first_r = nullptr;
+  bool use_run_decide = false, use_sweep = false, sweep_rows_on = false;
+
+  PlaneJobs(ykpred_engine* e_, Timer* tm_, unsigned pre_, unsigned filt_) : e(e_), tm(tm_), pre(pre_), filt(filt_), nt(node_table(e_)) {
+    res_on = filt & YKPRED_PLUGIN_NODE_RESOURCES_FIT;
+    aff_on = (filt | pre) & YKPRED_PLUGIN_NODE_AFFINITY;
+    pts_en = (filt & YKPRED_PLUGIN_POD_TOPOLOGY_SPREAD) && (pre & YKPRED_PLUGIN_POD_TOPOLOGY_SPREAD);
+    ipa_en = (filt & YKPRED_PLUGIN_INTER_POD_AFFINITY) && (pre & YKPRED_PLUGIN_INTER_POD_AFFINITY);
+    spread_on = (pts_en || ipa_en) && e->fam_spread.D > 0;
+    fit_error = (pre & YKPRED_PLUGIN_NODE_RESOURCES_FIT) ? 0 : 1;
+    wgroups = (unsigned)((e->row_words + ykk::kWavesPerBlock - 1) / ykk::kWavesPerBlock);
+    as = ykk::AffSigs{e->d_sig_aff_flags.as<unsigned>(), e->d_sig_aff_off.as<int>(), e->d_sig_aff_terms.as<u64>(), e->d_sig_pre_off.as<int>(),
+                      e->d_sig_pre_terms.as<u64>()};
+    auto out_of = [&](const Family& f) {
+      return ykk::PlaneOut{e->planes_canon.as<u64>() + (size_t)f.base * e->row_stride, e->planes_ranked.as<u64>() + (size_t)f.base * e->row_stride,
+                           e->row_stride, f.D, nullptr};
+    };
+    o_res = out_of(e->fam_res);
+    o_tol = out_of(e->fam_tol);
+    o_aff = out_of(e->fam_aff);
+    o_spread = out_of(e->fam_spread);
+  }
+  static unsigned sig_chunks(int D) {
+    const int spb = ykk::sigs_per_block(D);
+    return (unsigned)((D + spb - 1) / spb);
+  }
+  ykk::BasePlanes base_of(DevBuf& buf) const {
+    ykk::BasePlanes bp;
+    bp.req = buf.as<u64>();
+    bp.taint = bp.req + (size_t)64 * e->W * e->row_stride;
+    bp.port = bp.taint + (size_t)64 * e->KT * e->row_stride;
+    bp.unsched = bp.port + (size_t)64 * e->KP * e->row_stride;
+    bp.exists = bp.unsched + e->row_stride;
+    bp.stride = e->row_stride;
+    return bp;
+  }
+  void launch_dictionary_planes(hipStream_t s, const int* perm, bool ranked, const char* base_name, const char* sig_name, bool base_done = false) {
+    ykk::BasePlanes bp = base_of(ranked ? e->base_ranked : e->base_canon);
+    if (!base_done) {
+      tm->begin(s);
+      hipLaunchKernelGGL(ykk::k_base_planes, dim3((unsigned)(e->W + e->KT + e->KP + 1), wgroups), dim3(ykk::kBlock), 0, s, nt, perm, bp,
+                         e->row_words);
+      tm->end(s, base_name);
+    }
+    ykk::SigPlaneArgs sa{};
+    sa.base = bp;
+    sa.tol = o_tol;
+    sa.aff = o_aff;
+    if (ranked) {
+      sa.tol.canon = o_tol.ranked;
+      sa.aff.canon = o_aff.ranked;
+      sa.tol.first = first_r ? first_r + e->fam_tol.base : nullptr;
+      sa.aff.first = first_r ? first_r + e->fam_aff.base : nullptr;
+    }
+    if (!aff_on) sa.aff.D = 0;
+    sa.sig_tol = e->d_sig_tol.as<u64>();
+    sa.sig_tolflags = e->d_sig_tolflags.as<unsigned>();
+    sa.sig_ports = e->d_sig_ports.as<u64>();
+    sa.KP = e->KP;
+    for (int k = 0; k < ykk::kMaxKT; ++k) sa.taint_used[k] = e->taint_used[k];
+    sa.affs = as;
+    sa.KT = e->KT;
+    sa.W = e->W;
+    sa.pre_mask = pre;
+    sa.filt_mask = filt;
+    sa.n_words = e->row_words;
+    tm->begin(s);
+    const int wpl = e->sig_wpl > 0 ? e->sig_wpl : (e->row_words >= 4 * ykk::kWave ? 4 : (e->row_words >= 2 * ykk::kWave ? 2 : 1));
+    const unsigned chunks = std::max((unsigned)((std::max(sa.tol.D, sa.aff.D) + ykk::kBitSigsPerBlock - 1) / ykk::kBitSigsPerBlock), 1u);
+    const unsigned ygroups = (unsigned)((e->row_words + ykk::kBlock * wpl - 1) / (ykk::kBlock * wpl));
+    if (wpl >= 4)
+      hipLaunchKernelGGL(ykk::k_sig_planes<4>, dim3(chunks, ygroups, 2u), dim3(ykk::kBlock), 0, s, sa);
+    else if (wpl >= 2)
+      hipLaunchKernelGGL(ykk::k_sig_planes<2>, dim3(chunks, ygroups, 2u), dim3(ykk::kBlock), 0, s, sa);
+    else
+      hipLaunchKernelGGL(ykk::k_sig_planes<1>, dim3(chunks, ygroups, 2u), dim3(ykk::kBlock), 0, s, sa);
+    tm->end(s, sig_name);
+  }
+  void launch_ballot_planes(hipStream_t s, const int* perm, const char* name, bool with_base = false) {
+    ykk::PlaneArgs pa{};
+    pa.perm = perm;
+    pa.res = o_res;
+    pa.spread = o_spread;
+    if (perm && first_r) {
+      pa.res.first = first_r + e->fam_res.base;
+      pa.spread.first = first_r + e->fam_spread.base;
+    }
+    if (!spread_on) pa.spread.D = 0;
+    pa.dims = ykk::DimPlanes{e->d_dim_val.as<i64>(), e->d_dim_order.as<int>(), e->d_dim_chunk_dim.as<int>(), e->d_dim_chunk_begin.as<int>(),
+                             e->d_dim_chunk_len.as<int>(), res_on ? e->dim_chunks : 0};
+    pa.spreads = spread_sigs(e);
+    pa.fit_error = fit_error;
+    pa.n_words = e->row_words;
+    pa.spread_en = pts_en ? 1 : 0;
+    pa.ipa_en = ipa_en ? 1 : 0;
+    unsigned xchunks = std::max((unsigned)pa.dims.n_chunks, sig_chunks(pa.spread.D));
+    tm->begin(s);
+    if (with_base) {
+      xchunks = std::max(xchunks, (unsigned)(e->W + e->KT + e->KP + 1));
+      hipLaunchKernelGGL(ykk::k_node_planes, dim3(std::max(xchunks, 1u), wgroups, 3u), dim3(ykk::kBlock), 0, s, nt, pa,
+                         base_of(perm ? e->base_ranked : e->base_canon));
+    } else {
+      hipLaunchKernelGGL(ykk::k_planes, dim3(std::max(xchunks, 1u), wgroups, spread_on ? 2u : 1u), dim3(ykk::kBlock), 0, s, nt, pa);
+    }
+    tm->end(s, name);
+    const bool ranked = perm != nullptr;
+    if (res_on && e->n_big > 0 && !fit_error) {
+      ykk::DimWalk dw{e->d_dim_val.as<i64>(), e->d_dim_order.as<int>(), e->d_big_dim.as<int>(), e->d_walk_big.as<int>(), e->d_walk_begin.as<int>(),
+                      e->d_walk_len.as<int>(), (ranked ? e->d_sfree_r : e->d_sfree_c).as<i64>(), (ranked ? e->d_pmask_r : e->d_pmask_c).as<u64>(),
+                      e->n_big, e->walk_chunks, e->row_words, ranked ? nullptr : e->d_rbits_c.as<u64>(),
+                      (!ranked && sweep_rows_on) ? e->d_ent_c.as<unsigned>() : nullptr, e->d_sorted.as<i64>(), e->d_sorted_off.as<int>(),
+                      (ranked && use_run_decide) ? e->d_glin_r.as<unsigned>() : nullptr};
+      tm->begin(s);
+      hipLaunchKernelGGL(ykk::k_dim_sort, dim3((unsigned)e->n_big, wgroups), dim3(ykk::kBlock), 0, s, nt, perm, dw);
+      tm->end(s, ranked ? "k_dim_sort(ranked)" : "k_dim_sort");
+      tm->begin(s);
+      const unsigned walk_gy = (unsigned)((e->row_words + ykk::kBlock * ykk::kWalkWords - 1) / (ykk::kBlock * ykk::kWalkWords));
+      const dim3 walk_grid((unsigned)e->walk_chunks, walk_gy);
+      if (!ranked && use_sweep && e->walk2_chunks >= 0) {
+        if (e->walk2_chunks > 0) {
+          ykk::DimWalk dw2 = dw;
+          dw2.order = e->d_walk2_order.as<int>();
+          dw2.chunk_big = e->d_walk2_big.as<int>();
+          dw2.chunk_begin = e->d_walk2_begin.as<int>();
+          dw2.chunk_len = e->d_walk2_len.as<int>();
+          dw2.n_chunks = e->walk2_chunks;
+          hipLaunchKernelGGL(ykk::k_dim_walk, dim3((unsigned)e->walk2_chunks, walk_gy), dim3(ykk::kBlock), 0, s, dw2, e->d_idx_c.as<unsigned char>(), e->idx_stride);
+        }
+      } else if (!ranked) {
+        hipLaunchKernelGGL(ykk::k_dim_walk, walk_grid, dim3(ykk::kBlock), 0, s, dw, e->d_idx_c.as<unsigned char>(), e->idx_stride);
+      } else {
+        hipLaunchKernelGGL(ykk::k_dim_prefix_max, dim3((unsigned)e->n_big), dim3(ykk::kPfxBlock), 0, s, dw, e->d_pfx_r.as<i64>());
+        if (use_run_decide) {
+          if (e->walk2_chunks > 0) {
+            ykk::DimWalk dw2 = dw;
+            dw2.order = e->d_walk2_order.as<int>();
+            dw2.chunk_big = e->d_walk2_big.as<int>();
+            dw2.chunk_begin = e->d_walk2_begin.as<int>();
+            dw2.chunk_len = e->d_walk2_len.as<int>();
+            dw2.n_chunks = e->walk2_chunks;
+            hipLaunchKernelGGL(ykk::k_dim_walk_window<8>, dim3((unsigned)e->walk2_chunks, walk_gy), dim3(ykk::kBlock), 0, s, dw2, e->d_pfx_r.as<i64>(), e->d_win_r.as<unsigned char>());
+          }
+        } else {
+          hipLaunchKernelGGL(ykk::k_dim_walk_window<ykk::kWalkBatch>, walk_grid, dim3(ykk::kBlock), 0, s, dw, e->d_pfx_r.as<i64>(), e->d_win_r.as<unsigned char>());
+        }
+      }
+      tm->end(s, ranked ? "k_dim_walk(ranked)" : "k_dim_walk");
+    } else if (res_on && e->n_big > 0) {
+      if (!ranked) (void)hipMemsetAsync(e->d_idx_c.p, 64, (size_t)e->fam_res.D * (size_t)e->idx_stride, s);
+      (void)hipMemsetAsync((ranked ? e->d_pmask_r : e->d_pmask_c).p, 0, (size_t)e->n_big * (size_t)e->row_words * 65 * sizeof(u64), s);
+      if (!ranked) (void)hipMemsetAsync(e->d_rbits_c.p, 0, (size_t)e->n_big * (size_t)e->row_words * ykk::kRankBits * sizeof(u64), s);
+    }
+  }
+  enum { kFirst = 1, kDictionary = 2, kBallot = 4, kAll = 7 };
+  void launch_ranked(hipStream_t s, int parts) {
+    if ((parts & kFirst) && first_r) (void)hipMemsetAsync(first_r, 0x7f, (size_t)std::max(e->plane_rows_alloc, 1) * sizeof(int), s);
+    if (parts & kDictionary) launch_dictionary_planes(s, e->d_perm.as<int>(), true, "k_base_planes(ranked)", "k_sig_planes(ranked)");
+    if (parts & kBallot) {
+      const int ballot_rows = e->fam_tol.base;
+      if (ballot_rows <= ykk::kManySigs && e->n_big == 0) {
+        tm->begin(s);
+        hipLaunchKernelGGL(ykk::k_permute_planes, dim3(sig_chunks(ballot_rows), wgroups), dim3(ykk::kBlock), 0, s, e->N, e->d_perm.as<int>(),
+                           e->planes_canon.as<u64>(), e->planes_ranked.as<u64>(), e->row_stride, ballot_rows, e->row_words, first_r);
+        tm->end(s, "k_permute_planes");
+      } else if (res_on || spread_on) {
+        launch_ballot_planes(s, e->d_perm.as<int>(), "k_planes(ranked)");
+      }
+    }
+  }
+};
+
+int build_ranked_planes(ykpred_engine* e, hipStream_t st, unsigned pre, unsigned filt) {
+  Timer tm{e, false};
+  PlaneJobs pj(e, &tm, pre, filt);
+  if (e->decide_skip) {
+    HIPCHK(e->d_first_r.ensure((size_t)std::max(e->plane_rows_alloc, 1) * sizeof(int)));
+    pj.first_r = e->d_first_r.as<int>();
+  }
+  if (pj.res_on && e->n_big > 0 && !pj.fit_error) HIPCHK(e->d_pfx_r.ensure((size_t)e->n_big * (size_t)std::max(e->row_words, 1) * sizeof(i64)));
+  pj.launch_ranked(st, PlaneJobs::kAll);
+  HIPCHK(hipGetLastError());
+  e->win_partial = false;
+  e->ranked_specs_version = e->specs_version;
+  e->ranked_nodes_epoch = e->nodes_epoch;
+  e->ranked_pre = pre;
+  e->ranked_filt = filt;
+  e->ranked_has_first = e->decide_skip;
+  return YKPRED_OK;
+}
+
 }
 
 #define YK_SERIALISE(eng) \
@@ -1515,6 +1720,7 @@
   if (cfg->reserved[5] > 0) e->wave_combine_below = cfg->reserved[5];
   if (cfg->reserved[5] < 0) e->wave_combine_below = 0;
   if (cfg->reserved[6] < 0) e->bands_enabled = false;
+  if (cfg->reserved[7] < 0) e->decide_rows = 0;
   if (cfg->reserved[6] > 0) e->band_steps = std::min(256, std::max(4, (cfg->reserved[6] + 3) / 4 * 4));
   e->graph_disabled = cfg->reserved[3] != 1;
   {
@@ -1549,6 +1755,7 @@
       else if (key == "fail_after") e->fail_after = std::max(val, 0);
       else if (key == "round_prof") e->round_prof = val;
       else if (key == "round_batched") e->round_batched = val;
+      else if (key == "decide_rows") e->decide_rows = val;
       else if (key == "round_node_assume") e->round_node_assume = val;
       else if (key == "sweep_min_run") e->sweep_min_run = std::max(val, 0);
       else if (key == "sweep_groups") e->sweep_groups = std::max(val, 0);
@@ -2169,6 +2376,10 @@
   const int nblk_nodes = (N + ykk::kBlock - 1) / ykk::kBlock;
 
   bool use_run_decide_pass = false;
+  const bool rows_decide = e->decide_rows != 0 && want_dec && !(a->options & (YKPRED_EVAL_SKIP_BITMAP | YKPRED_EVAL_DIRTY_CLASSES | YKPRED_EVAL_DIRECT |
+                                                                              YKPRED_EVAL_SPREAD_COUNT_ONLY)) &&
+                           e->early_counts != 0 && e->n_classes_a > 0 && e->patch_chunks == 0 && !((long)e->NC * e->wave_combine_below > (long)P) &&
+                           e->n_classes_b <= 16384 && e->n_big == 0 && (size_t)e->row_stride * sizeof(u64) <= (size_t)48 * 1024;
   auto enqueue = [&]() -> int {
   if (spread_on || (a->options & YKPRED_EVAL_SPREAD_COUNT_ONLY)) {
     const bool ready = a->options & YKPRED_EVAL_SPREAD_COUNTS_READY, only = a->options & YKPRED_EVAL_SPREAD_COUNT_ONLY;
@@ -2189,22 +2400,10 @@
     return 1;
   }
 
-  const unsigned wgroups = (unsigned)((e->row_words + ykk::kWavesPerBlock - 1) / ykk::kWavesPerBlock);
-  const bool res_on = filt & YKPRED_PLUGIN_NODE_RESOURCES_FIT;
-  const bool aff_on = (filt | pre) & YKPRED_PLUGIN_NODE_AFFINITY;
-  const int fit_error = (pre & YKPRED_PLUGIN_NODE_RESOURCES_FIT) ? 0 : 1;
-  auto sig_chunks = [](int D) {
-    const int spb = ykk::sigs_per_block(D);
-    return (unsigned)((D + spb - 1) / spb);
-  };
-  ykk::AffSigs as{e->d_sig_aff_flags.as<unsigned>(), e->d_sig_aff_off.as<int>(), e->d_sig_aff_terms.as<u64>(), e->d_sig_pre_off.as<int>(),
-                  e->d_sig_pre_terms.as<u64>()};
-  auto canon_of = [&](const Family& f) { return e->planes_canon.as<u64>() + (size_t)f.base * e->row_stride; };
-  auto ranked_of = [&](const Family& f) { return e->planes_ranked.as<u64>() + (size_t)f.base * e->row_stride; };
-  ykk::PlaneOut o_res{canon_of(e->fam_res), ranked_of(e->fam_res), e->row_stride, e->fam_res.D, nullptr};
-  ykk::PlaneOut o_tol{canon_of(e->fam_tol), ranked_of(e->fam_tol), e->row_stride, e->fam_tol.D, nullptr};
-  ykk::PlaneOut o_aff{canon_of(e->fam_aff), ranked_of(e->fam_aff), e->row_stride, e->fam_aff.D, nullptr};
-  ykk::PlaneOut o_spread{canon_of(e->fam_spread), ranked_of(e->fam_spread), e->row_stride, e->fam_spread.D, nullptr};
+  PlaneJobs pj(e, &tm, pre, filt);
+  const bool res_on = pj.res_on, aff_on = pj.aff_on;
+  const int fit_error = pj.fit_error;
+  const ykk::PlaneOut &o_res = pj.o_res, &o_tol = pj.o_tol, &o_aff = pj.o_aff, &o_spread = pj.o_spread;
   const bool full_pass = !(a->options & (YKPRED_EVAL_SKIP_BITMAP | YKPRED_EVAL_DIRTY_CLASSES));
   const bool counts_early_here = e->early_counts != 0 && full_pass && e->n_classes_a > 0 && e->patch_chunks == 0 &&
                                  !((long)e->NC * e->wave_combine_below > (long)P) && e->n_classes_b <= 16384;
@@ -2224,10 +2423,14 @@
                  e->row_stride, e->d_res_rows.as<int>(), 1 + e->R, e->d_idx_c.as<unsigned char>(), e->idx_stride, e->d_pmask_c.as<u64>(), e->row_words,
                  nullptr, 0, 0, 0, 0, 0, nullptr, nullptr, nullptr, nullptr, nullptr};
   int* first_r = nullptr;
-  if ((a->options & (YKPRED_OUT_DECISIONS | YKPRED_OUT_DECISION_KEYS)) && e->decide_skip) {
+  if (want_dec && !rows_decide && e->decide_skip) {
     HIPCHK(e->d_first_r.ensure((size_t)std::max(e->plane_rows_alloc, 1) * sizeof(int)));
     first_r = e->d_first_r.as<int>();
   }
+  pj.first_r = first_r;
+  pj.use_run_decide = use_run_decide;
+  pj.use_sweep = use_sweep;
+  pj.sweep_rows_on = sweep_rows_on;
   if (want_dec && res_on && e->n_big > 0 && !fit_error) HIPCHK(e->d_pfx_r.ensure((size_t)e->n_big * (size_t)std::max(e->row_words, 1) * sizeof(i64)));
   ykk::Planes pr = ranked_planes_of(e, pre, filt, spread_on, first_r != nullptr);
   pc.n_big = pr.n_big;
@@ -2242,7 +2445,7 @@
       HIPCHK(hipMemsetAsync(e->d_class_count.p, 0, (size_t)e->C * sizeof(int), sb));
       HIPCHK(hipEventRecord(e->ev_zero, sb));
     }
-    if (first_r) HIPCHK(hipMemsetAsync(first_r, 0x7f, (size_t)std::max(e->plane_rows_alloc, 1) * sizeof(int), sb));
+    if (!rows_decide) pj.launch_ranked(sb, PlaneJobs::kFirst);
     tm.begin(sb);
     hipLaunchKernelGGL(ykk::k_score, dim3((unsigned)nblk_nodes), dim3(ykk::kBlock), 0, sb, nt, e->d_score.as<double>(), e->d_key.as<u64>());
     tm.end(sb, "k_score");
@@ -2261,151 +2464,14 @@
                        e->d_member_tie.as<int>(), e->d_member_key.as<u64>(), e->d_rank.as<int>(), e->d_perm.as<int>());
     tm.end(sb, "k_rank");
   }
-  auto base_of = [&](DevBuf& buf) {
-    ykk::BasePlanes bp;
-    bp.req = buf.as<u64>();
-    bp.taint = bp.req + (size_t)64 * e->W * e->row_stride;
-    bp.port = bp.taint + (size_t)64 * e->KT * e->row_stride;
-    bp.unsched = bp.port + (size_t)64 * e->KP * e->row_stride;
-    bp.exists = bp.unsched + e->row_stride;
-    bp.stride = e->row_stride;
-    return bp;
-  };
-  auto launch_dictionary_planes = [&](hipStream_t s, const int* perm, bool ranked, const char* base_name, const char* sig_name, bool base_done = false) -> int {
-    ykk::BasePlanes bp = base_of(ranked ? e->base_ranked : e->base_canon);
-    if (!base_done) {
-      tm.begin(s);
-      hipLaunchKernelGGL(ykk::k_base_planes, dim3((unsigned)(e->W + e->KT + e->KP + 1), wgroups), dim3(ykk::kBlock), 0, s, nt, perm, bp,
-                         e->row_words);
-      tm.end(s, base_name);
-    }
-    ykk::SigPlaneArgs sa{};
-    sa.base = bp;
-    sa.tol = o_tol;
-    sa.aff = o_aff;
-    if (ranked) {
-      sa.tol.canon = o_tol.ranked;
-      sa.aff.canon = o_aff.ranked;
-      sa.tol.first = first_r ? first_r + e->fam_tol.base : nullptr;
-      sa.aff.first = first_r ? first_r + e->fam_aff.base : nullptr;
-    }
-    if (!aff_on) sa.aff.D = 0;
-    sa.sig_tol = e->d_sig_tol.as<u64>();
-    sa.sig_tolflags = e->d_sig_tolflags.as<unsigned>();
-    sa.sig_ports = e->d_sig_ports.as<u64>();
-    sa.KP = e->KP;
-    for (int k = 0; k < ykk::kMaxKT; ++k) sa.taint_used[k] = e->taint_used[k];
-    sa.affs = as;
-    sa.KT = e->KT;
-    sa.W = e->W;
-    sa.pre_mask = pre;
-    sa.filt_mask = filt;
-    sa.n_words = e->row_words;
-    tm.begin(s);
-    const int wpl = e->sig_wpl > 0 ? e->sig_wpl : (e->row_words >= 4 * ykk::kWave ? 4 : (e->row_words >= 2 * ykk::kWave ? 2 : 1));
-    const unsigned chunks = std::max((unsigned)((std::max(sa.tol.D, sa.aff.D) + ykk::kBitSigsPerBlock - 1) / ykk::kBitSigsPerBlock), 1u);
-    const unsigned ygroups = (unsigned)((e->row_words + ykk::kBlock * wpl - 1) / (ykk::kBlock * wpl));
-    if (wpl >= 4)
-      hipLaunchKernelGGL(ykk::k_sig_planes<4>, dim3(chunks, ygroups, 2u), dim3(ykk::kBlock), 0, s, sa);
-    else if (wpl >= 2)
-      hipLaunchKernelGGL(ykk::k_sig_planes<2>, dim3(chunks, ygroups, 2u), dim3(ykk::kBlock), 0, s, sa);
-    else
-      hipLaunchKernelGGL(ykk::k_sig_planes<1>, dim3(chunks, ygroups, 2u), dim3(ykk::kBlock), 0, s, sa);
-    tm.end(s, sig_name);
-    return YKPRED_OK;
-  };
-  if (want_dec) TRY(launch_dictionary_planes(sb, e->d_perm.as<int>(), true, "k_base_planes(ranked)", "k_sig_planes(ranked)"));
-  auto ranked_walk = [](const int* perm) { return perm != nullptr; };
-  auto launch_ballot_planes = [&](hipStream_t s, const int* perm, const char* name, bool with_base = false) {
-    ykk::PlaneArgs pa{};
-    pa.perm = perm;
-    pa.res = o_res;
-    pa.spread = o_spread;
-    if (perm && first_r) {
-      pa.res.first = first_r + e->fam_res.base;
-      pa.spread.first = first_r + e->fam_spread.base;
-    }
-    if (!spread_on) pa.spread.D = 0;
-    pa.dims = ykk::DimPlanes{e->d_dim_val.as<i64>(), e->d_dim_order.as<int>(), e->d_dim_chunk_dim.as<int>(), e->d_dim_chunk_begin.as<int>(),
-                             e->d_dim_chunk_len.as<int>(), res_on ? e->dim_chunks : 0};
-    pa.spreads = spread_sigs(e);
-    pa.fit_error = fit_error;
-    pa.n_words = e->row_words;
-    pa.spread_en = pts_en ? 1 : 0;
-    pa.ipa_en = ipa_en ? 1 : 0;
-    unsigned xchunks = std::max((unsigned)pa.dims.n_chunks, sig_chunks(pa.spread.D));
-    tm.begin(s);
-    if (with_base) {
-      xchunks = std::max(xchunks, (unsigned)(e->W + e->KT + e->KP + 1));
-      hipLaunchKernelGGL(ykk::k_node_planes, dim3(std::max(xchunks, 1u), wgroups, 3u), dim3(ykk::kBlock), 0, s, nt, pa,
-                         base_of(perm ? e->base_ranked : e->base_canon));
-    } else {
-      hipLaunchKernelGGL(ykk::k_planes, dim3(std::max(xchunks, 1u), wgroups, spread_on ? 2u : 1u), dim3(ykk::kBlock), 0, s, nt, pa);
-    }
-    tm.end(s, name);
-    if (res_on && e->n_big > 0 && !fit_error) {
-      const bool ranked = perm != nullptr;
-      ykk::DimWalk dw{e->d_dim_val.as<i64>(), e->d_dim_order.as<int>(), e->d_big_dim.as<int>(), e->d_walk_big.as<int>(), e->d_walk_begin.as<int>(),
-                      e->d_walk_len.as<int>(), (ranked ? e->d_sfree_r : e->d_sfree_c).as<i64>(), (ranked ? e->d_pmask_r : e->d_pmask_c).as<u64>(),
-                      e->n_big, e->walk_chunks, e->row_words, ranked ? nullptr : e->d_rbits_c.as<u64>(),
-                      (!ranked && sweep_rows_on) ? e->d_ent_c.as<unsigned>() : nullptr, e->d_sorted.as<i64>(), e->d_sorted_off.as<int>(),
-                      (ranked && use_run_decide) ? e->d_glin_r.as<unsigned>() : nullptr};
-      tm.begin(s);
-      hipLaunchKernelGGL(ykk::k_dim_sort, dim3((unsigned)e->n_big, wgroups), dim3(ykk::kBlock), 0, s, nt, perm, dw);
-      tm.end(s, ranked ? "k_dim_sort(ranked)" : "k_dim_sort");
-      tm.begin(s);
-      const unsigned walk_gy = (unsigned)((e->row_words + ykk::kBlock * ykk::kWalkWords - 1) / (ykk::kBlock * ykk::kWalkWords));
-      const dim3 walk_grid((unsigned)e->walk_chunks, walk_gy);
-      if (!ranked && use_sweep && e->walk2_chunks >= 0) {
-        if (e->walk2_chunks > 0) {
-          ykk::DimWalk dw2 = dw;
-          dw2.order = e->d_walk2_order.as<int>();
-          dw2.chunk_big = e->d_walk2_big.as<int>();
-          dw2.chunk_begin = e->d_walk2_begin.as<int>();
-          dw2.chunk_len = e->d_walk2_len.as<int>();
-          dw2.n_chunks = e->walk2_chunks;
-          hipLaunchKernelGGL(ykk::k_dim_walk, dim3((unsigned)e->walk2_chunks, walk_gy), dim3(ykk::kBlock), 0, s, dw2, e->d_idx_c.as<unsigned char>(), e->idx_stride);
-        }
-      } else if (!ranked) {
-        hipLaunchKernelGGL(ykk::k_dim_walk, walk_grid, dim3(ykk::kBlock), 0, s, dw, e->d_idx_c.as<unsigned char>(), e->idx_stride);
-      } else {
-        hipLaunchKernelGGL(ykk::k_dim_prefix_max, dim3((unsigned)e->n_big), dim3(ykk::kPfxBlock), 0, s, dw, e->d_pfx_r.as<i64>());
-        if (use_run_decide) {
-          if (e->walk2_chunks > 0) {
-            ykk::DimWalk dw2 = dw;
-            dw2.order = e->d_walk2_order.as<int>();
-            dw2.chunk_big = e->d_walk2_big.as<int>();
-            dw2.chunk_begin = e->d_walk2_begin.as<int>();
-            dw2.chunk_len = e->d_walk2_len.as<int>();
-            dw2.n_chunks = e->walk2_chunks;
-            hipLaunchKernelGGL(ykk::k_dim_walk_window<8>, dim3((unsigned)e->walk2_chunks, walk_gy), dim3(ykk::kBlock), 0, s, dw2, e->d_pfx_r.as<i64>(), e->d_win_r.as<unsigned char>());
-          }
-        } else {
-          hipLaunchKernelGGL(ykk::k_dim_walk_window<ykk::kWalkBatch>, walk_grid, dim3(ykk::kBlock), 0, s, dw, e->d_pfx_r.as<i64>(), e->d_win_r.as<unsigned char>());
-        }
-      }
-      tm.end(s, ranked ? "k_dim_walk(ranked)" : "k_dim_walk");
-    } else if (res_on && e->n_big > 0) {
-      if (!ranked_walk(perm)) (void)hipMemsetAsync(e->d_idx_c.p, 64, (size_t)e->fam_res.D * (size_t)e->idx_stride, s);
-      (void)hipMemsetAsync((ranked_walk(perm) ? e->d_pmask_r : e->d_pmask_c).p, 0, (size_t)e->n_big * (size_t)e->row_words * 65 * sizeof(u64), s);
-      if (!ranked_walk(perm)) (void)hipMemsetAsync(e->d_rbits_c.p, 0, (size_t)e->n_big * (size_t)e->row_words * ykk::kRankBits * sizeof(u64), s);
-    }
-  };
+  if (want_dec && !rows_decide) pj.launch_ranked(sb, PlaneJobs::kDictionary);
   const bool fused_planes = res_on || spread_on;
-  if (fused_planes) launch_ballot_planes(st, nullptr, "k_planes+k_base_planes", true);
-  TRY(launch_dictionary_planes(st, nullptr, false, "k_base_planes", "k_sig_planes", fused_planes));
-  if (want_dec) {
+  if (fused_planes) pj.launch_ballot_planes(st, nullptr, "k_planes+k_base_planes", true);
+  pj.launch_dictionary_planes(st, nullptr, false, "k_base_planes", "k_sig_planes", fused_planes);
+  if (want_dec && !rows_decide) {
     HIPCHK(hipEventRecord(e->ev_planes, st));
     HIPCHK(hipStreamWaitEvent(sb, e->ev_planes, 0));
-    const int ballot_rows = e->fam_tol.base;
-    if (ballot_rows <= ykk::kManySigs && e->n_big == 0) {
-      tm.begin(sb);
-      hipLaunchKernelGGL(ykk::k_permute_planes, dim3(sig_chunks(ballot_rows), wgroups), dim3(ykk::kBlock), 0, sb, N, e->d_perm.as<int>(),
-                         e->planes_canon.as<u64>(), e->planes_ranked.as<u64>(), e->row_stride, ballot_rows, e->row_words, first_r);
-      tm.end(sb, "k_permute_planes");
-    } else if (res_on || spread_on) {
-      launch_ballot_planes(sb, e->d_perm.as<int>(), "k_planes(ranked)");
-    }
+    pj.launch_ranked(sb, PlaneJobs::kBallot);
     if (use_run_decide) {
       tm.begin(sb);
       hipLaunchKernelGGL(ykk::k_run_decide, dim3((unsigned)((e->run_ranges + ykk::kWavesPerBlock - 1) / ykk::kWavesPerBlock)), dim3(ykk::kBlock), 0, sb, pr,
@@ -2463,6 +2529,14 @@
       if (counts_early && want_dec) {
         HIPCHK(hipEventRecord(e->ev_counts, st));
         HIPCHK(hipStreamWaitEvent(sb, e->ev_counts, 0));
+        if (rows_decide) {
+          tm.begin(sb);
+          hipLaunchKernelGGL(ykk::k_decide_rows, dim3((unsigned)(e->n_classes_a + e->n_classes_b)), dim3(ykk::kBlock),
+                             (size_t)e->row_stride * sizeof(u64), sb, ct, pc, e->d_class_list_a.as<int>(), e->n_classes_a, e->d_class_list_b.as<int>(),
+                             e->n_classes_b, e->d_class_rows_a.as<u64>(), e->row_words, e->row_stride, N, e->d_perm.as<int>(),
+                             e->d_class_count.as<int>(), pin_on, e->d_class_best.as<int>());
+          tm.end(sb, "k_decide_rows");
+        }
         tm.begin(sb);
         hipLaunchKernelGGL(ykk::k_scatter, dim3((unsigned)((P + ykk::kBlock - 1) / ykk::kBlock)), dim3(ykk::kBlock), 0, sb, P,
                            e->d_pod_class.as<int>(), e->d_class_count.as<int>(), e->d_class_best.as<int>(), e->d_key.as<u64>(),
@@ -2725,9 +2799,13 @@
   e->last_pre = pre;
   e->last_filt = filt;
   e->last_eval_valid = true;
+  e->canon_specs_version = e->specs_version;
+  e->canon_nodes_epoch = e->nodes_epoch;
   if (!(a->options & (YKPRED_EVAL_SKIP_BITMAP | YKPRED_EVAL_DIRTY_CLASSES))) e->n_full_evals++;
   if (!(a->options & (YKPRED_EVAL_SKIP_BITMAP | YKPRED_EVAL_DIRTY_CLASSES))) std::fill(e->h_row_stale.begin(), e->h_row_stale.end(), 0);
-  if (want_dec) {
+  if (want_dec && rows_decide) {
+    e->rank_valid = true;
+  } else if (want_dec) {
     e->win_partial = use_run_decide_pass;
     e->rank_valid = true;
     e->ranked_specs_version = e->specs_version;
@@ -3180,8 +3258,10 @@
   Range roctx_range("ykpred:allocate_round");
   if (!e || n_asks < 0 || (n_asks > 0 && (!asks || !out_nodes))) return fail(e, YKPRED_E_INVALID, "allocate_round: bad argument");
   const bool sharded = e->comm && e->comm_world > 1;
+  const bool ranked_stale = e->ranked_pre != pre || e->ranked_filt != filt || e->ranked_nodes_epoch != e->nodes_epoch || e->ranked_specs_version != e->specs_version;
+  const bool canon_current = e->canon_specs_version == e->specs_version && e->canon_nodes_epoch == e->nodes_epoch;
   const bool stale = e->classes_dirty || !e->last_eval_valid || !e->rank_valid || e->bitmap_epoch != e->nodes_epoch || pre != e->last_pre || filt != e->last_filt ||
-                     e->ranked_pre != pre || e->ranked_filt != filt || e->ranked_nodes_epoch != e->nodes_epoch || e->ranked_specs_version != e->specs_version;
+                     (ranked_stale && !canon_current);
   const bool fx_current = e->fx_version == e->specs_version;
   const bool topo_on = (pre & filt & (YKPRED_PLUGIN_POD_TOPOLOGY_SPREAD | YKPRED_PLUGIN_INTER_POD_AFFINITY)) && e->fam_spread.D > 0;
   const bool ports_on = (pre & filt & YKPRED_PLUGIN_NODE_PORTS) && e->KP > 0;
@@ -3253,6 +3333,7 @@
   HIPCHK(hipSetDevice(e->cfg.device));
   hipStream_t st = e->own_stream;
   if (e->ev_eval_done) HIPCHK(hipStreamWaitEvent(st, e->ev_eval_done, 0));
+  if (ranked_stale) TRY(build_ranked_planes(e, st, pre, filt));
   if (topo_on) TRY(ensure_histograms(e, st));
   const bool live_ports = port_asks || (ports_on && e->fx_ports && fx_current);
   const size_t N = (size_t)std::max(e->N, 1), R = (size_t)e->R, C = (size_t)std::max(e->C, 1), RW = (size_t)std::max(e->row_words, 1);
diff --git a/yunikorn-k8shim_amd/csrc/engine/kernels.hip.h b/yunikorn-k8shim_amd/csrc/engine/kernels.hip.h
--- a/yunikorn-k8shim_amd/csrc/engine/kernels.hip.h
+++ b/yunikorn-k8shim_amd/csrc/engine/kernels.hip.h
@@ -2146,6 +2146,75 @@
     }
   }
   if (live && l == 0) class_best[cls] = best;
+}
+
+constexpr int kDecideRowsUnroll = 4, kDecideRowsPositions = kBlock * kDecideRowsUnroll;
+__global__ __launch_bounds__(kBlock) void k_decide_rows(ClassTable ct, Planes pl, const int* __restrict__ class_list_a, int n_a,
+                                                        const int* __restrict__ class_list_b, int n_b, const u64* __restrict__ row_table,
+                                                        int row_words, int row_stride, int n_nodes, const int* __restrict__ perm,
+                                                        const int* __restrict__ class_count, int pin_enabled, int* __restrict__ class_best) {
+  typedef u64 u64x2 __attribute__((ext_vector_type(2)));
+  extern __shared__ u64 s_row[];
+  __shared__ int s_first[2];
+  const int k = blockIdx.x, tid = threadIdx.x;
+  if (k >= n_a + n_b) return;
+  const bool in_a = k < n_a;
+  const int cls = in_a ? class_list_a[k] : class_list_b[k - n_a];
+  const bool all_fail = pin_enabled & 2;
+  const int pin = (pin_enabled & 1) ? ct.pin[cls] : -1;
+  if (pin == -2 || all_fail || class_count[cls] == 0) {
+    if (tid == 0) class_best[cls] = -1;
+    return;
+  }
+  const u64* src = row_table + (size_t)k * row_stride;
+  ClassRows cr;
+  if (!in_a) cr = class_rows(pl, ct.sig[cls * 4 + 0], ct.sig[cls * 4 + 1], ct.sig[cls * 4 + 2], ct.sig[cls * 4 + 3]);
+  if (pin >= 0) {
+    if (tid == 0) {
+      const u64 x = in_a ? src[pin >> 6] : class_word(cr, pin >> 6);
+      class_best[cls] = ((x >> (pin & 63)) & 1ull) ? pin : -1;
+    }
+    return;
+  }
+  if (in_a) {
+    for (int w = 2 * tid; w < row_stride; w += 2 * kBlock) *(u64x2*)(s_row + w) = *(const u64x2*)(src + w);
+  } else {
+    for (int w = tid; w < row_stride; w += kBlock) s_row[w] = w < row_words ? class_word(cr, w) : 0ull;
+  }
+  if (tid < 2) s_first[tid] = 0x7fffffff;
+  __syncthreads();
+  int node[kDecideRowsUnroll], next[kDecideRowsUnroll];
+#pragma unroll
+  for (int u = 0; u < kDecideRowsUnroll; ++u) {
+    const int pos = u * kBlock + tid;
+    next[u] = pos < n_nodes ? perm[pos] : -1;
+  }
+  int best = -1;
+  for (int base = 0, step = 0; base < n_nodes; base += kDecideRowsPositions, ++step) {
+#pragma unroll
+    for (int u = 0; u < kDecideRowsUnroll; ++u) node[u] = next[u];
+#pragma unroll
+    for (int u = 0; u < kDecideRowsUnroll; ++u) {
+      const int pos = base + kDecideRowsPositions + u * kBlock + tid;
+      next[u] = pos < n_nodes ? perm[pos] : -1;
+    }
+    int found = 0x7fffffff;
+#pragma unroll
+    for (int u = kDecideRowsUnroll - 1; u >= 0; --u) {
+      const int n = node[u];
+      const bool bit = n >= 0 && ((s_row[n >> 6] >> (n & 63)) & 1ull);
+      const u64 any = __ballot(bit);
+      if (any) found = base + u * kBlock + (tid & ~(kWave - 1)) + (__ffsll((long long)any) - 1);
+    }
+    if (found != 0x7fffffff && (tid & (kWave - 1)) == 0) atomicMin(&s_first[step & 1], found);
+    __syncthreads();
+    const int first = s_first[step & 1];
+    if (first != 0x7fffffff) {
+      best = perm[first];
+      break;
+    }
+  }
+  if (tid == 0) class_best[cls] = best;
 }
 
 constexpr int kRunDecideRows = 512;
```
